# ayumiymk/DiG

Measured on AMD Instinct MI355X. Metric: pretrain images/sec (32x128, 2-view, mask 0.7) ViT-S/4, higher is better.
Workload: dtype bf16

## Files before the change

### cpu_abi/dig_cpu.cpp

```cpp
#include <algorithm>
#include <cmath>
#include <cstdint>
#include <cstring>
#include <vector>

#include "dig_cpu_common.h"

namespace {

inline float gelu_f(float x) { return 0.5f * x * (1.0f + std::erf(x * 0.70710678118654752f)); }
inline float dgelu_f(float x) {
  const float cdf = 0.5f * (1.0f + std::erf(x * 0.70710678118654752f));
  return cdf + x * 0.39894228040143268f * std::exp(-0.5f * x * x);
}
inline float drop_apply(float v, const dig_dropout_t& d, long long i, int j, int cols) {
  float s = 1.f;
  if (d.pthr) s = drop_keep(d.pk0, d.pk1, (unsigned)(i / d.rows_per_sample), 0u, d.pthr) ? d.pscale : 0.f;
  if (d.thr) {
    s *= d.scale;
    return drop_keep(d.k0, d.k1, (unsigned)i * (unsigned)cols + (unsigned)j, 0u, d.thr) ? v * s : 0.f;
  }
  return v * s;
}

// ... 39 lines not shown
#pragma omp parallel for collapse(2)
    for (int s = 0; s < splits; ++s)
      for (int i = 0; i < I; ++i) {
        const int r0 = s * per, r1 = std::min(R, r0 + per);
        for (int j = 0; j < J; ++j) {
          float acc = 0.f;
          for (int r = r0; r < r1; ++r) acc += a[(size_t)i * R + r] * b[(size_t)j * R + r];
          C[((size_t)s * I + i) * J + j] = acc;
        }
      }
    return DIG_OK;
  }
  const int groups = (I + 63) / 64;
  std::vector<float> csum(colsum_partials ? (size_t)groups * J : 0, 0.f);
#pragma omp parallel for
  for (int g = 0; g < groups; ++g)
    for (int i = g * 64; i < std::min(I, g * 64 + 64); ++i)
      for (int j = 0; j < J; ++j) {
        float acc = 0.f;
        for (int r = 0; r < R; ++r) acc += a[(size_t)i * R + r] * b[(size_t)j * R + r];
        float v = (acc + (bias ? bias[j] : 0.f)) * (j < alpha_cols ? alpha : 1.0f);
        if (act == 1) {
          if (pre) pre[(size_t)i * ldp + j] = f2bf(v);
          v = gelu_f(v);
          if (dropping) v = drop_apply(v, *drop, i, j, J);
        } else if (act == 2) {
          v *= dgelu_f(bf2f(resid[(size_t)i * ldr + j]));
          if (dropping) v = drop_apply(v, *drop, i, j, J);
          if (colsum_partials) csum[(size_t)g * J + j] += v;
        } else if (dropping) {
          v = drop_apply(v, *drop, i, j, J);
        }
        if (resid && act != 2) v += bf2f(resid[(size_t)i * ldr + j]);
        if (out_kind == 0) ((bf16_t*)C_)[(size_t)i * ldc + j] = f2bf(v);
        else ((float*)C_)[(size_t)i * ldc + j] = v;
      }
  if (colsum_partials) std::memcpy(colsum_partials, csum.data(), csum.size() * sizeof(float));
  return DIG_OK;
}

int dig_gemm_bf16(const void* A, const void* B, void* C, int I, int J, int R, int lda, int ldb, int ldc, int trans_a, int trans_b,
                  int out_kind, const float* bias, const void* resid, int ldr, void* pre_act, int ldp, float alpha, int alpha_cols,
                  int act, int splits, int a_rows, int b_rows, int bk, float* colsum_partials, hipStream_t stream) {
  return dig_gemm_bf16_dropout(A, B, C, I, J, R, lda, ldb, ldc, trans_a, trans_b, out_kind, bias, resid, ldr, pre_act, ldp, alpha, alpha_cols,
                               act, splits, a_rows, b_rows, bk, colsum_partials, nullptr, stream);
}

int dig_reduce_partials_bf16(const float* partials, int splits, long long n, void* out_, hipStream_t) {
  if (int rc = dig_rules::reduce_partials_bf16(partials, splits, n, out_)) return rc;
  bf16_t* out = (bf16_t*)out_;
  for (long long e = 0; e < n; ++e) {
    float a = 0.f;
    for (int s = 0; s < splits; ++s) a += partials[(long long)s * n + e];
    out[e] = f2bf(a);
  }
  return DIG_OK;
}
int dig_reduce_partials(const float* partials, int splits, long long n, float* out, int accumulate, hipStream_t) {
  if (int rc = dig_rules::reduce_partials(partials, splits, n, out, accumulate)) return rc;
#pragma omp parallel for
  for (long long e = 0; e < n; ++e) {
    float acc = accumulate ? out[e] : 0.f;
    for (int s = 0; s < splits; ++s) acc += partials[(long long)s * n + e];
    out[e] = acc;
  }
  return DIG_OK;
}

int dig_reduce_partials_multi(const dig_reduce_seg_t* segs, int n_segs, hipStream_t stream) {
  if (int rc = dig_rules::reduce_partials_multi(segs, n_segs)) return rc;
  for (int k = 0; k < n_segs; ++k) {
    const int rc = dig_reduce_partials(segs[k].partials, segs[k].splits, segs[k].n, segs[k].out, 1, stream);
    if (rc) return rc;
  }
  return DIG_OK;
}

int dig_colsum_partials_multi(const dig_colsum_seg_t* segs, int n_segs, hipStream_t) {
  if (int rc = dig_rules::colsum_partials_multi(segs, n_segs)) return rc;
  for (int k = 0; k < n_segs; ++k) {
    const dig_colsum_seg_t& g = segs[k];
    for (int c = 0; c < g.C; ++c) {
      float a = 0.f;
      for (int b = 0; b < g.n_parts; ++b) a += g.partials[(size_t)b * g.stride + c];
      g.out[c] += a;
    }
  }
  return DIG_OK;
}

int dig_attn_fwd_dropout(const void* qkv_, void* ctx_, float* lse, int n_img, int heads, int embed_dim, const dig_dropout_t* drop,
                         int q_rows, hipStream_t) {
  if (int rc = dig_rules::attn_fwd_dropout(qkv_, ctx_, lse, n_img, heads, embed_dim, drop, q_rows)) return rc;
  const bf16_t* qkv = (const bf16_t*)qkv_;
  bf16_t* ctx = (bf16_t*)ctx_;
  const int D = embed_dim, ld = 3 * D, nq = (q_rows + 31) / 32 * 32;
  const bool dropping = drop && drop->thr;
#pragma omp parallel for collapse(2)
  for (int b = 0; b < n_img; ++b)
    for (int h = 0; h < heads; ++h) {
      std::vector<float> s(N_TOK);
      for (int i = 0; i < nq; ++i) {
        const bf16_t* q = qkv + ((size_t)b * N_TOK + i) * ld + h * DH;
        float mx = -3.0e38f;
        for (int j = 0; j < N_TOK; ++j) {
          const bf16_t* k = qkv + ((size_t)b * N_TOK + j) * ld + D + h * DH;
          float acc = 0.f;
          for (int c = 0; c < DH; ++c) acc += bf2f(q[c]) * bf2f(k[c]);
          s[j] = acc;
          mx = std::max(mx, acc);
        }
        float sum = 0.f;
        for (int j = 0; j < N_TOK; ++j) { s[j] = std::exp(s[j] - mx); sum += s[j]; }
        lse[((size_t)b * heads + h) * N_TOK + i] = mx + std::log(sum);
        const float inv = 1.0f / sum;
        float o[DH];
        for (int c = 0; c < DH; ++c) o[c] = 0.f;
        for (int j = 0; j < N_TOK; ++j) {
          float p = s[j] * inv;
          if (dropping) p = drop_keep(drop->k0, drop->k1, ((unsigned)i << 16) | (unsigned)j, (unsigned)(b * heads + h), drop->thr) ? p * drop->scale : 0.f;
          const bf16_t* v = qkv + ((size_t)b * N_TOK + j) * ld + 2 * D + h * DH;
          for (int c = 0; c < DH; ++c) o[c] += p * bf2f(v[c]);
        }
        for (int c = 0; c < DH; ++c) ctx[((size_t)b * N_TOK + i) * D + h * DH + c] = f2bf(o[c]);
      }
    }
  return DIG_OK;
}

int dig_attn_fwd(const void* qkv, void* ctx, float* lse, int n_img, int heads, int embed_dim, hipStream_t stream) {
  return dig_attn_fwd_dropout(qkv, ctx, lse, n_img, heads, embed_dim, nullptr, N_TOK, stream);
}

int dig_attn_bwd_mode(int) { return 0; }
int dig_attn_bwd_store(int) { return 0; }

int dig_attn_block_fwd(const void* ln1, const void* x, const void* qkv_w, const float* qkv_b, const void* proj_w, const float* proj_b,
                       void* qkv, void* ctx, float* lse, void* x_mid, int n_img, int heads, int embed_dim, float scale, hipStream_t stream) {
  if (int rc = dig_rules::attn_block_fwd(ln1, x, qkv_w, qkv_b, proj_w, proj_b, qkv, ctx, lse, x_mid, n_img, heads, embed_dim, scale)) return rc;
  const int D = embed_dim, R = n_img * N_TOK;
  std::vector<bf16_t> tq;
  std::vector<float> tl;
  if (!qkv) {
    tq.resize((size_t)R * 3 * D + 8);
    tl.resize((size_t)n_img * heads * N_TOK);
    qkv = (void*)(((uintptr_t)tq.data() + 15) & ~(uintptr_t)15);
    lse = tl.data();
  }
  int rc = dig_gemm_bf16(ln1, qkv_w, qkv, R, 3 * D, D, D, D, 3 * D, 0, 0, 0, qkv_b, nullptr, 0, nullptr, 0, scale, D, 0, 1, 0, 0, 0, nullptr, stream);
  if (rc) return rc;
  rc = dig_attn_fwd(qkv, ctx, lse, n_img, heads, D, stream);
  if (rc) return rc;
  return dig_gemm_bf16(ctx, proj_w, x_mid, R, D, D, D, D, D, 0, 0, 0, proj_b, x, D, nullptr, 0, 1.0f, 0, 0, 1, 0, 0, 0, nullptr, stream);
}

int dig_attn_bwd_dropout(const void* qkv_, const void* ctx_, const void* dctx_, const float* lse, void* dqkv_, int n_img, int heads,
                         int embed_dim, float scale, float* q_colsum, float* v_colsum, const dig_dropout_t* drop, int q_rows, hipStream_t) {
  if (int rc = dig_rules::attn_bwd_dropout(qkv_, ctx_, dctx_, lse, dqkv_, n_img, heads, embed_dim, scale, q_colsum, v_colsum, drop, q_rows))
    return rc;
  const int nqb = (q_rows + 31) / 32;
  const bf16_t* qkv = (const bf16_t*)qkv_;
  const bf16_t* ctx = (const bf16_t*)ctx_;
  const bf16_t* dctx = (const bf16_t*)dctx_;
  bf16_t* dqkv = (bf16_t*)dqkv_;
  const int D = embed_dim, ld = 3 * D, nq = nqb * 32;
  const bool dropping = drop && drop->thr;
#pragma omp parallel for
  for (int b = 0; b < n_img; ++b) {
    std::vector<float> qs(q_colsum ? D : 0, 0.f), vs(q_colsum ? D : 0, 0.f);
    for (int h = 0; h < heads; ++h) {
      std::vector<float> dk((size_t)N_TOK * DH, 0.f), dv((size_t)N_TOK * DH, 0.f), p(N_TOK), dp(N_TOK);
      for (int i = 0; i < nq; ++i) {
        const size_t row = (size_t)b * N_TOK + i;
        const bf16_t* q = qkv + row * ld + h * DH;
        const bf16_t* o = ctx + row * D + h * DH;
        const bf16_t* go = dctx + row * D + h * DH;
        const float l = lse[((size_t)b * heads + h) * N_TOK + i];
        float delta = 0.f;
        for (int c = 0; c < DH; ++c) delta += bf2f(go[c]) * bf2f(o[c]);
        for (int j = 0; j < N_TOK; ++j) {
          const bf16_t* k = qkv + ((size_t)b * N_TOK + j) * ld + D + h * DH;
          const bf16_t* v = qkv + ((size_t)b * N_TOK + j) * ld + 2 * D + h * DH;
          float s = 0.f, d = 0.f;
          for (int c = 0; c < DH; ++c) { s += bf2f(q[c]) * bf2f(k[c]); d += bf2f(go[c]) * bf2f(v[c]); }
          p[j] = std::exp(s - l);
          dp[j] = d;
        }
        float dq[DH];
        for (int c = 0; c < DH; ++c) dq[c] = 0.f;
        for (int j = 0; j < N_TOK; ++j) {
          float keep = 1.f;
          if (dropping) keep = drop_keep(drop->k0, drop->k1, ((unsigned)i << 16) | (unsigned)j, (unsigned)(b * heads + h), drop->thr) ? drop->scale : 0.f;
          const float pd = bf2f(f2bf(p[j] * keep));
          const float ds = bf2f(f2bf(p[j] * (dp[j] * keep - delta)));
          const bf16_t* k = qkv + ((size_t)b * N_TOK + j) * ld + D + h * DH;
          for (int c = 0; c < DH; ++c) {
            dq[c] += ds * bf2f(k[c]);
            dk[(size_t)j * DH + c] += ds * bf2f(q[c]);
            dv[(size_t)j * DH + c] += pd * bf2f(go[c]);
          }
        }
        for (int c = 0; c < DH; ++c) {
          dqkv[row * ld + h * DH + c] = f2bf(dq[c] * scale);
          if (q_colsum) qs[h * DH + c] += dq[c] * scale;
        }
      }
      for (int j = 0; j < N_TOK; ++j)
        for (int c = 0; c < DH; ++c) {
          dqkv[((size_t)b * N_TOK + j) * ld + D + h * DH + c] = f2bf(dk[(size_t)j * DH + c]);
          dqkv[((size_t)b * N_TOK + j) * ld + 2 * D + h * DH + c] = f2bf(dv[(size_t)j * DH + c]);
          if (q_colsum) vs[h * DH + c] += dv[(size_t)j * DH + c];
        }
    }
    if (q_colsum) {
      std::memcpy(q_colsum + (size_t)b * D, qs.data(), D * sizeof(float));
      std::memcpy(v_colsum + (size_t)b * D, vs.data(), D * sizeof(float));
    }
  }
  return DIG_OK;
}

int dig_attn_bwd(const void* qkv, const void* ctx, const void* dctx, const float* lse, void* dqkv, int n_img, int heads, int embed_dim,
                 float scale, float* q_colsum, float* v_colsum, hipStream_t stream) {
  return dig_attn_bwd_dropout(qkv, ctx, dctx, lse, dqkv, n_img, heads, embed_dim, scale, q_colsum, v_colsum, nullptr, N_TOK, stream);
}

int dig_attn_bwd_proj(const void* qkv, const void* ctx, const void* dy_, const void* projt_, const float* lse, void* dqkv, int n_img, int heads,
                      int embed_dim, float scale, float* q_colsum, float* v_colsum, hipStream_t stream) {
  if (int rc = dig_rules::attn_bwd_proj(qkv, ctx, dy_, projt_, lse, dqkv, n_img, heads, embed_dim, scale, q_colsum, v_colsum)) return rc;
  const int D = embed_dim;
  const long R = (long)n_img * N_TOK;
  const uint16_t* dy = (const uint16_t*)dy_;
  const uint16_t* wt = (const uint16_t*)projt_;
  std::vector<float> w((size_t)D * D);
  for (size_t k = 0; k < w.size(); ++k) w[k] = bf2f(wt[k]);
  std::vector<uint16_t> dctx((size_t)R * D);
#pragma omp parallel for
  for (long r = 0; r < R; ++r) {
    std::vector<float> row(D);
    for (int o = 0; o < D; ++o) row[o] = bf2f(dy[r * D + o]);
    for (int i = 0; i < D; ++i) {
      float a = 0.f;
      for (int o = 0; o < D; ++o) a += row[o] * w[(size_t)i * D + o];
      dctx[r * D + i] = f2bf(a);
    }
  }
  return dig_attn_bwd(qkv, ctx, dctx.data(), lse, dqkv, n_img, heads, embed_dim, scale, q_colsum, v_colsum, stream);
}


int dig_layernorm_fwd(const void* x_, const float* gamma, const float* beta, void* y_, float* mean, float* rstd, int rows, int D, float eps,
                      int fuse_gelu, hipStream_t) {
  if (int rc = dig_rules::layernorm_fwd(x_, gamma, beta, y_, mean, rstd, rows, D, eps, fuse_gelu)) return rc;
  const bf16_t* x = (const bf16_t*)x_;
  bf16_t* y = (bf16_t*)y_;
#pragma omp parallel for
  for (int r = 0; r < rows; ++r) {
    float s = 0.f;
    for (int c = 0; c < D; ++c) s += bf2f(x[(size_t)r * D + c]);
    const float mu = s / D;
    float q = 0.f;
    for (int c = 0; c < D; ++c) { const float d = bf2f(x[(size_t)r * D + c]) - mu; q += d * d; }
    const float rs = 1.0f / std::sqrt(q / D + eps);
    for (int c = 0; c < D; ++c) {
      float v = (bf2f(x[(size_t)r * D + c]) - mu) * rs * gamma[c] + beta[c];
      if (fuse_gelu) v = gelu_f(v);
      y[(size_t)r * D + c] = f2bf(v);
    }
    mean[r] = mu;
    rstd[r] = rs;
  }
  return DIG_OK;
}


int dig_layernorm_bwd_partials(const void* dy_, const void* x_, const float* gamma, const float* beta, const float* mean, const float* rstd,
                               const void* dres_, void* dx_, float* workspace, int rows, int D, int fuse_gelu, hipStream_t) {
  if (int rc = dig_rules::layernorm_bwd_partials(dy_, x_, gamma, beta, mean, rstd, dres_, dx_, workspace, rows, D, fuse_gelu)) return rc;
  const bf16_t* dy = (const bf16_t*)dy_;
  const bf16_t* x = (const bf16_t*)x_;
  const bf16_t* dres = (const bf16_t*)dres_;
  bf16_t* dx = (bf16_t*)dx_;
  const int parts = dig_rules::layernorm_bwd_parts(rows);
  std::memset(workspace, 0, (size_t)parts * 3 * D * sizeof(float));
#pragma omp parallel for
  for (int p = 0; p < parts; ++p) {
    float* w = workspace + (size_t)p * 3 * D;
    std::vector<float> xh(D), d(D);
    for (int r = p; r < rows; r += parts) {
      float c1 = 0.f, c2 = 0.f;
      for (int c = 0; c < D; ++c) {
        xh[c] = (bf2f(x[(size_t)r * D + c]) - mean[r]) * rstd[r];
        float g = bf2f(dy[(size_t)r * D + c]);
        if (fuse_gelu) g *= dgelu_f(xh[c] * gamma[c] + beta[c]);
        w[c] += g * xh[c];
        w[D + c] += g;
        d[c] = g * gamma[c];
        c1 += d[c];
        c2 += d[c] * xh[c];
      }
      c1 /= D;
      c2 /= D;
      for (int c = 0; c < D; ++c) {
        float o = rstd[r] * (d[c] - c1 - xh[c] * c2);
        if (dres) { const float e = bf2f(dres[(size_t)r * D + c]); o += e; w[2 * D + c] += e; }
        dx[(size_t)r * D + c] = f2bf(o);
// ... 1101 lines not shown
```

### dig_amd/block_calls.py

```python
import ctypes
import math
from typing import NamedTuple

import torch

from . import ops

BF16, F32 = torch.bfloat16, torch.float32
_F32_PIECES = ("lse", "mu2", "rs2", "nmu", "nrs")


class Plan(NamedTuple):
    defer: bool
    red_defer: bool
    tile_direct: int
    attn_proj: bool
    fuse_ln2: bool
    chain_proj: bool


class _BlockSaved:
    __slots__ = ("b16", "b32", "off", "rows", "D", "F", "n_img", "heads", "inp", "inp_ptr")

    def __init__(self, b16, b32, off, rows, D, F, n_img, heads, inp, inp_ptr):
        self.b16, self.b32, self.off, self.rows, self.D, self.F, self.n_img, self.heads = b16, b32, off, rows, D, F, n_img, heads
        self.inp = inp
        self.inp_ptr = inp_ptr

    def ptr(self, name):
        return (self.b32 if name in _F32_PIECES else self.b16).data_ptr() + self.off[name]

    def view(self, name):
        R, D, F = self.rows, self.D, self.F
        if name == "lse":
            a = self.off["lse"] // 4
            return self.b32[a:a + self.n_img * self.heads * 256].view(self.n_img * self.heads, 256)
        if name in _F32_PIECES:
            a = self.off[name] // 4
            return self.b32[a:a + R]
        cols = {"qkv": 3 * D, "pre": F, "act": F}.get(name, D)
        a = self.off[name] // 2
        return self.b16[a:a + R * cols].view(R, cols)

    def tensors(self):
        if len(self.inp) == 4:
            x, ln1, mu1, rs1 = self.inp
        else:
            p = self.inp[2]
            x, ln1, mu1, rs1 = p.view("out"), p.view("nln"), p.view("nmu"), p.view("nrs")
        return (x, ln1, mu1, rs1) + tuple(self.view(k) for k in ("qkv", "ctx", "lse", "x_mid", "ln2", "mu2", "rs2", "pre", "act"))


def forward(blocks, x, n_img, heads, Fh, eps, save, fuse_attn):
    R, D = x.shape
    dev = x.device
    off, n16, n32 = ops.block_fwd_layout(R, D, Fh, n_img, heads, save)
    ln1, mu1, rs1 = ops.layernorm_fwd(x, blocks[0]["norm1.weight"], blocks[0]["norm1.bias"], eps)
    inp, inp_ptr = (x, ln1, mu1, rs1), (x.data_ptr(), ln1.data_ptr(), mu1.data_ptr(), rs1.data_ptr())
    stream, key, fuse_attn = ops.L.stream(), ("fwd_call", bool(save), R, n_img), int(fuse_attn)
    saved, prev = [], None
    for i, blk in enumerate(blocks):
        st = blk.get(key)
        if st is None:
            nb = blocks[i + 1] if i + 1 < len(blocks) else None
            st = blk[key] = ops.BlockFwd(
                n_img=n_img, heads=heads, D=D, F=Fh, rows=R, save=int(bool(save)),
                tile_qkv=ops.fwd_tile_code(R, 3 * D, D) or ops.GEMM_BK_FWD, tile_proj=ops.fwd_tile_code(R, D, D, has_resid=True) or ops.GEMM_BK_FWD,
                fuse_attn=fuse_attn, eps=eps, scale=(D // heads) ** -0.5,
                qkv_w=blk["attn.qkv.weight"].data_ptr(), qkv_b=blk["qkv_bias"].data_ptr(), proj_w=blk["attn.proj.weight"].data_ptr(),
                proj_b=blk["attn.proj.bias"].data_ptr(), n2_g=blk["norm2.weight"].data_ptr(), n2_b=blk["norm2.bias"].data_ptr(),
                fc1_w=blk["mlp.fc1.weight"].data_ptr(), fc1_b=blk["mlp.fc1.bias"].data_ptr(), fc2_w=blk["mlp.fc2.weight"].data_ptr(),
                fc2_b=blk["mlp.fc2.bias"].data_ptr(), next_n1_g=nb["norm1.weight"].data_ptr() if nb else None,
                next_n1_b=nb["norm1.bias"].data_ptr() if nb else None)
        b16 = torch.empty(n16 // 2, device=dev, dtype=BF16)
        b32 = torch.empty(n32 // 4, device=dev, dtype=F32)
        p16, p32 = b16.data_ptr(), b32.data_ptr()
        st.fuse_attn = fuse_attn
        st.x, st.ln1 = inp_ptr[0], inp_ptr[1]
        for k in off:
            setattr(st, k, (p32 if k in _F32_PIECES else p16) + off[k])
        ops.L.call("dig_encoder_block_fwd", ctypes.byref(st), stream)
        cur = _BlockSaved(b16, b32, off, R, D, Fh, n_img, heads, inp, inp_ptr)
        if save:
            saved.append(cur)
            inp, inp_ptr = (b16, b32, cur), (p16 + off["out"], p16 + off["nln"], p32 + off["nmu"], p32 + off["nrs"])
        else:
            inp, inp_ptr = (b16, b32), (p16 + off["out"], p16 + off["nln"], 0, 0)
        prev = cur
    return prev.view("out"), saved


def _bwd_struct(blk, wplan, n_img, heads, D, Fh, R):
    g, gb = blk["g"], blk["g"]["qkv_bias"]
    assert all(g[k].is_contiguous() for k in ("attn.qkv.weight", "attn.proj.weight", "mlp.fc1.weight", "mlp.fc2.weight"))
    return ops.BlockBwd(
        n_img=n_img, heads=heads, D=D, F=Fh, rows=R, tile_dgrad=ops.dgrad_tile_code(R, D) or ops.GEMM_BK_BWD, scale=(D // heads) ** -0.5,
        qkv_w=blk["attn.qkv.weight"].data_ptr(), proj_w=blk["attn.proj.weight"].data_ptr(),
        n1_g=blk["norm1.weight"].data_ptr(), n1_b=blk["norm1.bias"].data_ptr(), n2_g=blk["norm2.weight"].data_ptr(),
        n2_b=blk["norm2.bias"].data_ptr(),
        g_n1_g=g["norm1.weight"].data_ptr(), g_n1_b=g["norm1.bias"].data_ptr(), g_qkv_w=g["attn.qkv.weight"].data_ptr(),
        g_q_b=gb.data_ptr(), g_v_b=gb[2 * D:].data_ptr(), g_proj_w=g["attn.proj.weight"].data_ptr(),
        g_proj_b=g["attn.proj.bias"].data_ptr(), g_n2_g=g["norm2.weight"].data_ptr(), g_n2_b=g["norm2.bias"].data_ptr(),
        g_fc1_w=g["mlp.fc1.weight"].data_ptr(), g_fc1_b=g["mlp.fc1.bias"].data_ptr(), g_fc2_w=g["mlp.fc2.weight"].data_ptr(),
        g_fc2_b=g["mlp.fc2.bias"].data_ptr(),
        wg_fn=wplan.fn, wg_wa=wplan.wa, wg_splits=wplan.splits, wg_n_wg=wplan.n_wg, wg_fold_splits=wplan.splits,
        wg_trans=(ctypes.c_int * 4)(*wplan.trans))


def _hold_back(red, g, t32, off, R, n_img, D, Fh, n_b, n_l2):
    def piece(name, *shape):
        a = off[name] // 4
        return t32[a:a + math.prod(shape)].view(shape)
    gb = g["qkv_bias"]
    red.colsum_partials(piece("bparts", n_b, Fh), g["mlp.fc1.bias"])
    red.layernorm_finalize_parts(piece("ws2", n_l2, 3, D), g["norm2.weight"], g["norm2.bias"], g["mlp.fc2.bias"])
    red.colsum_partials(piece("qs", n_img, D), gb[:D])
    red.colsum_partials(piece("vs", n_img, D), gb[2 * D:])
    red.layernorm_finalize(t32[off["ws1"] // 4:], R, D, g["norm1.weight"], g["norm1.bias"], g["attn.proj.bias"])


def backward(plan, blocks, saved, dx, wT, wplan, n_img, heads, Fh, side, keep, block_done, grad_ready):
    R, D = dx.shape
    dev = dx.device
    off, n16, n32 = ops.block_bwd_layout(R, D, Fh, n_img)
    grp = wplan.group
    stream, key = ops.L.stream(), ("bwd_call", R, n_img)
    n_b, n_l2 = ops.L.query("dig_mlp_chain_colsum_rows", R), ops.L.query("dig_mlp_chain_ln_parts", R)
    red = ops.GradReduceBatch() if plan.red_defer else None

    def block(i, dy_ptr, probs, fold=None):
        blk, sv = blocks[i], saved[i]
        saved[i] = None
        st = blk.get(key)
        if st is None:
            st = blk[key] = _bwd_struct(blk, wplan, n_img, heads, D, Fh, R)
        w2t, w1t, projt, qkvt = wT[i]
        st.w2t, st.w1t = w2t.data_ptr(), w1t.data_ptr()
        st.projt = projt.data_ptr() if plan.chain_proj else None
        st.tile_direct, st.attn_proj = plan.tile_direct, int(plan.attn_proj)
        st.proj_wt = projt.data_ptr() if (plan.tile_direct or plan.attn_proj) else None
        st.qkv_wt = qkvt.data_ptr() if plan.tile_direct else None
        st.wg_defer, st.fuse_ln2, st.defer_red = int(plan.defer), int(plan.fuse_ln2), int(plan.red_defer)
        st.x, st.ln1, st.mu1, st.rs1 = sv.inp_ptr
        for k in ("qkv", "ctx", "lse", "x_mid", "ln2", "mu2", "rs2", "pre", "act"):
            setattr(st, k, sv.ptr(k))
        t16 = torch.empty(n16 // 2, device=dev, dtype=BF16)
        t32 = torch.empty(n32 // 4, device=dev, dtype=F32)
        p16, p32 = t16.data_ptr(), t32.data_ptr()
        st.dy = dy_ptr
        for k in off:
            setattr(st, k, (p16 if k in ("dln2", "dpre", "dctx", "dqkv") else p32) + off[k])
        slabs = grp.next_slabs(wplan.slab_bytes)
        st.wg_map, st.wg_slabs, st.wg_probs = wplan.wmap.data_ptr(), slabs.data_ptr(), ctypes.addressof(probs)
        st.wg_fold_n, st.wg_fold_probs, st.wg_fold_slabs = (4, ctypes.addressof(fold[0]), fold[1].data_ptr()) if fold else (0, None, None)
        st.side = side
        if red:
            _hold_back(red, blk["g"], t32, off, R, n_img, D, Fh, n_b, n_l2)
        ops.L.call("dig_encoder_block_bwd", ctypes.byref(st), stream)
        if keep is not None and not red:
            keep(t32)
        block_done()
        return t16, t32, slabs

    def ready(i):
        if i is not None:
            grad_ready(f"encoder.blocks.{i}")

    def inline():
        tables = ((ops._WgProb * 4)(), (ops._WgProb * 4)())
        t16, t32, last, dy_ptr = dx, None, None, dx.data_ptr()
        for n, i in enumerate(reversed(range(len(blocks)))):
            t16, t32, slabs = block(i, dy_ptr, tables[n & 1], last and (last[1], last[2]))
            dy_ptr = t16.data_ptr() + off["dctx"]
            ready(last and last[0])
            last = (i, tables[n & 1], slabs)
        return t16, last

    def deferred():
        t16, t32, held, dy_ptr = dx, None, [], dx.data_ptr()
        for i in reversed(range(len(blocks))):
            own, sv = (ops._WgProb * 4)(), saved[i]
            t16, t32, _ = block(i, dy_ptr, own)
            held.append((i, own, t16, sv))
            dy_ptr = t16.data_ptr() + off["dctx"]
        if red:
            red.flush()
        last = None
        for i, own, _, _ in held:
            slabs = grp.next_slabs(wplan.slab_bytes)
            grp.call(ctypes.addressof(own), 4, ctypes.addressof(last[1]) if last else None, 4 if last else 0, wplan.splits, wplan.wmap, wplan.n_wg,
                     slabs, last and last[2], wplan.splits)
            ready(last and last[0])
            last = (i, own, slabs)
        return t16, last

    t16, (i, table, slabs) = (deferred if plan.defer else inline)()
    grp.fold(ctypes.addressof(table), 4, slabs, wplan.splits)
    ready(i)
    a = off["dctx"] // 2
    return t16[a:a + R * D].view(R, D)


def defer_fits(cache, dev, extra_bytes):
    key = (dev.index, extra_bytes)
    if key not in cache:
        free, _ = torch.cuda.mem_get_info(dev)
        pooled = torch.cuda.memory_reserved(dev) - torch.cuda.memory_allocated(dev)
        cache[key] = extra_bytes <= (free + pooled) // 4
    return cache[key]
```

### dig_amd/build.py

```python
import os
import subprocess
import sys
from concurrent.futures import ThreadPoolExecutor

HERE = os.path.dirname(os.path.abspath(__file__))
CSRC = os.path.join(HERE, "csrc")
LIBDIR = os.path.join(HERE, "lib")
LIB = os.path.join(LIBDIR, "libdig_hip.so")
FLAGS = ["--offload-arch=gfx950", "-O3", "-std=c++17", "-fPIC", "-munsafe-fp-atomics", "-ffp-contract=fast",
         "-Wno-unused-result"]
FLAGS.append("-fno-slp-vectorize")
EXTRA_FLAGS = {"keyview.hip": ["-ffp-contract=off"], "abiaug.hip": ["-ffp-contract=off"]}


def sources():
    return sorted(f for f in os.listdir(CSRC) if f.endswith(".hip"))


def source_hash() -> str:
    import hashlib
    h = hashlib.sha256()
    files = sorted(os.path.join(CSRC, f) for f in os.listdir(CSRC) if f.endswith((".hip", ".h", ".inc")))
    inc = os.path.join(os.path.dirname(HERE), "include")
    files += sorted(os.path.join(inc, f) for f in os.listdir(inc) if f.endswith(".h"))
    for f in files:
        h.update(os.path.basename(f).encode())
        with open(f, "rb") as fh:
            h.update(fh.read())
    h.update(repr((FLAGS, sorted(EXTRA_FLAGS.items()))).encode())
    return h.hexdigest()[:16]


def _stale(out, deps):
    if not os.path.exists(out):
        return True
    t = os.path.getmtime(out)
    return any(os.path.getmtime(d) > t for d in deps)


def build(force: bool = False, verbose: bool = True) -> str:
    hipcc = os.environ.get("HIPCC", "/opt/rocm/bin/hipcc")
    os.makedirs(LIBDIR, exist_ok=True)
    objdir = os.path.join(LIBDIR, "obj")
    os.makedirs(objdir, exist_ok=True)
    headers = [os.path.join(CSRC, f) for f in os.listdir(CSRC) if f.endswith((".h", ".inc"))]
    inc = os.path.join(os.path.dirname(HERE), "include")
    headers += [os.path.join(inc, f) for f in os.listdir(inc) if f.endswith(".h")]
    headers = [h for h in headers if os.path.exists(h)]
    jobs = []
    for s in sources():
        src = os.path.join(CSRC, s)
        obj = os.path.join(objdir, s[:-4] + ".o")
        if force or _stale(obj, [src] + headers):
            jobs.append((src, obj))

    def cc(job):
        src, obj = job
        cmd = [hipcc] + FLAGS + EXTRA_FLAGS.get(os.path.basename(src), []) + ["-I", os.path.join(os.path.dirname(HERE), "include"), "-c", src, "-o", obj]
        r = subprocess.run(cmd, capture_output=True, text=True)
        if r.returncode != 0:
            raise RuntimeError(f"hipcc failed for {src}:\n{r.stderr}")
        if verbose:
            print("[dig_amd.build] compiled", os.path.basename(src), flush=True)

    with ThreadPoolExecutor(max_workers=min(8, max(1, len(jobs)))) as ex:
        list(ex.map(cc, jobs))
    objs = [os.path.join(objdir, s[:-4] + ".o") for s in sources()]
    if force or jobs or _stale(LIB, objs):
        r = subprocess.run([hipcc, "--offload-arch=gfx950", "-shared", "-fPIC", "-o", LIB] + objs,
                           capture_output=True, text=True)
        if r.returncode != 0:
            raise RuntimeError("link failed:\n" + r.stderr)
        if verbose:
            print("[dig_amd.build] linked", LIB, flush=True)
    return LIB


HOT_KERNELS = ("mlp_chain_kernel<1, true, false>", "mlp_chain_kernel<2, true, false>", "mlp_chain_kernel<0, true, false>",
               "wgrad_wide_kernel<3, 7>", "attn_block_kernel<true, 2>", "attn_block_kernel<false, 2>", "attn_bwd_kernel<false, 3, false>", "attn_bwd_kernel<false, 3, true>",
               "gemm_wide_kernel<false, true, 0, 4, 3, 2, 2, false, 64, 2, false>", "gemm_pwide_kernel<4, false, false>",
               "keyview_sample_kernel", "keyview_stage_a_kernel", "keyview_stage_b_kernel",
               "abiaug_sample_kernel", "abiaug_warp_kernel", "abiaug_det_kernel", "abiaug_tail_kernel",
               "lexicon_search_kernel",
               "tcv_fwd_kernel", "tcv_bwd_q_kernel", "tcv_bwd_k_kernel",
               "ctc_kernel<false>", "ctc_kernel<true>",
               "ctc_beam_kernel",
               "ctc_lex_score_kernel",
               "ctc_align_kernel",
               "addattn_fwd_slots_kernel", "attn_beam_advance_kernel")
LLVM_BIN = os.environ.get("DIG_LLVM_BIN", "/opt/rocm/lib/llvm/bin")


def kernel_resources():
    import re
    import tempfile
    rows = []
    objdir = os.path.join(LIBDIR, "obj")
    with tempfile.TemporaryDirectory() as tmp:
        for o in sorted(f for f in os.listdir(objdir) if f.endswith(".o")):
            fat, dev = os.path.join(tmp, o + ".fat"), os.path.join(tmp, o + ".co")
            r = subprocess.run([os.path.join(LLVM_BIN, "llvm-objcopy"), f"--dump-section=.hip_fatbin={fat}", os.path.join(objdir, o)], capture_output=True, text=True)
            if r.returncode != 0 or not os.path.exists(fat):
                continue
            subprocess.run([os.path.join(LLVM_BIN, "clang-offload-bundler"), "--unbundle", "--type=o", f"--input={fat}",
                            "--targets=hipv4-amdgcn-amd-amdhsa--gfx950", f"--output={dev}"], check=True, capture_output=True)
            notes = subprocess.run([os.path.join(LLVM_BIN, "llvm-readelf"), "--notes", dev], check=True, capture_output=True, text=True).stdout
            for blk in notes.split("- .agpr_count")[1:]:
                f = {k: re.search(rf"\.{k}:\s+(\S+)", blk) for k in ("name", "private_segment_fixed_size", "vgpr_count", "sgpr_count")}
                if not all(f.values()):
                    continue
                mangled = f["name"].group(1)
                try:
                    dm = subprocess.run(["c++filt", mangled], capture_output=True, text=True).stdout.strip() or mangled
                except OSError:
                    dm = mangled
                short = re.sub(r"^void ", "", dm).replace("(anonymous namespace)::", "")
                rows.append({"name": short, "object": o, "scratch": int(f["private_segment_fixed_size"].group(1)),
                             "vgpr": int(f["vgpr_count"].group(1)), "sgpr": int(f["sgpr_count"].group(1)),
                             "hot": any(short.startswith(h) for h in HOT_KERNELS)})
    return rows


def check_scratch(rows=None, raise_on_fail=True):
    rows = kernel_resources() if rows is None else rows
    missing = [h for h in HOT_KERNELS if not any(r["name"].startswith(h) for r in rows)]
    bad = [r for r in rows if r["hot"] and r["scratch"] > 0]
    if raise_on_fail and (bad or missing):
        raise RuntimeError(f"hot kernels with scratch memory: {[(b['name'][:60], b['scratch']) for b in bad]}; not found: {missing}")
    return bad + [{"name": m + " (not found)", "scratch": -1} for m in missing]


if __name__ == "__main__":
    build(force="--force" in sys.argv)
```

### dig_amd/csrc/abi_rules.h

```cpp
#pragma once
#include <cstddef>
#include <cstdint>

#include "../../include/dig_hip.h"

static inline bool aligned16(const void* p) { return (((uintptr_t)p) & 15u) == 0; }
static inline bool aligned8(const void* p) { return (((uintptr_t)p) & 7u) == 0; }
static inline bool ranges_overlap(const void* a, const void* b, size_t bytes) {
  const uintptr_t x = (uintptr_t)a, y = (uintptr_t)b;
  return x < y + bytes && y < x + bytes;
}

namespace dig_rules {

constexpr int LDS_LIMIT = 160 * 1024;
constexpr unsigned long long OFFSET_LIMIT = 1ull << 32;
constexpr int ATTN_TOKENS = 256, ATTN_HEAD_DIM = 64;
constexpr int ATTN_BWD_PROJ_MAX_DIM = 512;
constexpr int ATTN_BLOCK_DIM = 384, ATTN_BLOCK_HEADS = 6;
constexpr int GEMM_BR = 64;
constexpr int CHAIN_DIM = 384, CHAIN_FC = 64, CHAIN_ROWS = 128, CHAIN_SLOT = 16384;
constexpr int CHAIN_MAX_F = 6144, CHAIN_LN_MAX_F = 2048;
constexpr int BN_FUSED_COLS = 32, BN_FUSED_MAX_ROWS = 4096, BN_FUSED_MIN_C = 256;
constexpr int PATCH_EMBED_MAX_D = 1024;
// ... 274 lines not shown
}

static inline int layernorm_fwd(const void* x, const float* gamma, const float* beta, void* y, float* mean, float* rstd, int rows, int D, float eps,
                                int fuse_gelu) {
  if (!x || !gamma || !beta || !y || !mean || !rstd || rows <= 0) return DIG_ERR_ARG;
  if (!aligned16(x) || !aligned16(y)) return DIG_ERR_ALIGN;
  if (!layernorm_dim_ok(D)) return DIG_ERR_UNSUPPORTED;
  return DIG_OK;
}
static inline int layernorm_bwd_partials(const void* dy, const void* x, const float* gamma, const float* beta, const float* mean, const float* rstd,
                                         const void* dres, void* dx, float* workspace, int rows, int D, int fuse_gelu) {
  if (!dy || !x || !gamma || !mean || !rstd || !dx || !workspace || rows <= 0) return DIG_ERR_ARG;
  if (fuse_gelu && !beta) return DIG_ERR_ARG;
  if (!aligned16(x) || !aligned16(dy) || !aligned16(dx) || (dres && !aligned16(dres))) return DIG_ERR_ALIGN;
  if (!layernorm_dim_ok(D)) return DIG_ERR_UNSUPPORTED;
  return DIG_OK;
}

static inline int mask_views_u8(const void* mask, int elem_kind, int B, int V, int N, int keep_views, unsigned char* out) {
  if (!mask || !out || B <= 0 || V <= 0 || N <= 0 || keep_views < 0) return DIG_ERR_ARG;
  if (elem_kind < 0 || elem_kind > 4) return DIG_ERR_UNSUPPORTED;
  return DIG_OK;
}
static inline int colsum_partials_multi(const dig_colsum_seg_t* segs, int n_segs) {
  if (!segs || n_segs < 1 || n_segs > DIG_COLSUM_MAX_SEGS) return DIG_ERR_ARG;
  for (int k = 0; k < n_segs; ++k) {
    const dig_colsum_seg_t& g = segs[k];
    if (!g.partials || !g.out || g.n_parts <= 0 || g.C <= 0 || (g.C & 7) || g.stride < g.C || (g.stride & 3)) return DIG_ERR_ARG;
    if (!aligned16(g.partials)) return DIG_ERR_ALIGN;
  }
  return DIG_OK;
}

static inline int beam_step(const float* logits, int ld, float* seq_scores, int B, int beam_width, int C, int eos, long long* symbols,
                            long long* predecessors, float* stored_scores) {
  return beam_common(logits, ld, seq_scores, B, beam_width, BEAM_STEP_MAX_WIDTH, C, symbols, predecessors, stored_scores);
}
static inline int attn_beam_advance(const float* logits, int ld, float* seq_scores, int B, int beam_width, int C, int eos, long long* symbols,
                                    long long* predecessors, float* stored_scores, const long long* force_candidates, const float* s_in,
                                    const void* sbf_in, float* s_out, void* sbf_out, int S, const float* table, int E, void* inp, int ld_inp) {
  if (!s_in || !sbf_in || !s_out || !sbf_out || !table || !inp || S <= 0 || E <= 0 || ld_inp < E) return DIG_ERR_ARG;
  if (int rc = beam_common(logits, ld, seq_scores, B, beam_width, BEAM_ADVANCE_MAX_WIDTH, C, symbols, predecessors, stored_scores)) return rc;
  const size_t rows = (size_t)B * beam_width * S;
  if (ranges_overlap(s_in, s_out, rows * sizeof(float)) || ranges_overlap(sbf_in, sbf_out, rows * 2)) return DIG_ERR_ARG;
  return DIG_OK;
}

static inline int tcv_attn_fwd(const void* film, const void* u, const void* vk, const void* mem, const float* lnc_g, const float* lnc_b, float eps,
                               void* c, float* lse, float* wmean, int S, int Lq, int N, int heads, int d, int slots_per_mem,
                               const dig_dropout_t* drop) {
  if (!c || !lse) return DIG_ERR_ARG;
  if (int rc = tcv_common(film, u, vk, mem, lnc_g, lnc_b, S, Lq, N, heads, d, slots_per_mem)) return rc;
  if (!aligned16(c)) return DIG_ERR_ALIGN;
  return DIG_OK;
}
static inline int tcv_attn_bwd(const void* film, const void* u, const void* vk, const void* mem, const float* lnc_g, const float* lnc_b, float eps,
                               const void* c, const float* lse, const void* dc, void* du, void* dfilm, void* dvk, void* dmem, float* dlnc_g,
                               float* dlnc_b, float* workspace, int S, int Lq, int N, int heads, int d, int slots_per_mem,
                               const dig_dropout_t* drop) {
  if (!c || !lse || !dc || !du || !dfilm || !dvk || !dmem || !dlnc_g || !dlnc_b || !workspace) return DIG_ERR_ARG;
  if (int rc = tcv_common(film, u, vk, mem, lnc_g, lnc_b, S, Lq, N, heads, d, slots_per_mem)) return rc;
  if (slots_per_mem != 1) return DIG_ERR_UNSUPPORTED;
  if (!aligned16(c) || !aligned16(dc) || !aligned16(du) || !aligned16(dfilm) || !aligned16(dvk) || !aligned16(dmem)) return DIG_ERR_ALIGN;
  return DIG_OK;
}

static inline int ctc_loss(const float* logits, int ld, const long long* target, int ldt, const long long* target_len, int len_offset, int B, int T,
                           int C, int blank, float* nll, float* loss) {
  if (!nll || !loss) return DIG_ERR_ARG;
  return ctc_common(logits, ld, target, ldt, target_len, B, T, C, blank);
}
static inline int ctc_loss_bwd(const float* logits, int ld, const long long* target, int ldt, const long long* target_len, int len_offset,
                               const float* gscalar, int B, int T, int C, int blank, void* dlogits, int ldd, int dlogits_is_f32) {
  if (!dlogits || ldd < C) return DIG_ERR_ARG;
  return ctc_common(logits, ld, target, ldt, target_len, B, T, C, blank);
}
static inline int ctc_align(const float* logits, int ld, const long long* target, int ldt, const long long* target_len, int len_offset, int B, int T,
                            int C, int blank, int* start, int* end, float* char_logp, float* path_logp, int* frame_label) {
  if (!start || !end || !char_logp || !path_logp) return DIG_ERR_ARG;
  return ctc_common(logits, ld, target, ldt, target_len, B, T, C, blank);
}

static inline int abiaug_sample(dig_abi_params* params, long long* info, const int* heights, const int* widths, int n_img, const dig_abi_run* run,
                                unsigned long long seed, unsigned step) {
  if (!params || !info || !heights || !widths || n_img <= 0 || !abi_run_ok(run)) return DIG_ERR_ARG;
  return DIG_OK;
}
static inline int abiaug_workspace_bytes(int geom, int det, int wh, int ww, const dig_abi_run* run) {
  if (!abi_run_ok(run) || wh <= 0 || ww <= 0) return DIG_ERR_ARG;
  return DIG_OK;
}
static inline int abiaug_warp_u8(const unsigned char* packed, const long long* offsets, const int* heights, const int* widths, int n_img,
                                 const dig_abi_params* params, const dig_abi_run* run, unsigned char* work, long long work_bytes, int max_wh,
                                 int max_ww) {
  if (!packed || !offsets || !heights || !widths || !params || !abi_run_ok(run) || n_img <= 0 || max_wh <= 0 || max_ww <= 0 ||
      work_bytes < 0 || (work_bytes > 0 && !work))
    return DIG_ERR_ARG;
  return DIG_OK;
}
static inline int abiaug_deteriorate_u8(const unsigned char* packed, const long long* offsets, const int* heights, const int* widths, int n_img,
                                        const dig_abi_params* params, const dig_abi_run* run, unsigned char* work, long long work_bytes, int max_wh,
                                        int max_ww) {
  if (!packed || !offsets || !heights || !widths || !params || !abi_run_ok(run) || n_img <= 0 || max_wh <= 0 || max_ww <= 0 ||
      work_bytes < 0 || (work_bytes > 0 && !work))
    return DIG_ERR_ARG;
  return DIG_OK;
}
static inline int abiaug_tail(const unsigned char* packed, const long long* offsets, const int* heights, const int* widths, int n_img,
                              const dig_abi_params* params, const dig_abi_run* run, const unsigned char* work, long long work_bytes, float* out,
                              int out_h, int out_w, float mean, float std_, int max_wh, int max_ww) {
  if (!packed || !offsets || !heights || !widths || !params || !abi_run_ok(run) || !out || n_img <= 0 || out_h <= 0 || out_w <= 0 ||
      max_wh <= 0 || max_ww <= 0 || std_ == 0.f || work_bytes < 0 || (work_bytes > 0 && !work))
    return DIG_ERR_ARG;
  if (abiaug_tail_lds_bytes(out_h, out_w, resize_taps(max_ww, out_w), resize_taps(max_wh, out_h)) > LDS_LIMIT) return DIG_ERR_UNSUPPORTED;
  return DIG_OK;
}

static inline int attn_fwd_dropout(const void* qkv, void* ctx, float* lse, int n_img, int heads, int embed_dim, const dig_dropout_t* drop,
                                   int q_rows) {
  if (!qkv || !ctx || !lse || n_img <= 0 || heads <= 0 || embed_dim != (long long)heads * ATTN_HEAD_DIM || q_rows < 1 || q_rows > ATTN_TOKENS) return DIG_ERR_ARG;
  if (!aligned16(qkv) || !aligned16(ctx)) return DIG_ERR_ALIGN;
  if (attn_qkv_bytes_over(n_img, embed_dim)) return DIG_ERR_ARG;
  return DIG_OK;
}
static inline int attn_bwd_dropout(const void* qkv, const void* ctx, const void* dctx, const float* lse, void* dqkv, int n_img, int heads,
                                   int embed_dim, float scale, float* q_colsum, float* v_colsum, const dig_dropout_t* drop, int q_rows) {
  if (!qkv || !ctx || !dctx || !lse || !dqkv || n_img <= 0 || heads <= 0 || embed_dim != (long long)heads * ATTN_HEAD_DIM || q_rows < 1 || q_rows > ATTN_TOKENS) return DIG_ERR_ARG;
  if ((q_rows + 31) / 32 < 8 && q_colsum) return DIG_ERR_UNSUPPORTED;
  if ((q_colsum == nullptr) != (v_colsum == nullptr)) return DIG_ERR_ARG;
  if (!aligned16(qkv) || !aligned16(ctx) || !aligned16(dctx) || !aligned16(dqkv)) return DIG_ERR_ALIGN;
  if (attn_qkv_bytes_over(n_img, embed_dim)) return DIG_ERR_ARG;
  return DIG_OK;
}
static inline int attn_bwd_proj(const void* qkv, const void* ctx, const void* dy, const void* projt, const float* lse, void* dqkv, int n_img,
                                int heads, int embed_dim, float scale, float* q_colsum, float* v_colsum) {
  if (!qkv || !ctx || !dy || !projt || !lse || !dqkv || n_img <= 0 || heads <= 0) return DIG_ERR_ARG;
  if ((q_colsum == nullptr) != (v_colsum == nullptr)) return DIG_ERR_ARG;
  if (embed_dim != (long long)heads * ATTN_HEAD_DIM || (embed_dim & 127) || embed_dim > ATTN_BWD_PROJ_MAX_DIM) return DIG_ERR_UNSUPPORTED;
  if (!aligned16(qkv) || !aligned16(ctx) || !aligned16(dy) || !aligned16(projt) || !aligned16(dqkv)) return DIG_ERR_ALIGN;
  if (attn_qkv_bytes_over(n_img, embed_dim)) return DIG_ERR_ARG;
  return DIG_OK;
}

static inline int attn_block_fwd(const void* ln1, const void* x, const void* qkv_w, const float* qkv_b, const void* proj_w, const float* proj_b,
                                 void* qkv, void* ctx, float* lse, void* x_mid, int n_img, int heads, int embed_dim, float scale) {
  if (!ln1 || !x || !qkv_w || !proj_w || !ctx || !x_mid || n_img <= 0) return DIG_ERR_ARG;
  if ((qkv == nullptr) != (lse == nullptr)) return DIG_ERR_ARG;
  if (!attn_block_supported(heads, embed_dim)) return DIG_ERR_UNSUPPORTED;
  if (!aligned16(ln1) || !aligned16(x) || !aligned16(qkv_w) || !aligned16(proj_w) || !aligned16(ctx) || !aligned16(x_mid) || (qkv && !aligned16(qkv)))
    return DIG_ERR_ALIGN;
  if (attn_qkv_bytes_over(n_img, ATTN_BLOCK_DIM)) return DIG_ERR_ARG;
  return DIG_OK;
}

static inline int im2col3x3(const void* x, void* col, int n_img, int H, int W, int C, int ldc) {
  if (!x || !col || n_img <= 0 || H <= 0 || W <= 0 || C <= 0 || (C & 7) || ldc < 9LL * C || (ldc & 7)) return DIG_ERR_ARG;
  if (!aligned16(x) || !aligned16(col)) return DIG_ERR_ALIGN;
  return DIG_OK;
}
static inline int conv3x3_weight_flip(const void* w, void* wt, int c_out, int c_in) {
  if (!w || !wt || c_out <= 0 || c_in <= 0) return DIG_ERR_ARG;
  return DIG_OK;
}
static inline int maxpool2x2_fwd(const void* x, void* y, unsigned char* idx, int n_img, int H, int W, int C) {
  if (!x || !y || !idx || n_img <= 0 || H <= 0 || W <= 0 || (H & 1) || (W & 1) || C <= 0 || (C & 7)) return DIG_ERR_ARG;
  if (!aligned16(x) || !aligned16(y) || !aligned8(idx)) return DIG_ERR_ALIGN;
  return DIG_OK;
}
static inline int maxpool2x2_bwd(const void* dy, const unsigned char* idx, void* dx, int n_img, int H, int W, int C) {
  if (!dy || !dx || !idx || n_img <= 0 || H <= 0 || W <= 0 || (H & 1) || (W & 1) || C <= 0 || (C & 7)) return DIG_ERR_ARG;
  if (!aligned16(dy) || !aligned16(dx) || !aligned8(idx)) return DIG_ERR_ALIGN;
  return DIG_OK;
}

static inline int ctc_greedy_decode(const float* logits, int ld, int B, int T, int C, int blank, int eos, int padding, long long* ids, float* score,
                                    int* n) {
  if (!logits || !ids || !score || !n || B < 0 || T <= 0 || C <= 0 || ld < C) return DIG_ERR_ARG;
  if (T > CTC_MAX_T || C < 2 || C > CTC_MAX_C) return DIG_ERR_UNSUPPORTED;
  return DIG_OK;
}
static inline int ctc_beam_decode(const float* logits, int ld, int B, int T, int C, int blank, int eos, int padding, int beam_width, long long* ids,
                                  float* score, float* logp, int* n) {
  if (!logits || !ids || !score || !logp || !n || B < 0 || T <= 0 || C <= 0 || ld < C || blank < 0 || blank >= C || beam_width <= 0) return DIG_ERR_ARG;
  if (T > CTC_MAX_T || C < 2 || C > CTC_MAX_C || beam_width > CTC_MAX_W) return DIG_ERR_UNSUPPORTED;
  return DIG_OK;
}
static inline int ctc_lexicon_decode(const float* logits, int ld, int B, int T, int C, int blank, int eos, int padding, const int* words,
                                     const int* word_len, int ldw, int W, const int* lex_begin, const int* lex_count, int max_count, int* best_index,
                                     float* logp, long long* ids, float* score, int* n, float* scores, void* workspace, long long workspace_bytes) {
  if (!logits || !words || !word_len || !lex_begin || !lex_count || !best_index || !logp || !ids || !score || !n || !workspace) return DIG_ERR_ARG;
  if (B < 0 || T <= 0 || C <= 0 || ldw <= 0 || ld < C || blank < 0 || blank >= C || W < 0 || max_count < 0) return DIG_ERR_ARG;
  if (T > CTC_MAX_T || C < 2 || C > CTC_MAX_C || ldw > CTC_MAX_LDT || B > GRID_Y_MAX) return DIG_ERR_UNSUPPORTED;
  if (B == 0) return DIG_OK;
  if (!aligned8(workspace)) return DIG_ERR_ALIGN;
  if (workspace_bytes < ctc_lexicon_workspace_bytes(B, T, C, max_count)) return DIG_ERR_ARG;
  return DIG_OK;
}

static inline int decode_embed(const long long* tokens, const float* emb, const float* pe_row, void* x, int B, int d, int vocab) {
  if (!tokens || !emb || !pe_row || !x || B <= 0 || d <= 0 || vocab <= 0) return DIG_ERR_ARG;
  return DIG_OK;
}
static inline int decode_self_attn(const void* qkv_cache, void* out, int B, int T, int heads, int head_dim, int t, float scale) {
  if (!qkv_cache || !out || B <= 0 || heads <= 0 || t < 0 || t >= T) return DIG_ERR_ARG;
  if (!seq_head_dim_ok(head_dim)) return DIG_ERR_UNSUPPORTED;
  return DIG_OK;
}
static inline int decode_cross_attn(const void* q, const void* kv_mem, void* out, float* weights, int B, int n_mem, int heads, int head_dim,
                                    float scale, int slots_per_mem) {
  if (!q || !kv_mem || !out || B <= 0 || n_mem <= 0 || heads <= 0 || slots_per_mem < 1 || B % slots_per_mem) return DIG_ERR_ARG;
  if (!seq_head_dim_ok(head_dim) || n_mem > DECODE_MAX_MEM) return DIG_ERR_UNSUPPORTED;
  if (!aligned16(kv_mem) || !aligned16(q)) return DIG_ERR_ALIGN;
  return DIG_OK;
}
static inline int softmax_argmax(const float* logits, int ld, float* probs, long long* tokens, int B, int C) {
  if (!logits || !probs || !tokens || B <= 0 || C <= 0 || ld < C) return DIG_ERR_ARG;
  return DIG_OK;
}

static inline int patch_embed_fwd(const float* img, const float* W, const float* bias, const unsigned char* mask, const float* mask_token,
                                  const float* pos, void* out, int n_img, int gh, int gw, int D) {
  if (!img || !W || !bias || !mask_token || !pos || !out || n_img <= 0 || D <= 0 || D > PATCH_EMBED_MAX_D || (D & 63)) return DIG_ERR_ARG;
  return DIG_OK;
}
static inline int patch_embed_bwd(const void* dy, const float* img, const unsigned char* mask, float* dW, float* dbias, float* dmask_token,
                                  int n_img, int gh, int gw, int D) {
  if (!dy || !img || !dW || !dbias || !dmask_token || n_img <= 0 || D <= 0 || D > PATCH_EMBED_MAX_D || (D & 63)) return DIG_ERR_ARG;
  return DIG_OK;
}
static inline int window_pool_fwd(const void* x, void* out, int out_is_f32, int n_img, int gh, int gw, int nwin, int D) {
  if (!x || !out || n_img <= 0 || nwin <= 0 || gh <= 0 || gw <= 0 || (D & 1)) return DIG_ERR_ARG;
  return DIG_OK;
}
static inline int window_pool_bwd(const void* dpool, void* dx, int n_img, int gh, int gw, int nwin, int D, int accumulate) {
  if (!dpool || !dx || n_img <= 0 || nwin <= 0 || gh <= 0 || gw <= 0 || (D & 1)) return DIG_ERR_ARG;
  return DIG_OK;
}
static inline int mask_to_index(const unsigned char* mask, int* idx, int* count, int B, int N, int max_per_sample) {
  if (!mask || !idx || !count || B <= 0 || N <= 0 || max_per_sample <= 0) return DIG_ERR_ARG;
  return DIG_OK;
}
static inline int gather_rows(const void* src, const int* idx, void* dst, int M, int M_pad, int D) {
  if (!src || !idx || !dst || M <= 0 || M_pad < M || (D & 7)) return DIG_ERR_ARG;
  if (!aligned16(src) || !aligned16(dst)) return DIG_ERR_ALIGN;
  return DIG_OK;
}
static inline int scatter_rows_add(const void* src, const int* idx, void* dst, int M, int D) {
  if (!src || !idx || !dst || M <= 0 || (D & 7)) return DIG_ERR_ARG;
  if (!aligned16(src) || !aligned16(dst)) return DIG_ERR_ALIGN;
  return DIG_OK;
}
static inline int mim_target(const float* img, const int* idx, float* target, int M, int gh, int gw, int normalize) {
  if (!img || !idx || !target || M <= 0) return DIG_ERR_ARG;
  return DIG_OK;
}
static inline int mse_fwd_bwd_ws(const float* pred, int ld_pred, const float* target, int M, int C, float gscale, float* loss, void* dpred,
                                 int ld_dpred, float* workspace) {
  if (!pred || !target || M <= 0 || C <= 0 || ld_pred < C || (dpred && ld_dpred < C)) return DIG_ERR_ARG;
  return DIG_OK;
}
static inline int add_bf16(const void* a, const void* b, void* out, long long n) {
  if (!a || !b || !out || n <= 0 || (n & 7)) return DIG_ERR_ARG;
  if (!aligned16(a) || !aligned16(b) || !aligned16(out)) return DIG_ERR_ALIGN;
  return DIG_OK;
}
static inline int gelu_bwd(const void* dact, const void* pre, void* dpre, long long n) {
  if (!dact || !pre || !dpre || n <= 0 || (n & 7)) return DIG_ERR_ARG;
  if (!aligned16(dact) || !aligned16(pre) || !aligned16(dpre)) return DIG_ERR_ALIGN;
  return DIG_OK;
}
static inline int colsum(const void* x, float* out, float* workspace, int rows, int C, int ld) {
  if (!x || !out || !workspace || rows <= 0 || C <= 0 || (C & 7) || (ld & 7)) return DIG_ERR_ARG;
  if (!aligned16(x)) return DIG_ERR_ALIGN;
  return DIG_OK;
}
static inline int colsum_partials(const float* partials, int n_parts, int C, float* out) {
  if (!partials || !out || n_parts <= 0 || C <= 0 || (C & 7)) return DIG_ERR_ARG;
  if (!aligned16(partials)) return DIG_ERR_ALIGN;
  return DIG_OK;
}
static inline int patchify_bf16(const float* img, const unsigned char* mask, void* out, int n_img, int gh, int gw) {
  if (!img || !out || n_img <= 0) return DIG_ERR_ARG;
  if (!aligned16(img) || !aligned16(out)) return DIG_ERR_ALIGN;
  return DIG_OK;
}
static inline int colsum_masked(const void* x, const unsigned char* mask, float* out_unmasked, float* out_masked, float* workspace, int rows, int C) {
  if (!x || !mask || !out_unmasked || !out_masked || !workspace || rows <= 0 || C <= 0 || (C & 7)) return DIG_ERR_ARG;
  if (!aligned16(x)) return DIG_ERR_ALIGN;
  return DIG_OK;
}
static inline int dropout_apply(const void* in, void* out, long long rows, int cols, const dig_dropout_t* drop) {
  if (!in || !out || !drop || rows <= 0 || cols <= 0 || (cols & 7) || rows >= (1ll << 32) || rows * cols >= (1ll << 32)) return DIG_ERR_ARG;
  if (drop->pthr && drop->rows_per_sample <= 0) return DIG_ERR_ARG;
  if (!aligned16(in) || !aligned16(out)) return DIG_ERR_ALIGN;
  return DIG_OK;
}

static inline int reduce_partials_bf16(const float* partials, int splits, long long n, void* out) {
  if (!partials || !out || splits < 1 || n <= 0 || (n & 3)) return DIG_ERR_ARG;
  if (!aligned16(partials) || !aligned8(out)) return DIG_ERR_ALIGN;
  return DIG_OK;
}
static inline int reduce_partials(const float* partials, int splits, long long n, float* out, int accumulate) {
  if (!partials || !out || splits < 1 || n <= 0 || (n & 3)) return DIG_ERR_ARG;
  if (!aligned16(partials) || !aligned16(out)) return DIG_ERR_ALIGN;
  return DIG_OK;
// ... 357 lines not shown
```

### dig_amd/csrc/attn_block.hip

```cpp
#include "common.h"
#include "lds_dma.h"
#include "attn_tiles.h"
#include <type_traits>

#ifndef DIG_AB_SAFE_WAITS
#define DIG_AB_SAFE_WAITS 0
#endif
#ifndef DIG_AB_NSPLIT
#define DIG_AB_NSPLIT 2
#endif
#ifndef DIG_AB_P0
#define DIG_AB_P0 2
#define DIG_AB_P1 5
#define DIG_AB_P2 8
#endif
#ifndef DIG_AB_PRIO
#define DIG_AB_PRIO 0
#endif
#ifndef DIG_AB_NT
#define DIG_AB_NT 1
#endif
#ifndef DIG_AB_SKEW
#define DIG_AB_SKEW 0
#endif
#ifndef DIG_AB_ABL
#define DIG_AB_ABL 0
#endif
#ifndef DIG_AB_TS
#define DIG_AB_TS(k)
#define DIG_AB_TS_BEGIN()
#define DIG_AB_TS_END()
#endif

namespace {

constexpr int KD = dig_rules::ATTN_BLOCK_DIM;
constexpr int NH = dig_rules::ATTN_BLOCK_HEADS;
constexpr int SLOTB = 24576;
constexpr int RING_OFF = 0;
constexpr int K_OFF = 3 * SLOTB;
constexpr int V_OFF = K_OFF + 32768;
constexpr int VEC_OFF = V_OFF + 32768;
constexpr int STG_OFF = VEC_OFF + (3 * KD + KD) * 4;
constexpr int LDS_BYTES = STG_OFF + 8 * 2048;
constexpr int NTICK = 48;

struct AbParams {
  const bf16_t* X;
  const bf16_t* resid;
  const bf16_t* Wqkv;
  const float* bqkv;
  const bf16_t* Wp;
  const float* bp;
  bf16_t* qkv;
  bf16_t* ctx;
  float* lse;
  bf16_t* out;
  float scale;
  unsigned x_bytes;
};

template <int N>
__device__ __forceinline__ void ab_wait_vm() {
  if (DIG_AB_SAFE_WAITS) asm volatile("s_waitcnt vmcnt(0)" ::: "memory");
  else asm volatile("s_waitcnt vmcnt(%0)" ::"n"(N) : "memory");
}
__device__ __forceinline__ void ab_wait_lgkm0() { asm volatile("s_waitcnt lgkmcnt(0)" ::: "memory"); }

template <bool NT = false>
__device__ __forceinline__ void store_block_lines(bf16_t* blk , int ld, unsigned (&P)[2][4][2],
                                                  unsigned char* stg, int lane) {
  const int rr = lane & 31, hi = lane >> 5;
  const int wr = (rr & 15) * 128 + hi * 8, ws = rr & 7;
  const int r8 = lane >> 3, c = lane & 7;
#pragma unroll
  for (int pass = 0; pass < 2; ++pass) {
    if ((rr >> 4) == pass) {
#pragma unroll
      for (int b = 0; b < 2; ++b)
#pragma unroll
        for (int g = 0; g < 4; ++g) *reinterpret_cast<uint2*>(stg + wr + (((4 * b + g) ^ ws) << 4)) = make_uint2(P[b][g][0], P[b][g][1]);
    }
    asm volatile("s_waitcnt lgkmcnt(0)" ::: "memory");
    __builtin_amdgcn_wave_barrier();
    const dig_u32x4 v0 = *reinterpret_cast<const dig_u32x4*>(stg + r8 * 128 + ((c ^ (r8 & 7)) << 4));
    const dig_u32x4 v1 = *reinterpret_cast<const dig_u32x4*>(stg + (8 + r8) * 128 + ((c ^ (r8 & 7)) << 4));
    asm volatile("s_waitcnt lgkmcnt(0)" ::: "memory");
    __builtin_amdgcn_wave_barrier();
    if (!(DIG_AB_ABL & 4)) {
      dig_u32x4* d0 = reinterpret_cast<dig_u32x4*>(blk + (size_t)(16 * pass + r8) * ld + c * 8);
      dig_u32x4* d1 = reinterpret_cast<dig_u32x4*>(blk + (size_t)(16 * pass + 8 + r8) * ld + c * 8);
      if (NT) { __builtin_nontemporal_store(v0, d0); __builtin_nontemporal_store(v1, d1); }
      else { *d0 = v0; *d1 = v1; }
    }
  }
}

template <bool SAVE> struct AbCounts {
  static constexpr int E_BLK = (DIG_AB_ABL & 4) ? 0 : (SAVE ? 4 : 0);
  static constexpr int E_ATT = (DIG_AB_ABL & 4) ? 0 : 4 + (SAVE ? 1 : 0);
  static constexpr int E_OUT = (DIG_AB_ABL & 4) ? 0 : 4;
  static constexpr int E_RES = 4;
};

__device__ __forceinline__ int ab_opaque(int v) {
  asm volatile("" : "+v"(v));
  return v;
}

template <bool SAVE, int NSPLIT>
__global__ __launch_bounds__(512) void attn_block_kernel(AbParams p) {
  using C = AbCounts<SAVE>;
  extern __shared__ __attribute__((aligned(16))) unsigned char smem[];
  const int tid0 = threadIdx.x;
  const int wave = __builtin_amdgcn_readfirstlane(tid0 >> 6);
  const int img = blockIdx.x;
  DIG_AB_TS_BEGIN()
#if DIG_AB_PRIO
  if (wave >= 4) __builtin_amdgcn_s_setprio(1);
#endif
#if DIG_AB_SKEW
  for (int i = 0; i < (int)((blockIdx.x >> 3) & 15); ++i) __builtin_amdgcn_s_sleep(DIG_AB_SKEW);
#endif

  const dig_u32x4 rWq = make_rsrc(p.Wqkv, 3u * KD * KD * 2u);
  const dig_u32x4 rWp = make_rsrc(p.Wp, (unsigned)(KD * KD * 2));
  const dig_u32x4 rRes = make_rsrc(p.resid, p.x_bytes);
  const unsigned lds0 = (unsigned)(uintptr_t)LDS_PTR(smem);

  auto piece_voff = [&](int tid, int k) -> unsigned {
    if (k < 2) {
      const int r0 = tid >> 4, c0 = (tid & 15) ^ (r0 & 15);
      return (unsigned)(((r0 + 32 * k) * KD + 8 * c0) * 2);
    }
    const int r2 = tid >> 3, c2 = (tid & 7) ^ ((r2 >> 1) & 7);
    return (unsigned)((r2 * KD + 128 + 8 * c2) * 2);
  };
  dig_u32x4 src_rs = rWq;
  unsigned src_off = 0;
  auto select_source = [&](bool proj, int row0) {
#pragma unroll
    for (int e = 0; e < 4; ++e) src_rs[e] = proj ? rWp[e] : rWq[e];
    src_off = (unsigned)(row0 * KD * 2);
  };
  auto issue_piece = [&](int slot, int tau, int k, unsigned voff) {
    if (DIG_AB_ABL & 16) voff = 0x7fffff00u;
    dma16(lds0 + (unsigned)(RING_OFF + slot * SLOTB + k * 8192 + wave * 1024), voff, src_rs, src_off + (unsigned)(tau * 192 * 2));
  };
#pragma unroll
  for (int tau = 0; tau < 2; ++tau)
#pragma unroll
    for (int k = 0; k < 3; ++k) issue_piece(tau, tau, k, piece_voff(tid0, k));

  dig_u32x4 xf[KD / 16];
  auto load_rows = [&](const bf16_t* base) {
    const int tid = ab_opaque(tid0);
    const auto rX = __builtin_amdgcn_make_buffer_rsrc((void*)base, 0, p.x_bytes, 0x00020000);
    const unsigned xo = (unsigned)((((unsigned)img * 256u + (unsigned)(wave * 32 + (tid & 31))) * KD + ((tid >> 5) & 1) * 8) * 2);
#pragma unroll
    for (int s = 0; s < KD / 16; ++s) xf[s] = __builtin_amdgcn_raw_buffer_load_b128(rX, xo, s * 32, 0);
  };
  load_rows(p.X);
  {
    float* vec = reinterpret_cast<float*>(smem + VEC_OFF);
#pragma unroll
    for (int u = 0; u < 3; ++u) {
      const int i = u * 512 + tid0;
      float v;
      if (i < 3 * KD) v = p.bqkv ? p.bqkv[i] : 0.f;
      else v = p.bp ? p.bp[i - 3 * KD] : 0.f;
      vec[i] = v;
    }
  }

  auto tick = [&](auto slot_tag, auto tau_tag, auto nw_tag, auto pre_tag, f32x16 (&acc)[2], auto&& pre_fn) {
    constexpr int SLOT = decltype(slot_tag)::value, TAU = decltype(tau_tag)::value, NW = decltype(nw_tag)::value;
    constexpr int FREE = (SLOT + 2) % 3;
    DIG_AB_TS(0)
    ab_wait_vm<NW>();
    ab_wait_lgkm0();
    __builtin_amdgcn_s_barrier();
    asm volatile("" ::: "memory");
    DIG_AB_TS(1)
    if (decltype(pre_tag)::value) pre_fn();
    const int tid = ab_opaque(tid0);
    const int rr = tid & 31, hi = (tid >> 5) & 1;
    const int bA = rr * 256 + ((hi ^ (rr & 15)) << 4) + RING_OFF + SLOT * SLOTB;
    const int bB = 16384 + rr * 128 + ((hi ^ ((rr >> 1) & 7)) << 4) + RING_OFF + SLOT * SLOTB;
    auto frag = [&](int s, int half) {
      const int a = s < 8 ? (bA ^ (s << 5)) + half * 8192 : (bB ^ ((s - 8) << 5)) + half * 4096;
      return *reinterpret_cast<const bf16x8*>(smem + a);
    };
    bf16x8 fa[2], fb[2];
    fa[0] = frag(0, 0);
    fa[1] = frag(0, 1);
    __builtin_amdgcn_sched_barrier(0);
    auto kstep = [&](auto s_tag, bf16x8 (&cur)[2], bf16x8 (&nxt)[2]) {
      constexpr int S = decltype(s_tag)::value;
      if constexpr (S < 11) {
        nxt[0] = frag(S + 1, 0);
        nxt[1] = frag(S + 1, 1);
      }
      if (!(DIG_AB_ABL & 2)) {
        acc[0] = __builtin_amdgcn_mfma_f32_32x32x16_bf16(cur[0], __builtin_bit_cast(bf16x8, xf[TAU * 12 + S]), acc[0], 0, 0, 0);
        acc[1] = __builtin_amdgcn_mfma_f32_32x32x16_bf16(cur[1], __builtin_bit_cast(bf16x8, xf[TAU * 12 + S]), acc[1], 0, 0, 0);
      } else {
        asm volatile("" ::"v"(cur[0]), "v"(cur[1]));
      }
      if (S == DIG_AB_P0) issue_piece(FREE, TAU, 0, piece_voff(tid, 0));
      if (S == DIG_AB_P1) issue_piece(FREE, TAU, 1, piece_voff(tid, 1));
      if (S == DIG_AB_P2) issue_piece(FREE, TAU, 2, piece_voff(tid, 2));
      __builtin_amdgcn_sched_barrier(0);
    };
    kstep(std::integral_constant<int, 0>{}, fa, fb); kstep(std::integral_constant<int, 1>{}, fb, fa);
    kstep(std::integral_constant<int, 2>{}, fa, fb); kstep(std::integral_constant<int, 3>{}, fb, fa);
    kstep(std::integral_constant<int, 4>{}, fa, fb); kstep(std::integral_constant<int, 5>{}, fb, fa);
    kstep(std::integral_constant<int, 6>{}, fa, fb); kstep(std::integral_constant<int, 7>{}, fb, fa);
    kstep(std::integral_constant<int, 8>{}, fa, fb); kstep(std::integral_constant<int, 9>{}, fb, fa);
    kstep(std::integral_constant<int, 10>{}, fa, fb); kstep(std::integral_constant<int, 11>{}, fb, fa);
    DIG_AB_TS(2)
  };
  auto no_pre = []() {};
  using FALSE_ = std::false_type;
  using TRUE_ = std::true_type;

  auto finish_block = [&](const f32x16 (&acc)[2], int vec_col0, float al, unsigned (&P)[2][4][2], int hi) {
    const float* bv = reinterpret_cast<const float*>(smem + VEC_OFF + (vec_col0 + 4 * hi) * 4);
#pragma unroll
    for (int b = 0; b < 2; ++b)
#pragma unroll
      for (int g = 0; g < 4; ++g) {
        const f32x4 b4 = *reinterpret_cast<const f32x4*>(bv + 32 * b + 8 * g);
        P[b][g][0] = pack_bf2((acc[b][4 * g] + b4[0]) * al, (acc[b][4 * g + 1] + b4[1]) * al);
        P[b][g][1] = pack_bf2((acc[b][4 * g + 2] + b4[2]) * al, (acc[b][4 * g + 3] + b4[3]) * al);
      }
  };
  const size_t wave_row0 = (DIG_AB_ABL & 32) ? (size_t)wave * 32 : (size_t)img * 256 + wave * 32;

  bf16x8 Qp[4];

  auto head = [&](auto first_tag, int h) {
    constexpr bool FIRST = decltype(first_tag)::value;
    constexpr int EPREV = FIRST ? 0 : C::E_BLK + C::E_ATT;
    using I0 = std::integral_constant<int, 0>;
    using I1 = std::integral_constant<int, 1>;
    using I2 = std::integral_constant<int, 2>;
    f32x16 acc[2];
    unsigned P[2][4][2];
    auto zero = [&]() {
#pragma unroll
      for (int b = 0; b < 2; ++b)
#pragma unroll
        for (int e = 0; e < 16; ++e) acc[b][e] = 0.f;
    };
    select_source(false, KD + h * 64);
    zero();
    tick(I0{}, I0{}, std::integral_constant<int, 3 + EPREV>{}, FALSE_{}, acc, no_pre);
    tick(I1{}, I1{}, std::integral_constant<int, 3 + EPREV>{}, FALSE_{}, acc, no_pre);
    {
      const int tid = ab_opaque(tid0), hi = (tid >> 5) & 1;
      finish_block(acc, h * 64, p.scale, P, hi);
#pragma unroll
      for (int b = 0; b < 2; ++b)
#pragma unroll
        for (int u = 0; u < 2; ++u)
          Qp[2 * b + u] = __builtin_bit_cast(bf16x8, make_uint4(P[b][2 * u][0], P[b][2 * u][1], P[b][2 * u + 1][0], P[b][2 * u + 1][1]));
      if (SAVE) store_block_lines<(DIG_AB_NT & 1) != 0>(p.qkv + wave_row0 * (3 * KD) + h * 64, 3 * KD, P, smem + STG_OFF + wave * 2048, tid & 63);
    }
    __builtin_amdgcn_sched_barrier(0);
    select_source(false, 2 * KD + h * 64);
    zero();
    tick(I2{}, I0{}, std::integral_constant<int, 3 + C::E_BLK>{}, FALSE_{}, acc, no_pre);
    tick(I0{}, I1{}, std::integral_constant<int, 3 + C::E_BLK>{}, FALSE_{}, acc, no_pre);
    {
      const int tid = ab_opaque(tid0), hi = (tid >> 5) & 1;
      finish_block(acc, KD + h * 64, 1.0f, P, hi);
      unsigned char* kw = smem + K_OFF + wave * 4096 + (tid & 63) * 16;
#pragma unroll
      for (int b = 0; b < 2; ++b)
#pragma unroll
        for (int u = 0; u < 2; ++u)
          *reinterpret_cast<uint4*>(kw + (2 * b + u) * 1024) = make_uint4(P[b][2 * u][0], P[b][2 * u][1], P[b][2 * u + 1][0], P[b][2 * u + 1][1]);
      if (SAVE) store_block_lines<(DIG_AB_NT & 1) != 0>(p.qkv + wave_row0 * (3 * KD) + KD + h * 64, 3 * KD, P, smem + STG_OFF + wave * 2048, tid & 63);
    }
    __builtin_amdgcn_sched_barrier(0);
    select_source(h + 1 == NH, h + 1 == NH ? 0 : (h + 1) * 64);
    zero();
    tick(I1{}, I0{}, std::integral_constant<int, 3 + C::E_BLK>{}, FALSE_{}, acc, no_pre);
    tick(I2{}, I1{}, std::integral_constant<int, 3 + C::E_BLK>{}, FALSE_{}, acc, no_pre);
    {
      const int tid = ab_opaque(tid0), hi = (tid >> 5) & 1;
      finish_block(acc, 2 * KD + h * 64, 1.0f, P, hi);
      const int key = wave * 32 + (tid & 31);
      const int vw = V_OFF + key * 128 + 8 * hi + (swz(key) << 4);
#pragma unroll
      for (int b = 0; b < 2; ++b)
#pragma unroll
        for (int g = 0; g < 4; ++g) *reinterpret_cast<uint2*>(smem + (vw ^ ((4 * b + g) << 4))) = make_uint2(P[b][g][0], P[b][g][1]);
      if (SAVE) store_block_lines<(DIG_AB_NT & 1) != 0>(p.qkv + wave_row0 * (3 * KD) + 2 * KD + h * 64, 3 * KD, P, smem + STG_OFF + wave * 2048, tid & 63);
    }
    ab_wait_lgkm0();
    __builtin_amdgcn_s_barrier();
    asm volatile("" ::: "memory");
    __builtin_amdgcn_sched_barrier(0);

    DIG_AB_TS(3)
    const int tid = ab_opaque(tid0);
    const int lane = tid & 63, hi = lane >> 5;
    f32x16 O[2];
#pragma unroll
    for (int dt = 0; dt < 2; ++dt)
#pragma unroll
      for (int e = 0; e < 16; ++e) O[dt][e] = 0.f;
    float m = 0.f, l = 0.f;
    const unsigned char* Kl = smem + K_OFF + lane * 16;
    const int i16 = lane & 15;
    const int vt0 = V_OFF + u_addr(4 * hi + (i16 >> 2), ((lane >> 4) & 1) * 16 + (i16 & 3) * 4);
    auto vfrag = [&](int blk16, int dt) {
      typedef __attribute__((address_space(3))) bf16x4* lp;
      const int a = vt0 ^ (dt * 64);
      const bf16x4 lo = __builtin_amdgcn_ds_read_tr16_b64_v4i16((lp)(smem + a + blk16 * 2048));
      const bf16x4 h4 = __builtin_amdgcn_ds_read_tr16_b64_v4i16((lp)(smem + (a ^ 32) + 1024 + blk16 * 2048));
      return __builtin_shufflevector(lo, h4, 0, 1, 2, 3, 4, 5, 6, 7);
    };
    auto xhalf = [&](float v, float& lo, float& up) {
      const unsigned a = __float_as_uint(v);
      const auto r = __builtin_amdgcn_permlane32_swap(a, a, false, false);
      const unsigned r0 = r[0], r1 = r[1];
      lo = __uint_as_float(r0);
      up = __uint_as_float(r1);
    };
    auto xhalf_max = [&](float v) {
      float lo, up;
      xhalf(v, lo, up);
      return fmaxf(lo, up);
    };
    constexpr int TPP = 8 / NSPLIT;
#pragma unroll
    for (int part = 0; part < NSPLIT; ++part) {
      f32x16 S[TPP];
#pragma unroll
      for (int kt = 0; kt < TPP; ++kt)
#pragma unroll
        for (int e = 0; e < 16; ++e) S[kt][e] = 0.f;
      __builtin_amdgcn_sched_barrier(0);
      if (!(DIG_AB_ABL & 1)) {
#pragma unroll
        for (int bu = 0; bu < 4; ++bu)
#pragma unroll
          for (int kt = 0; kt < TPP; ++kt)
            S[kt] = __builtin_amdgcn_mfma_f32_32x32x16_bf16(*reinterpret_cast<const bf16x8*>(Kl + ((TPP * part + kt) * 4 + bu) * 1024), Qp[bu],
                                                            S[kt], 0, 0, 0);
      }
      __builtin_amdgcn_sched_barrier(0);
      float mx = S[0][0];
#pragma unroll
      for (int kt = 0; kt < TPP; ++kt)
#pragma unroll
        for (int e = 0; e < 16; ++e) mx = fmaxf(mx, S[kt][e]);
      mx = xhalf_max(mx);
      if (part == 0) {
        m = mx;
      } else {
        const float mn = fmaxf(m, mx);
        const float alpha = __expf(m - mn);
        m = mn;
        l *= alpha;
#pragma unroll
        for (int dt = 0; dt < 2; ++dt)
#pragma unroll
          for (int e = 0; e < 16; ++e) O[dt][e] *= alpha;
      }
      __builtin_amdgcn_sched_barrier(0);
#pragma unroll
      for (int kt = 0; kt < TPP; ++kt) {
        float la = 0.f, lb = 0.f;
#pragma unroll
        for (int e = 0; e < 16; e += 2) {
          const float pa = (DIG_AB_ABL & 8) ? S[kt][e] : __expf(S[kt][e] - m), pb = (DIG_AB_ABL & 8) ? S[kt][e + 1] : __expf(S[kt][e + 1] - m);
          S[kt][e] = pa; S[kt][e + 1] = pb;
          la += pa; lb += pb;
        }
        l += la + lb;
        asm volatile("" : "+v"(l));
        if (!(DIG_AB_ABL & 1)) {
#pragma unroll
          for (int u = 0; u < 2; ++u) {
            const bf16x8 v0 = vfrag((TPP * part + kt) * 2 + u, 0), v1 = vfrag((TPP * part + kt) * 2 + u, 1);
            const bf16x8 pf = pack8(S[kt], u);
            O[0] = __builtin_amdgcn_mfma_f32_32x32x16_bf16(v0, pf, O[0], 0, 0, 0);
            O[1] = __builtin_amdgcn_mfma_f32_32x32x16_bf16(v1, pf, O[1], 0, 0, 0);
          }
        } else {
#pragma unroll
          for (int e = 0; e < 16; ++e) asm volatile("" ::"v"(S[kt][e]));
        }
        __builtin_amdgcn_sched_barrier(0);
      }
    }
    {
      float lo, up;
      xhalf(l, lo, up);
      l = lo + up;
    }
    const float inv = 1.0f / l;
    {
      unsigned Pc[2][4][2];
#pragma unroll
      for (int dt = 0; dt < 2; ++dt)
#pragma unroll
        for (int g = 0; g < 4; ++g) {
          Pc[dt][g][0] = pack_bf2(O[dt][4 * g] * inv, O[dt][4 * g + 1] * inv);
          Pc[dt][g][1] = pack_bf2(O[dt][4 * g + 2] * inv, O[dt][4 * g + 3] * inv);
        }
      store_block_lines<(DIG_AB_NT & 4) != 0>(p.ctx + wave_row0 * KD + h * 64, KD, Pc, smem + STG_OFF + wave * 2048, lane);
    }
    if (SAVE && hi == 0 && !(DIG_AB_ABL & 4)) p.lse[((size_t)img * NH + h) * 256 + wave * 32 + (lane & 31)] = m + __logf(l);
    __builtin_amdgcn_sched_barrier(0);
  };

  head(TRUE_{}, 0);
  for (int h = 1; h < NH; ++h) head(FALSE_{}, h);

  DIG_AB_TS(4)
  asm volatile("s_waitcnt vmcnt(0)" ::: "memory");
  load_rows(p.ctx);
  asm volatile("s_waitcnt vmcnt(0)" ::: "memory");
  auto triple = [&](auto first_tag, int jb0) {
    constexpr bool FIRST = decltype(first_tag)::value;
    using I0 = std::integral_constant<int, 0>;
    using I1 = std::integral_constant<int, 1>;
    using I2 = std::integral_constant<int, 2>;
    auto block = [&](auto s0_tag, auto s1_tag, auto eprev_tag, int jb) {
      constexpr int EPREV = decltype(eprev_tag)::value;
      select_source(true, jb < 5 ? (jb + 1) * 64 : 0);
      f32x16 acc[2];
#pragma unroll
      for (int b = 0; b < 2; ++b)
#pragma unroll
        for (int e = 0; e < 16; ++e) acc[b][e] = 0.f;
      auto res_pre = [&]() {
        const int tid = ab_opaque(tid0), lane = tid & 63;
        const unsigned rbase = ((unsigned)img * 256u + (unsigned)(wave * 32 + (lane >> 3))) * KD;
#pragma unroll
        for (int k = 0; k < 4; ++k)
          dma16(lds0 + (unsigned)(K_OFF + wave * 4096 + k * 1024),
                (unsigned)((rbase + 8 * ((lane & 7) ^ (4 * (k & 1) + (lane >> 4)))) * 2) + (unsigned)(k * 8 * KD * 2), rRes, (unsigned)(jb * 64 * 2));
      };
      tick(s0_tag, I0{}, std::integral_constant<int, 3 + EPREV>{}, TRUE_{}, acc, res_pre);
      tick(s1_tag, I1{}, std::integral_constant<int, 3 + EPREV + C::E_RES>{}, FALSE_{}, acc, no_pre);
      ab_wait_vm<6>();
      const int tid = ab_opaque(tid0), rr = tid & 31, hi = (tid >> 5) & 1;
      unsigned P[2][4][2];
      const float* bv = reinterpret_cast<const float*>(smem + VEC_OFF + (3 * KD + jb * 64 + 4 * hi) * 4);
      const int ro = K_OFF + wave * 4096 + rr * 128 + hi * 8 + (((rr >> 1) & 7) << 4);
#pragma unroll
      for (int b = 0; b < 2; ++b)
#pragma unroll
        for (int g = 0; g < 4; ++g) {
          const f32x4 b4 = *reinterpret_cast<const f32x4*>(bv + 32 * b + 8 * g);
          const uint2 rw = *reinterpret_cast<const uint2*>(smem + (ro ^ ((4 * b + g) << 4)));
          const float v0 = (acc[b][4 * g] + b4[0]) + bf2f((bf16_t)(rw.x & 0xffff));
          const float v1 = (acc[b][4 * g + 1] + b4[1]) + bf2f((bf16_t)(rw.x >> 16));
          const float v2 = (acc[b][4 * g + 2] + b4[2]) + bf2f((bf16_t)(rw.y & 0xffff));
          const float v3 = (acc[b][4 * g + 3] + b4[3]) + bf2f((bf16_t)(rw.y >> 16));
          P[b][g][0] = pack_bf2(v0, v1);
          P[b][g][1] = pack_bf2(v2, v3);
        }
      store_block_lines<(DIG_AB_NT & 2) != 0>(p.out + wave_row0 * KD + jb * 64, KD, P, smem + STG_OFF + wave * 2048, tid & 63);
      __builtin_amdgcn_sched_barrier(0);
    };
    block(I0{}, I1{}, std::integral_constant<int, FIRST ? 0 : C::E_OUT>{}, jb0);
    block(I2{}, I0{}, std::integral_constant<int, C::E_OUT>{}, jb0 + 1);
    block(I1{}, I2{}, std::integral_constant<int, C::E_OUT>{}, jb0 + 2);
  };
  triple(TRUE_{}, 0);
  triple(FALSE_{}, 3);
  asm volatile("s_waitcnt vmcnt(0)" ::: "memory");
  DIG_AB_TS_END()
}

}


extern "C" int dig_attn_block_fwd(const void* ln1, const void* x, const void* qkv_w, const float* qkv_b, const void* proj_w, const float* proj_b,
                                  void* qkv, void* ctx, float* lse, void* x_mid, int n_img, int heads, int embed_dim, float scale,
                                  hipStream_t stream) {
  if (int rc = dig_rules::attn_block_fwd(ln1, x, qkv_w, qkv_b, proj_w, proj_b, qkv, ctx, lse, x_mid, n_img, heads, embed_dim, scale)) return rc;
  const size_t qb = (size_t)n_img * 256 * 3 * KD * 2;
  AbParams p;
  p.X = (const bf16_t*)ln1; p.resid = (const bf16_t*)x; p.Wqkv = (const bf16_t*)qkv_w; p.bqkv = qkv_b; p.Wp = (const bf16_t*)proj_w; p.bp = proj_b;
  p.qkv = (bf16_t*)qkv; p.ctx = (bf16_t*)ctx; p.lse = lse; p.out = (bf16_t*)x_mid; p.scale = scale;
  p.x_bytes = (unsigned)((size_t)n_img * 256 * KD * 2);
  static bool attr[DIG_MAX_DEVICES] = {};
  const int dev = dig_device();
  if (!attr[dev]) {
    if (hipFuncSetAttribute(reinterpret_cast<const void*>(&attn_block_kernel<false, DIG_AB_NSPLIT>), hipFuncAttributeMaxDynamicSharedMemorySize, LDS_BYTES) != hipSuccess ||
        hipFuncSetAttribute(reinterpret_cast<const void*>(&attn_block_kernel<true, DIG_AB_NSPLIT>), hipFuncAttributeMaxDynamicSharedMemorySize, LDS_BYTES) != hipSuccess)
      return DIG_ERR_LAUNCH;
    attr[dev] = true;
  }
  if (qkv) dig_launch(attn_block_kernel<true, DIG_AB_NSPLIT>, dim3(n_img), dim3(512), LDS_BYTES, stream, p);
  else dig_launch(attn_block_kernel<false, DIG_AB_NSPLIT>, dim3(n_img), dim3(512), LDS_BYTES, stream, p);
  return dig_check_launch();
}
```

### dig_amd/csrc/encoder_block.inc

```

#define DIG_BLOCK_TRY(call) do { const int rc_ = (call); if (rc_) return rc_; } while (0)

extern "C" int dig_encoder_block_fwd(const dig_block_fwd_t* b, hipStream_t stream) {
  if (!b || b->rows <= 0 || b->D <= 0 || b->F <= 0 || b->n_img <= 0 || b->heads <= 0 || b->rows != b->n_img * 256) return -1;
  if (!b->x || !b->ln1 || !b->qkv || !b->ctx || !b->lse || !b->x_mid || !b->out) return -1;
  if (b->save && (!b->ln2 || !b->mu2 || !b->rs2 || !b->pre || !b->act)) return -1;
  if (b->next_n1_g && (!b->nln || (b->save && (!b->nmu || !b->nrs)))) return -1;
  const int D = b->D, R = b->rows;
  if (b->fuse_attn && dig_attn_block_supported(b->heads, D)) {
    DIG_BLOCK_TRY(dig_attn_block_fwd(b->ln1, b->x, b->qkv_w, b->qkv_b, b->proj_w, b->proj_b, b->save ? b->qkv : nullptr, b->ctx,
                                     b->save ? b->lse : nullptr, b->x_mid, b->n_img, b->heads, D, b->scale, stream));
  } else {
    DIG_BLOCK_TRY(dig_gemm_bf16(b->ln1, b->qkv_w, b->qkv, R, 3 * D, D, D, D, 3 * D, 0, 0, 0, b->qkv_b, nullptr, 0, nullptr, 0, b->scale, D, 0, 1, 0, 0,
                                b->tile_qkv, nullptr, stream));
    DIG_BLOCK_TRY(dig_attn_fwd(b->qkv, b->ctx, b->lse, b->n_img, b->heads, D, stream));
    DIG_BLOCK_TRY(dig_gemm_bf16(b->ctx, b->proj_w, b->x_mid, R, D, D, D, D, D, 0, 0, 0, b->proj_b, b->x, D, nullptr, 0, 1.0f, 0, 0, 1, 0, 0,
                                b->tile_proj, nullptr, stream));
  }
  return dig_mlp_chain_fwd_ln(b->x_mid, b->x_mid, b->n2_g, b->n2_b, b->eps, b->save ? b->ln2 : nullptr, b->save ? b->mu2 : nullptr,
                              b->save ? b->rs2 : nullptr, b->fc1_w, b->fc1_b, b->fc2_w, b->fc2_b, b->out, b->save ? b->pre : nullptr,
                              b->save ? b->act : nullptr, b->next_n1_g, b->next_n1_b, b->next_n1_g ? b->nln : nullptr,
                              (b->next_n1_g && b->save) ? b->nmu : nullptr, (b->next_n1_g && b->save) ? b->nrs : nullptr, R, D, b->F, stream);
}

extern "C" int dig_encoder_block_bwd(const dig_block_bwd_t* b, hipStream_t stream) {
  if (!b || b->rows <= 0 || b->D <= 0 || b->F <= 0 || b->n_img <= 0 || b->rows != b->n_img * 256) return -1;
  if (!b->dy || !b->dln2 || !b->dpre || !b->dctx || !b->dqkv || !b->bparts || !b->ws1 || !b->ws2 || !b->qs || !b->vs) return -1;
  if (!b->wg_probs || (!b->wg_defer && (!b->wg_map || !b->wg_slabs || (b->wg_fold_n > 0 && (!b->wg_fold_probs || !b->wg_fold_slabs))))) return -1;
  const int D = b->D, F = b->F, R = b->rows;
  dig_wgrad_prob_t* q = b->wg_probs;
  auto prob = [&](int k, const void* dy, int out_dim, const void* x, int in_dim, float* dw) {
    if (b->wg_trans[k]) q[k] = dig_wgrad_prob_t{x, dy, dw, in_dim, out_dim, in_dim, in_dim, out_dim, 1};
    else                q[k] = dig_wgrad_prob_t{dy, x, dw, out_dim, in_dim, in_dim, out_dim, in_dim, 0};
  };
  prob(0, b->dy, D, b->act, F, b->g_fc2_w);
  const bool proj_in = b->fuse_ln2 && b->projt;
  if (b->fuse_ln2) {
    DIG_BLOCK_TRY(dig_mlp_chain_bwd_ln_proj(b->dy, b->w2t, b->pre, b->w1t, b->dpre, b->x_mid, b->n2_g, b->mu2, b->rs2, b->dln2, b->bparts, b->ws2,
                                            proj_in ? b->projt : nullptr, proj_in ? b->dctx : nullptr, R, D, F, stream));
    prob(1, b->dpre, F, b->ln2, D, b->g_fc1_w);
  } else {
    DIG_BLOCK_TRY(dig_mlp_chain_bwd(b->dy, b->w2t, b->pre, b->w1t, b->dpre, b->dln2, b->bparts, R, D, F, stream));
    prob(1, b->dpre, F, b->ln2, D, b->g_fc1_w);
    DIG_BLOCK_TRY(dig_layernorm_bwd_partials(b->dln2, b->x_mid, b->n2_g, b->n2_b, b->mu2, b->rs2, b->dy, b->dln2, b->ws2, R, D, 0, stream));
  }
  prob(2, b->dln2, D, b->ctx, D, b->g_proj_w);
  const bool proj_attn = !proj_in && b->attn_proj && b->proj_wt && (D & 127) == 0 && D <= 512 && D == b->heads * 64;
  if (!proj_in && !proj_attn) {
    if (b->tile_direct && b->proj_wt)
      DIG_BLOCK_TRY(dig_gemm_bf16(b->dln2, b->proj_wt, b->dctx, R, D, D, D, D, D, 0, 0, 0, nullptr, nullptr, 0, nullptr, 0, 1.0f, 0, 0, 1, 0, 0,
                                  b->tile_direct, nullptr, stream));
    else
      DIG_BLOCK_TRY(dig_gemm_bf16(b->dln2, b->proj_w, b->dctx, R, D, D, D, D, D, 0, 1, 0, nullptr, nullptr, 0, nullptr, 0, 1.0f, 0, 0, 1, 0, 0,
                                  b->tile_dgrad, nullptr, stream));
  }
  if (proj_attn)
    DIG_BLOCK_TRY(dig_attn_bwd_proj(b->qkv, b->ctx, b->dln2, b->proj_wt, b->lse, b->dqkv, b->n_img, b->heads, D, b->scale, b->qs, b->vs, stream));
  else
    DIG_BLOCK_TRY(dig_attn_bwd(b->qkv, b->ctx, b->dctx, b->lse, b->dqkv, b->n_img, b->heads, D, b->scale, b->qs, b->vs, stream));
  prob(3, b->dqkv, 3 * D, b->ln1, D, b->g_qkv_w);
  if (!b->wg_defer)
    DIG_BLOCK_TRY(dig_wgrad_group(q, 4, b->wg_fold_probs, b->wg_fold_n, R, b->wg_splits, b->wg_map, b->wg_n_wg, b->wg_slabs, b->wg_fold_slabs,
                                  b->wg_fold_n > 0 ? b->wg_fold_splits : 1, b->wg_fn, b->wg_wa, stream));
  if (b->tile_direct && b->qkv_wt)
    DIG_BLOCK_TRY(dig_gemm_bf16(b->dqkv, b->qkv_wt, b->dctx, R, D, 3 * D, 3 * D, 3 * D, D, 0, 0, 0, nullptr, nullptr, 0, nullptr, 0, 1.0f, 0, 0, 1, 0, 0,
                                b->tile_direct, nullptr, stream));
  else
    DIG_BLOCK_TRY(dig_gemm_bf16(b->dqkv, b->qkv_w, b->dctx, R, D, 3 * D, 3 * D, D, D, 0, 1, 0, nullptr, nullptr, 0, nullptr, 0, 1.0f, 0, 0, 1, 0, 0,
                                b->tile_dgrad, nullptr, stream));
  DIG_BLOCK_TRY(dig_layernorm_bwd_partials(b->dctx, b->x, b->n1_g, b->n1_b, b->mu1, b->rs1, b->dln2, b->dctx, b->ws1, R, D, 0, stream));
  if (b->defer_red) return 0;
  DIG_BLOCK_TRY(DIG_BLOCK_HANDOVER(stream, b->side));
  hipStream_t sd = b->side;
  DIG_BLOCK_TRY(dig_colsum_partials(b->bparts, dig_mlp_chain_colsum_rows(R), F, b->g_fc1_b, sd));
  if (b->fuse_ln2) DIG_BLOCK_TRY(dig_layernorm_bwd_finalize_parts(b->ws2, dig_mlp_chain_ln_parts(R), D, b->g_n2_g, b->g_n2_b, b->g_fc2_b, sd));
  else DIG_BLOCK_TRY(dig_layernorm_bwd_finalize(b->ws2, R, D, b->g_n2_g, b->g_n2_b, b->g_fc2_b, sd));
  DIG_BLOCK_TRY(dig_colsum_partials(b->qs, b->n_img, D, b->g_q_b, sd));
  DIG_BLOCK_TRY(dig_colsum_partials(b->vs, b->n_img, D, b->g_v_b, sd));
  return dig_layernorm_bwd_finalize(b->ws1, R, D, b->g_n1_g, b->g_n1_b, b->g_proj_b, sd);
}
```

### dig_amd/encoder_blocks.py

```python
from typing import NamedTuple

import torch

from . import ops

BF16 = torch.bfloat16
_NO_DROP = (None, None, None)


class Plan(NamedTuple):
    chain: bool = False
    chain_ln: bool = False
    attn_block: bool = False
    chain_bwd: bool = False
    chain_every: int = 1
    chain_phase: int = 0
    chain_lnb: bool = False
    chain_proj: bool = False
    attn_proj: bool = False
    direct: bool = False
    fused_qv: bool = False
    grouping: str = "off"
    inline: bool = False
    side_each: bool = False
    batch_reduce: bool = False
    red_defer: bool = False


def _tensors(s):
    return s if isinstance(s, tuple) else s.tensors()


def _no_mark(name, dev):
    pass


def forward(plan, blocks, x, n_img, heads, eps, save, drops=None, tail=(None, None), frozen=0):
    R, D = x.shape
    scale = (D // heads) ** -0.5
    saved, nxt, last = [], None, len(blocks) - 1
    for i, blk in enumerate(blocks):
        keep = save and i >= frozen
        ln1, mu1, rs1 = nxt if nxt is not None else ops.layernorm_fwd(x, blk["norm1.weight"], blk["norm1.bias"], eps)
        nxt = None
        da, dp, dm = (drops[i] or _NO_DROP) if drops is not None else _NO_DROP
        if plan.attn_block and da is None and dp is None:
            x_mid, ctx, qkv, lse = ops.attn_block_fwd(ln1, x, blk["attn.qkv.weight"], blk["qkv_bias"], blk["attn.proj.weight"],
                                                      blk["attn.proj.bias"], n_img, heads, D, scale, save=keep)
        else:
            qkv = ops.linear_fwd(ln1, blk["attn.qkv.weight"], bias=blk["qkv_bias"], alpha=scale, alpha_cols=D)
            ctx, lse = ops.attn_fwd(qkv, n_img, heads, D, drop=da)
            x_mid = ops.linear_fwd(ctx, blk["attn.proj.weight"], bias=blk["attn.proj.bias"], resid=x, drop=dp)
        if plan.chain_ln:
            ng, nb = (blocks[i + 1]["norm1.weight"], blocks[i + 1]["norm1.bias"]) if i < last else tail
            if i < frozen:
                ng = nb = None
            r = ops.mlp_chain_fwd_ln(x_mid, blk["norm2.weight"], blk["norm2.bias"], eps, blk["mlp.fc1.weight"], blk["mlp.fc1.bias"],
                                     blk["mlp.fc2.weight"], blk["mlp.fc2.bias"], ng, nb, save=keep, drop=dm)
            x_out, ln2, mu2, rs2, pre, act = r["out"], r["ln"], r["ln_mean"], r["ln_rstd"], r["pre"], r["act"]
            if ng is not None:
                nxt = (r["nln"], r["nln_mean"], r["nln_rstd"])
        else:
            ln2, mu2, rs2 = ops.layernorm_fwd(x_mid, blk["norm2.weight"], blk["norm2.bias"], eps)
            if plan.chain and dm is None:
                r = ops.mlp_chain_fwd(ln2, blk["mlp.fc1.weight"], blk["mlp.fc1.bias"], blk["mlp.fc2.weight"], blk["mlp.fc2.bias"], x_mid, save=keep)
                x_out, pre, act = r if keep else (r, None, None)
            else:
                pre = torch.empty((R, blk["mlp.fc1.weight"].shape[0]), device=x.device, dtype=BF16) if keep else None
                act = ops.linear_fwd(ln2, blk["mlp.fc1.weight"], bias=blk["mlp.fc1.bias"], act=1, pre=pre)
                x_out = ops.linear_fwd(act, blk["mlp.fc2.weight"], bias=blk["mlp.fc2.bias"], resid=x_mid, drop=dm)
        if save:
            saved.append((x, ln1, mu1, rs1, qkv, ctx, lse, x_mid, ln2, mu2, rs2, pre, act) if keep else None)
        x = x_out
    return x, saved, nxt


def backward(plan, blocks, saved, dx, wT, n_img, heads, on_side, first=0, drops=None, rows=None, block_done=None, grad_ready=None,
             mark=_no_mark):
    D = dx.shape[1]
    scale = (D // heads) ** -0.5
    dev = dx.device
    grp = ops.WgradGroup(dev) if plan.grouping != "off" else None
    batch_side = grp is not None and not plan.side_each
    vred = ops.GradReduceBatch() if (plan.red_defer and grp) else None
    prev_block = None

    def launch_group(*tensors):
        if plan.inline:
            grp.launch()
        else:
            on_side(grp.launch, *tensors)

    for i in reversed(range(first, len(blocks))):
        blk, g = blocks[i], blocks[i]["g"]
        x, ln1, mu1, rs1, qkv, ctx, lse, x_mid, ln2, mu2, rs2, pre, act = _tensors(saved[i])
        saved[i] = None
        chain = plan.chain_bwd and (i % plan.chain_every == plan.chain_phase % plan.chain_every)
        if rows is not None:
            x, ln1, mu1, rs1, qkv, ctx, x_mid, ln2, mu2, rs2, pre, act = (t[:rows] for t in (x, ln1, mu1, rs1, qkv, ctx, x_mid, ln2, mu2, rs2, pre, act))
            lse = lse[:n_img * heads]
        red = ops.GradReduceBatch() if plan.batch_reduce else None
        wg = red.wgrad if red else ops.linear_wgrad
        csum = red.colsum_partials if red else ops.colsum_partials
        held = []
        late, late_t = [], []

        def side_later(fn, *tensors):
            if batch_side:
                late.append(fn)
                late_t.extend(tensors)
            else:
                on_side(fn, *tensors)
        if grp:
            def wg(dy_, x_, dw_):
                if not grp.add(dy_, x_, dw_):
                    raise RuntimeError("grouped weight gradient: a problem of this block does not fit the group's plan")
                held.extend((dy_, x_))
        da, dp, dm = (drops[i] or _NO_DROP) if drops is not None else _NO_DROP
        dz = ops.dropout_apply(dx, dm)
        if dm is not None:
            on_side(lambda dz=dz: ops.colsum(dz, g["mlp.fc2.bias"]), dz)
        if grp:
            wg(dz, act, g["mlp.fc2.weight"])
        else:
            on_side(lambda dz=dz: wg(dz, act, g["mlp.fc2.weight"]), dz, act)
        dctx = lnp = None
        if chain:
            w2t, w1t = wT[i][0], wT[i][1]
            if dm is not None or red is not None or not plan.chain_lnb:
                dln2, dact, bparts = ops.mlp_chain_bwd(dz, w2t, pre, w1t)
            elif plan.chain_proj:
                dx_mid, dact, bparts, lnp, dctx = ops.mlp_chain_bwd_ln(dx, w2t, pre, w1t, x_mid, blk["norm2.weight"], mu2, rs2, projt=wT[i][2])
                dln2 = dx_mid
            else:
                dx_mid, dact, bparts, lnp = ops.mlp_chain_bwd_ln(dx, w2t, pre, w1t, x_mid, blk["norm2.weight"], mu2, rs2)
                dln2 = dx_mid
            mark("blk: fused MLP backward", dev)
        else:
            dact, bparts = ops.linear_dgrad(dz, blk["mlp.fc2.weight"], gelu_pre=pre, colsum=True)
            dln2 = None
        if grp:
            wg(dact, ln2, g["mlp.fc1.weight"])
            if vred:
                vred.colsum_partials(bparts, g["mlp.fc1.bias"])
            else:
                side_later(lambda: csum(bparts, g["mlp.fc1.bias"]), bparts)
            if plan.grouping == "pair":
                launch_group(*held)
        elif plan.side_each:
            on_side(lambda: csum(bparts, g["mlp.fc1.bias"]), bparts)
            on_side(lambda: wg(dact, ln2, g["mlp.fc1.weight"]), dact, ln2)
        else:
            on_side(lambda: (wg(dact, ln2, g["mlp.fc1.weight"]), csum(bparts, g["mlp.fc1.bias"])), dact, ln2, bparts)
        if dln2 is None:
            dln2 = ops.dgrad_direct(dact, wT[i][1]) if plan.direct else None
            if dln2 is None:
                dln2 = ops.linear_dgrad(dact, blk["mlp.fc1.weight"])
        if lnp is not None and vred:
            vred.layernorm_finalize_parts(lnp, g["norm2.weight"], g["norm2.bias"], g["mlp.fc2.bias"])
        elif lnp is not None:
            side_later(lambda lnp=lnp, g=g: ops.layernorm_finalize_parts(lnp, g["norm2.weight"], g["norm2.bias"], g["mlp.fc2.bias"]), lnp)
        else:
            fc2_b = g["mlp.fc2.bias"] if dm is None else None
            dx_mid, fin2, ws2 = ops.layernorm_bwd(dln2, x_mid, blk["norm2.weight"], blk["norm2.bias"], mu2, rs2, dx, g["norm2.weight"],
                                                  g["norm2.bias"], out=dln2, dres_colsum=fc2_b, defer=True)
            if red or vred:
                (red or vred).layernorm_finalize(ws2, x_mid.shape[0], D, g["norm2.weight"], g["norm2.bias"], fc2_b)
            else:
                side_later(fin2, ws2)
        dzp = ops.dropout_apply(dx_mid, dp)
        if dp is not None:
            on_side(lambda dzp=dzp: ops.colsum(dzp, g["attn.proj.bias"]), dzp)
        if grp:
            wg(dzp, ctx, g["attn.proj.weight"])
        else:
            on_side(lambda dzp=dzp: wg(dzp, ctx, g["attn.proj.weight"]), dzp, ctx)
        mark("blk: LayerNorm backward (norm2)", dev)
        proj_attn = dctx is None and plan.attn_proj and plan.fused_qv and dp is None and da is None
        if dctx is None and not proj_attn:
            dctx = ops.dgrad_direct(dzp, wT[i][2]) if plan.direct else None
            if dctx is None:
                dctx = ops.linear_dgrad(dzp, blk["attn.proj.weight"])
        mark("blk: proj data gradient", dev)
        gb = g["qkv_bias"]
        if plan.fused_qv:
            if proj_attn:
                dqkv, qs, vs = ops.attn_bwd_proj(qkv, ctx, dzp, wT[i][2], lse, n_img, heads, D, scale, bias_sums=True)
                dctx = None
            else:
                dqkv, qs, vs = ops.attn_bwd(qkv, ctx, dctx, lse, n_img, heads, D, scale, bias_sums=True, drop=da)
            mark("blk: attention backward", dev)
            if grp:
                wg(dqkv, ln1, g["attn.qkv.weight"])
                launch_group(*held)
                mark("blk: grouped weight gradients", dev)
                if vred:
                    vred.colsum_partials(qs, gb[:D]); vred.colsum_partials(vs, gb[2 * D:])
                else:
                    side_later(lambda: (csum(qs, gb[:D]), csum(vs, gb[2 * D:])), qs, vs)
            else:
                on_side(lambda: (wg(dqkv, ln1, g["attn.qkv.weight"]), csum(qs, gb[:D]), csum(vs, gb[2 * D:])), dqkv, ln1, qs, vs)
        else:
            dqkv = ops.attn_bwd(qkv, ctx, dctx, lse, n_img, heads, D, scale, drop=da)
            if grp:
                wg(dqkv, ln1, g["attn.qkv.weight"])
                launch_group(*held)
                side_later(lambda: (ops.colsum(dqkv, gb[:D], cols=D), ops.colsum(dqkv[:, 2 * D:], gb[2 * D:], cols=D)), dqkv)
            else:
# ... 56 lines not shown
```

### dig_amd/engine_core.py

```python
import ctypes
import functools
import itertools
import os
import weakref
from typing import Optional, Tuple

import torch

from . import block_calls as BC
from . import encoder_blocks as EB
from . import ops
from .arena import enc_block_views
from .parallel import LOCAL, LocalComm, bn_backward, bn_forward

BF16, F32 = torch.bfloat16, torch.float32
FWD_MODE = os.environ.get("DIG_FWD_MODE", "flip")
CHAIN_BWD_EVERY = max(1, int(os.environ.get("DIG_CHAIN_BWD_EVERY", "1")))
CHAIN_BWD_PHASE = int(os.environ.get("DIG_CHAIN_BWD_PHASE", "0"))
BATCH_REDUCE = os.environ.get("DIG_BATCH_REDUCE", "0") == "1"
FUSED_QV_BIAS_SUMS = os.environ.get("DIG_FUSED_QV_BIAS", "1") != "0"
WGRAD_GROUPING = os.environ.get("DIG_WGRAD_GROUPING", "block")
WGRAD_INLINE = os.environ.get("DIG_WGRAD_INLINE", "1") == "1"
WGRAD_DEFER = os.environ.get("DIG_WGRAD_DEFER", "auto").strip().lower()
if WGRAD_DEFER not in ("auto", "0", "1"):
    raise ValueError(f"DIG_WGRAD_DEFER={WGRAD_DEFER!r}: one of auto, 0, 1")
RED_DEFER = os.environ.get("DIG_RED_DEFER", "1") != "0"
BWD_SINGLE_STREAM = os.environ.get("DIG_BWD_SINGLE", "0") == "1"


PHASE_MARKS = None


def _mark(name, dev):
    if PHASE_MARKS is not None:
        ev = torch.cuda.Event(enable_timing=True)
        ev.record(torch.cuda.current_stream(dev))
        PHASE_MARKS.append((name, ev))


ONLINE_HEADS = ("online", "pix_projector", "patch_extractor", "encoder_projection_layer", "predictor")
MOMENTUM_HEADS = ("momentum", "pix_projector_m", "momentum_patch_extractor", "momentum_projection_layer", None)


class _EncWeights:

    def __init__(self, model, prefix, arena):
        f32, g32 = model._f32, model._g32 if arena == "online" else {}
        self.blocks = enc_block_views(model.specs, prefix, model.depth, model.D, model._flat[arena], model.shadow(arena),
                                      model._flat["grad"] if g32 else None)
        self.pe_w = f32[prefix + "patch_embed.proj.weight"].view(model.D, 48)
        self.pe_b = f32[prefix + "patch_embed.proj.bias"]
        self.mask_token = f32[prefix + "mask_token"].view(model.D)
        if g32:
            self.g_pe_w = g32[prefix + "patch_embed.proj.weight"].view(model.D, 48)
            self.g_pe_b = g32[prefix + "patch_embed.proj.bias"]
            self.g_mask_token = g32[prefix + "mask_token"].view(model.D)


def _weights(model):
    cache = getattr(model, "_wcache", None)
    mom = getattr(model, "use_moco_target", True)
    if cache is None or cache[0] != model._views_version or model._shadow.get("online") is None or (mom and model._shadow.get("momentum") is None):
        model.shadow("online")
        if mom:
            model.shadow("momentum")
        model._w16 = None
        cache = (model._views_version, _EncWeights(model, "encoder.", "online"),
                 _EncWeights(model, "momentum_encoder.", "momentum") if mom else None)
        model._wcache = cache
    return cache[1], cache[2]


class _Step:
    def __init__(self, model):
        self._keep = []
        self._keep_marks = []
        self.m = model
        self.comm = model.comm or LOCAL

    def _path_specs(self, plan, site_off):
        from . import dropout as DR
        M = self.m
        out = []
        for i, p in enumerate(M.dpr):
            if not p:
                out.append(None)
                continue
            out.append((plan.spec(0, 0.0, path_site=DR.enc_site(i + site_off, 2), path_p=p, rows_per_sample=M.N),
                        plan.spec(0, 0.0, path_site=DR.enc_site(i + site_off, 4), path_p=p, rows_per_sample=M.N)))
        return out

    def encoder_forward(self, ew, images, aug, mask_u8, save, views=2, path=None):
        M = self.m
        B, D, H, N = images.shape[0], M.D, M.H, M.N
        R = views * B * N
        x = torch.empty((R, D), device=images.device, dtype=BF16)
        for half, im in enumerate((images, aug)[:views]):
            ops.L.call("dig_patch_embed_fwd", ops.L.ptr(im), ops.L.ptr(ew.pe_w), ops.L.ptr(ew.pe_b),
                       ops.L.ptr(mask_u8[half * B:(half + 1) * B]), ops.L.ptr(ew.mask_token), ops.L.ptr(M._pos),
                       ops.L.ptr(x[half * B * N:(half + 1) * B * N]), B, M.gh, M.gw, D, ops.L.stream())
        chain = ops.mlp_chain_supported(D, M.F, R) and bool(ops.MLP_CHAIN_MASK & (2 if save else 1))
        plan = EB.Plan(chain=chain, chain_ln=chain and ops.MLP_CHAIN_LN and M.F <= 2048,
                       attn_block=ops.attn_block_supported(H, D, B if views == 1 else None))
        if plan.chain_ln and ops.BLOCK_CALLS and D == H * 64 and path is None:
            return BC.forward(ew.blocks, x, views * B, H, M.F, M.ln_eps, save, fuse_attn=plan.attn_block)
        drops = [ds and (None, ds[0], ds[1]) for ds in path] if path is not None else None
        x, saved, _ = EB.forward(plan, ew.blocks, x, views * B, H, M.ln_eps, save, drops=drops)
        return x, saved

    def mlp_weight_transposes(self, ew, fresh=False):
        tr = self.m.transposed_weight_table() if hasattr(self.m, "transposed_weight_table") else None
        self.head_wT = {}
        if tr is not None and fresh:
            self.head_wT = tr[6]
            return tr[4]
        outs = tr[4] if tr is not None else None
        w2t = ops.transpose_bf16_multi([b["mlp.fc2.weight"] for b in ew.blocks], [o[0] for o in outs] if outs else None)
        w1t = ops.transpose_bf16_multi([b["mlp.fc1.weight"] for b in ew.blocks], [o[1] for o in outs] if outs else None)
        projt = ops.transpose_bf16_multi([b["attn.proj.weight"] for b in ew.blocks], [o[2] for o in outs] if outs else None)
        qkvt = ops.transpose_bf16_multi([b["attn.qkv.weight"] for b in ew.blocks], [o[3] for o in outs] if outs else None)
        if tr is not None:
            w16 = self.m._w("online")
            for name, dst in tr[6].items():
                ops.transpose_bf16(w16[name], dst)
            self.head_wT = tr[6]
        return list(zip(w2t, w1t, projt, qkvt))

    def _backward_transposes(self, ew, training, rows, fresh):
        M = self.m
        if training and ((ops.mlp_chain_supported(M.D, M.F, rows) and (ops.MLP_CHAIN_MASK & 4)) or (ops.DGRAD_DIRECT and rows >= 8192)):
            return self.mlp_weight_transposes(ew, fresh)
        return None

    def _streams(self, dev):
        M = self.m
        main = torch.cuda.current_stream(dev)
        side = M._bwd_side_stream(dev) if (getattr(M, "overlap_streams", True) and not BWD_SINGLE_STREAM) else main
        return main, side

    def _on_side(self, dev, fn, *tensors):
        main, side = self._streams(dev)
        if side is main:
            fn()
            return
        side.wait_stream(main)
        with torch.cuda.stream(side):
            fn()
        self._keep.extend(tensors)

    def _mark_kept(self, dev):
        main, side = self._streams(dev)
        if side is main or not self._keep:
            return
        ev = torch.cuda.Event()
        ev.record(side)
        self._keep_marks.append((ev, len(self._keep)))

    def _release_kept(self, dev, lag=2):
        main, side = self._streams(dev)
        while len(self._keep_marks) > lag:
            ev, n = self._keep_marks.pop(0)
            main.wait_event(ev)
            del self._keep[:n]
            self._keep_marks = [(e, m - n) for e, m in self._keep_marks]

    def _grad_ready(self, dev, key):
        main, side = self._streams(dev)
        if side is not main and (self.comm.world > 1 or getattr(self.comm, "world_override", False)):
            side.wait_stream(main)
            with torch.cuda.stream(side):
                self.comm.grad_ready(self.m, key)
        else:
            self.comm.grad_ready(self.m, key)

    def _backward_plan(self, chain, have_wT, rows, path):
        D, Fh = self.m.D, self.m.F
        grouped = (ops.WGRAD_GROUP and WGRAD_GROUPING != "off" and
                   all(ops.wgrad_group_route(o, i_, rows) is not None for o, i_ in ((Fh, D), (D, Fh), (3 * D, D), (D, D))))
        return EB.Plan(chain_bwd=chain, chain_every=CHAIN_BWD_EVERY, chain_phase=CHAIN_BWD_PHASE, chain_lnb=ops.MLP_CHAIN_LNB,
                       chain_proj=ops.MLP_CHAIN_PROJ, direct=have_wT, fused_qv=FUSED_QV_BIAS_SUMS,
                       attn_proj=bool(ops.ATTN_BWD_PROJ and FUSED_QV_BIAS_SUMS and have_wT and ops.attn_bwd_proj_supported(D)
                                      and not ops.attn_bwd_mode()),
                       grouping=WGRAD_GROUPING if grouped else "off", inline=WGRAD_INLINE, batch_reduce=BATCH_REDUCE,
                       red_defer=bool(RED_DEFER and self.comm is LOCAL and path is None and not BATCH_REDUCE and PHASE_MARKS is None))

    def _block_call_plan(self, dev, n_img, R):
        M, local = self.m, self.comm is LOCAL
        kept = M.depth * ops.block_bwd_layout(R, M.D, M.F, n_img)[1]
        defer = WGRAD_DEFER == "1" or (WGRAD_DEFER == "auto" and local and BC.defer_fits(M.__dict__.setdefault("_defer_fits_cache", {}), dev, kept))
        return BC.Plan(defer=defer, red_defer=bool(RED_DEFER and defer and local and ops.MLP_CHAIN_LNB and M.depth * 9 <= ops.COLSUM_MAX_SEGS),
                       tile_direct=ops.dgrad_direct_tile_code(R, M.D),
                       attn_proj=bool(ops.ATTN_BWD_PROJ and ops.attn_bwd_proj_supported(M.D) and not ops.attn_bwd_mode()),
                       fuse_ln2=bool(ops.MLP_CHAIN_LNB), chain_proj=bool(ops.MLP_CHAIN_LNB and ops.MLP_CHAIN_PROJ))

    @staticmethod
    def _takes_block_calls(plan, path, saved, dx):
        return (ops.BLOCK_CALLS and plan.grouping == "block" and plan.inline and plan.chain_bwd and plan.chain_every == 1 and plan.fused_qv
                and path is None and not plan.batch_reduce and PHASE_MARKS is None and all(isinstance(s_, BC._BlockSaved) for s_ in saved)
                and dx.is_contiguous())

    def encoder_backward(self, ew, saved, dx, images, aug, mask_u8, views=2):
        M = self.m
        B, D, H, N = images.shape[0], M.D, M.H, M.N
        dev = dx.device
        main, side = self._streams(dev)
        n_img, R = views * B, views * B * N
        chain = ops.mlp_chain_supported(D, M.F, R) and bool(ops.MLP_CHAIN_MASK & 4)
        wT = getattr(self, "wT", None)
        if chain and wT is None:
            wT = self.mlp_weight_transposes(ew)
        elif wT is not None:
            for pair_ in wT:
                for t in pair_:
                    t.record_stream(main)
        path = getattr(self, "path_on", None)
        plan = self._backward_plan(chain, wT is not None, R, path)
        grad_ready = functools.partial(self._grad_ready, dev)

        def block_done():
            self._mark_kept(dev)
            self._release_kept(dev)
        wplan = ops.wgrad_block_plan(dev, R, D, M.F) if self._takes_block_calls(plan, path, saved, dx) else None
        if wplan is not None:
            dx = BC.backward(self._block_call_plan(dev, n_img, R), ew.blocks, saved, dx, wT, wplan, n_img, H, M.F,
                             ctypes.c_void_p(side.cuda_stream), keep=self._keep.append if side is not main else None,
                             block_done=block_done, grad_ready=grad_ready)
        else:
            drops = [ds and (None, ds[0], ds[1]) for ds in path] if path is not None else None
            dx = EB.backward(plan, ew.blocks, saved, dx, wT, n_img, H, functools.partial(self._on_side, dev), drops=drops, rows=R if views == 1 else None,
                             block_done=block_done, grad_ready=grad_ready, mark=_mark)
        for half, im in enumerate((images, aug)[:views]):
            ops.patch_embed_bwd_mfma(dx[half * B * N:(half + 1) * B * N], im, mask_u8[half * B:(half + 1) * B], ew.g_pe_w, ew.g_pe_b,
                                     ew.g_mask_token, D, M.gh, M.gw)
        main.wait_stream(side)
        self.comm.grad_ready(M, "encoder.embed")

    def mlp_forward(self, stacks):
        M = self.m
        dims = M.mlps[stacks[0][1]]
        assert all(M.mlps[pre] == dims for _, pre, _, _ in stacks)
        xs = [x for x, _, _, _ in stacks]
        saved = [[] for _ in stacks]
        for l in range(len(dims)):
            last = l == len(dims) - 1
            hs = [ops.linear_fwd(x, M._w(arena)[f"{pre}.{3 * l}.weight"]) for x, (_, pre, arena, _) in zip(xs, stacks)]
            outs = bn_forward(self, hs, [f"{pre}.{3 * l + 1}" for _, pre, _, _ in stacks], relu=not last, affine=not last)
            for k, (y, mean, rstd) in enumerate(outs):
                if stacks[k][3]:
                    saved[k].append((xs[k], hs[k], mean, rstd))
                xs[k] = y
        self.saved_heads.update({pre: kept for (_, pre, _, save), kept in zip(stacks, saved) if save})
        return xs

    def mlp_backward(self, dy, pre, need_dx=True, dx_out=None):
        M = self.m
        dims, saved = M.mlps[pre], self.saved_heads[pre]
        w16, g32 = M._w("online"), M._g32
        for l in reversed(range(len(dims))):
# ... 372 lines not shown
```

### dig_amd/ops.py

```python
import ctypes
import os
from collections import namedtuple

import torch

from . import _lib as L
from . import scratch

cf = ctypes.c_float
cll = ctypes.c_longlong
BF16 = torch.bfloat16
F32 = torch.float32

OUT_BF16, OUT_F32, OUT_F32_PARTIAL = 0, 1, 2
GEMM_BK_FWD, GEMM_BK_BWD = 64, 32
SLAB_FLOOR, PARTIAL_FLOOR, LOSS_FLOOR, GROUP_FLOOR = 1 << 22, 1 << 20, 4096, 1 << 24
_workspace = _workspace2 = None


def gemm(A, B, I, J, R, *, ta=False, tb=False, out=None, out_kind=OUT_BF16, bias=None, resid=None, pre=None, alpha=1.0,
         alpha_cols=0, act=0, splits=1, ldc=None, a_rows=0, b_rows=0, bk=0, colsum_partials=None, drop=None):
    if out is None:
        out = torch.empty((I, J), device=A.device, dtype=BF16 if out_kind == OUT_BF16 else F32)
    if not bk:
# ... 292 lines not shown
        n = L.query("dig_layernorm_bwd_parts", rows)
        for k, out in enumerate((dgamma, dbeta, dcolsum)):
            if out is not None:
                self._vec(ws[k * D:], out, 3 * D, n, D)

    def layernorm_finalize_parts(self, ln_parts, dgamma, dbeta, dcolsum):
        n, _, D = ln_parts.shape
        flat = ln_parts.view(-1)
        for k, out in enumerate((dgamma, dbeta, dcolsum)):
            if out is not None:
                self._vec(flat[k * D:], out, 3 * D, n, D)

    def _vec(self, parts, out, stride, n_parts, C):
        if len(self.vecs) == COLSUM_MAX_SEGS:
            self._flush_vecs()
        self.vecs.append((parts, out, stride, n_parts, C))

    def tensors(self):
        return [v[0] for v in self.vecs]

    def _flush_vecs(self):
        if self.vecs:
            segs = (_ColsumSeg * len(self.vecs))(*[_ColsumSeg(p.data_ptr(), o.data_ptr(), st, n, C) for p, o, st, n, C in self.vecs])
            L.call("dig_colsum_partials_multi", segs, len(self.vecs), L.stream())
            self.vecs = []

    def flush(self):
        if self.slabs:
            segs = (_ReduceSeg * len(self.slabs))(*[_ReduceSeg(w.data_ptr(), d.data_ptr(), n, sp, 0) for w, d, n, sp in self.slabs])
            L.call("dig_reduce_partials_multi", segs, len(self.slabs), L.stream())
            self.slabs, self.off = [], 0
        self._flush_vecs()


WGRAD_ASSIGN = os.environ.get("DIG_WGRAD_ASSIGN", "1") != "0"


def linear_wgrad(dy, x, dw, rows=None, assign=False):
    rows = dy.shape[0] if rows is None else rows
    I, J = dw.shape
    if assign and WGRAD_ASSIGN and rows <= 2048 and dw.is_contiguous() and ((I + 127) // 128) * ((J + 127) // 128) >= 64:
        gemm(dy, x, I, J, rows, ta=True, tb=True, out=dw, out_kind=OUT_F32_PARTIAL, splits=1, ldc=J, bk=32)
        return
    wgrad(dy, x, dw, I, J, rows)


WGRAD_GROUP = os.environ.get("DIG_WGRAD_GROUP", "1") != "0"
WGRAD_GROUP_WA = int(os.environ.get("DIG_WGRAD_WA", "2"))
WGRAD_GROUP_SLOTS = int(os.environ.get("DIG_WGRAD_SLOTS", "0")) or 512 // WGRAD_GROUP_WA
_wg_plans = {}


class _WgProb(ctypes.Structure):
    _fields_ = [("A", ctypes.c_void_p), ("B", ctypes.c_void_p), ("out", ctypes.c_void_p), ("lda", ctypes.c_int), ("ldb", ctypes.c_int),
                ("ldo", ctypes.c_int), ("I", ctypes.c_int), ("J", ctypes.c_int), ("trans_out", ctypes.c_int)]


def wgrad_group_route(out_dim, in_dim, rows, fn=None):
    cands = ((0, out_dim, in_dim), (1, in_dim, out_dim))
    if out_dim < in_dim:
        cands = cands[::-1]
    for trans, wide, narrow in cands:
        if narrow <= 512 and L.query("dig_wgrad_group_supported", int(wide), int(narrow), int(rows)):
            f = L.query("dig_wgrad_group_fn", int(narrow))
            if fn is None or f == fn:
                return trans, f
    return None


class WgradGroup:

    def __init__(self, dev):
        self.dev, self.cur, self.pending, self.set, self.fn, self.rows = dev, [], None, 0, None, None

    def add(self, dy, x, dw, rows=None):
        rows = dy.shape[0] if rows is None else rows
        r = wgrad_group_route(dw.shape[0], dw.shape[1], rows, self.fn) if WGRAD_GROUP else None
        if r is None or len(self.cur) == 6 or (self.rows not in (None, rows)) or dw.stride(1) != 1:
            return False
        if rows * max(dy.stride(0), x.stride(0)) * 2 >= 1 << 32:
            return False
        trans, self.fn = r
        self.rows = rows
        A, B = (x, dy) if trans else (dy, x)
        self.cur.append((A, B, dw, trans))
        return True

    def _plan(self, tiles):
        key = (tuple(tiles), self.rows, WGRAD_GROUP_SLOTS, WGRAD_GROUP_WA, str(self.dev))
        pl = _wg_plans.get(key)
        if pl is None:
            tp = (ctypes.c_int * len(tiles))(*tiles)
            cap = 8 * max(WGRAD_GROUP_SLOTS, sum(tiles))
            buf = (ctypes.c_uint * cap)()
            sp = ctypes.c_int(0)
            n = L.query("dig_wgrad_group_plan", tp, len(tiles), int(self.rows), WGRAD_GROUP_SLOTS, ctypes.byref(sp), buf, cap)
            if n <= 0:
                L.check(n or -1, "dig_wgrad_group_plan")
            import numpy as np
            m = torch.from_numpy(np.frombuffer(buf, dtype=np.uint32, count=n).view(np.int32).copy())
            pl = _wg_plans[key] = (sp.value, n, m.to(self.dev))
        return pl

    def _structs(self, items):
        arr = (_WgProb * max(len(items), 1))()
        for k, (A, B, dw, trans) in enumerate(items):
            J = dw.shape[0] if trans else dw.shape[1]
            I = dw.shape[1] if trans else dw.shape[0]
            arr[k] = _WgProb(A.data_ptr() if A is not None else None, B.data_ptr() if B is not None else None, dw.data_ptr(),
                             A.stride(0) if A is not None else 0, B.stride(0) if B is not None else 0, dw.stride(0), I, J, trans)
        return arr

    def next_slabs(self, nbytes):
        slabs = scratch.get(f"wgrad_group{self.set}", self.dev, (nbytes + 3) // 4, floor=GROUP_FLOOR)
        self.set ^= 1
        return slabs

    def call(self, probs, n, fold_probs, fold_n, splits, wmap, n_wg, slabs, fold_slabs, fold_splits):
        L.call("dig_wgrad_group", probs, n, fold_probs, fold_n, int(self.rows), splits, L.ptr(wmap), n_wg, L.ptr(slabs), L.ptr(fold_slabs), fold_splits,
               self.fn, WGRAD_GROUP_WA, L.stream())

    def fold(self, probs, n, slabs, splits):
        self.call(None, 0, probs, n, 1, None, WGRAD_GROUP_SLOTS, None, slabs, splits)

    def launch(self):
        if not self.cur and self.pending is None:
            return
        fn, wa = self.fn, WGRAD_GROUP_WA
        tiles = [L.query("dig_wgrad_group_tiles", int(dw.shape[1] if t else dw.shape[0]), int(dw.shape[0] if t else dw.shape[1]), fn, wa)
                 for _, _, dw, t in self.cur]
        if self.cur:
            splits, n_wg, wmap = self._plan(tiles)
            slabs = self.next_slabs(sum(tiles) * splits * 128 * wa * 128 * fn * 4)
        else:
            splits, n_wg, wmap, slabs = 1, WGRAD_GROUP_SLOTS, None, None
        items, fold_slabs, fold_splits = self.pending or ([], None, 1)
        self.call(self._structs(self.cur), len(self.cur), self._structs(items) if items else None, len(items), splits, wmap, n_wg, slabs,
                  fold_slabs, fold_splits)
        self.pending = ([(None, None, dw, t) for _, _, dw, t in self.cur], slabs, splits) if self.cur else None
        self.cur = []

    def flush(self):
        assert not self.cur, "launch() the queued problems first"
        self.launch()


BLOCK_CALLS = os.environ.get("DIG_BLOCK_CALLS", "1") != "0"
_VP, _FP, _I, _F = ctypes.c_void_p, ctypes.c_void_p, ctypes.c_int, ctypes.c_float


class BlockFwd(ctypes.Structure):
    _fields_ = ([(k, _I) for k in ("n_img", "heads", "D", "F", "rows", "save", "tile_qkv", "tile_proj", "fuse_attn", "reserved0")] + [("eps", _F), ("scale", _F)] +
                [(k, _VP) for k in ("qkv_w", "qkv_b", "proj_w", "proj_b", "n2_g", "n2_b", "fc1_w", "fc1_b", "fc2_w", "fc2_b", "next_n1_g", "next_n1_b",
                                    "x", "ln1", "qkv", "ctx", "lse", "x_mid", "ln2", "mu2", "rs2", "pre", "act", "out", "nln", "nmu", "nrs")])


class BlockBwd(ctypes.Structure):
    _fields_ = ([(k, _I) for k in ("n_img", "heads", "D", "F", "rows", "tile_dgrad", "tile_direct")] + [("scale", _F)] +
                [(k, _VP) for k in ("qkv_w", "proj_w", "w2t", "w1t", "projt", "proj_wt", "qkv_wt", "n1_g", "n1_b", "n2_g", "n2_b",
                                    "g_n1_g", "g_n1_b", "g_qkv_w", "g_q_b", "g_v_b", "g_proj_w", "g_proj_b", "g_n2_g", "g_n2_b", "g_fc1_w", "g_fc1_b",
                                    "g_fc2_w", "g_fc2_b",
                                    "x", "ln1", "mu1", "rs1", "qkv", "ctx", "lse", "x_mid", "ln2", "mu2", "rs2", "pre", "act", "dy",
                                    "dln2", "dpre", "dctx", "dqkv", "bparts", "ws1", "ws2", "qs", "vs")] +
                [(k, _I) for k in ("wg_fn", "wg_wa", "wg_splits", "wg_n_wg", "wg_fold_n", "wg_fold_splits")] + [("wg_trans", _I * 4)] +
                [("wg_defer", _I), ("fuse_ln2", _I), ("attn_proj", _I), ("defer_red", _I)] +
                [(k, _VP) for k in ("wg_map", "wg_slabs", "wg_fold_slabs", "wg_probs", "wg_fold_probs", "side")])


def _round_up(n, m):
    return (n + m - 1) // m * m


_block_layouts = {}


def block_fwd_layout(rows, D, Fh, n_img, heads, save):
    key = ("f", rows, D, Fh, n_img, heads, bool(save))
    lay = _block_layouts.get(key)
    if lay is None:
        off, n16, n32 = {}, 0, 0
        for name, cols in (("qkv", 3 * D), ("ctx", D), ("x_mid", D), ("out", D), ("nln", D)) + ((("ln2", D), ("pre", Fh), ("act", Fh)) if save else ()):
            off[name] = n16
            n16 += _round_up(rows * cols * 2, 256)
        for name, n in (("lse", n_img * heads * 256),) + ((("mu2", rows), ("rs2", rows), ("nmu", rows), ("nrs", rows)) if save else ()):
            off[name] = n32
            n32 += _round_up(n * 4, 256)
        lay = _block_layouts[key] = (off, n16, n32)
    return lay


def block_bwd_layout(rows, D, Fh, n_img):
    key = ("b", rows, D, Fh, n_img)
    lay = _block_layouts.get(key)
    if lay is None:
        off, n16, n32 = {}, 0, 0
        for name, cols in (("dln2", D), ("dpre", Fh), ("dctx", D), ("dqkv", 3 * D)):
            off[name] = n16
            n16 += _round_up(rows * cols * 2, 256)
        parts = L.query("dig_layernorm_bwd_parts", rows) * 3 * D
        parts2 = max(parts, L.query("dig_mlp_chain_ln_parts", rows) * 3 * D)
        for name, n in (("bparts", L.query("dig_mlp_chain_colsum_rows", rows) * Fh), ("ws1", parts), ("ws2", parts2), ("qs", n_img * D), ("vs", n_img * D)):
            off[name] = n32
            n32 += _round_up(n * 4, 256)
        lay = _block_layouts[key] = (off, n16, n32)
    return lay


WgradBlockPlan = namedtuple("WgradBlockPlan", "fn wa splits n_wg wmap trans group slab_bytes")


def wgrad_block_plan(dev, rows, D, Fh):
    grp = WgradGroup(dev)
    grp.rows = rows
    trans, tiles = [], []
    for out_dim, in_dim in ((D, Fh), (Fh, D), (D, D), (3 * D, D)):
        r = wgrad_group_route(out_dim, in_dim, rows, grp.fn) if WGRAD_GROUP else None
        if r is None:
            return None
        t, grp.fn = r
        trans.append(t)
        tiles.append(L.query("dig_wgrad_group_tiles", int(in_dim if t else out_dim), int(out_dim if t else in_dim), grp.fn, WGRAD_GROUP_WA))
    splits, n_wg, wmap = grp._plan(tiles)
    return WgradBlockPlan(grp.fn, WGRAD_GROUP_WA, splits, n_wg, wmap, trans, grp, sum(tiles) * splits * 128 * WGRAD_GROUP_WA * 128 * grp.fn * 4)


def colsum(x, out, rows=None, cols=None):
    rows = x.shape[0] if rows is None else rows
    cols = x.shape[1] if cols is None else cols
    ws = scratch.get("partials", x.device, scratch.floats("dig_colsum_workspace_bytes", rows, cols), floor=PARTIAL_FLOOR)
    L.call("dig_colsum", L.ptr(x), L.ptr(out), L.ptr(ws), rows, cols, x.stride(0), L.stream())


def layernorm_fwd(x, gamma, beta, eps, gelu=False):
    rows, D = x.shape
    y = torch.empty_like(x)
    mean = torch.empty(rows, device=x.device, dtype=F32)
    rstd = torch.empty(rows, device=x.device, dtype=F32)
    L.call("dig_layernorm_fwd", L.ptr(x), L.ptr(gamma), L.ptr(beta), L.ptr(y), L.ptr(mean), L.ptr(rstd), rows, D, cf(eps),
           int(gelu), L.stream())
    return y, mean, rstd


def layernorm_bwd(dy, x, gamma, beta, mean, rstd, dres, dgamma, dbeta, gelu=False, out=None, dres_colsum=None, defer=False):
    rows, D = x.shape
    dx = torch.empty_like(x) if out is None else out
    if not defer:
        ws = scratch.get("partials", x.device, scratch.floats("dig_layernorm_bwd_workspace_bytes", rows, D), floor=PARTIAL_FLOOR)
        L.call("dig_layernorm_bwd", L.ptr(dy), L.ptr(x), L.ptr(gamma), L.ptr(beta), L.ptr(mean), L.ptr(rstd), L.ptr(dres), L.ptr(dx),
               L.ptr(dgamma), L.ptr(dbeta), L.ptr(dres_colsum), L.ptr(ws), rows, D, int(gelu), L.stream())
        return dx
    ws = torch.empty(L.query("dig_layernorm_bwd_parts", rows) * 3 * D, device=x.device, dtype=F32)
    L.call("dig_layernorm_bwd_partials", L.ptr(dy), L.ptr(x), L.ptr(gamma), L.ptr(beta), L.ptr(mean), L.ptr(rstd), L.ptr(dres),
           L.ptr(dx), L.ptr(ws), rows, D, int(gelu), L.stream())

    def finish():
        L.call("dig_layernorm_bwd_finalize", L.ptr(ws), rows, D, L.ptr(dgamma), L.ptr(dbeta), L.ptr(dres_colsum), L.stream())
    return dx, finish, ws


def attn_fwd(qkv, n_img, heads, D, drop=None, q_rows=256):
    ctx = torch.empty((qkv.shape[0], D), device=qkv.device, dtype=BF16)
    lse = torch.empty((n_img * heads, 256), device=qkv.device, dtype=F32)
    L.call("dig_attn_fwd_dropout", L.ptr(qkv), L.ptr(ctx), L.ptr(lse), n_img, heads, D, ctypes.byref(drop) if drop is not None else None,
           q_rows, L.stream())
    return ctx, lse


def seq_attn_fwd(q, k, v, B, heads, Lq, Lk, dk, scale, causal=False, lens=None, drop=None):
    out = torch.empty((B * Lq, heads * dk), device=q.device, dtype=BF16)
    lse = torch.empty((B, heads, Lq), device=q.device, dtype=F32)
    L.call("dig_seq_attn_fwd_hd", L.ptr(q), q.stride(0), L.ptr(k), k.stride(0), L.ptr(v), v.stride(0), L.ptr(out), heads * dk, L.ptr(lse), B, heads,
           Lq, Lk, cf(scale), int(causal), L.ptr(lens), ctypes.byref(drop) if drop is not None else None, dk, L.stream())
    return out, lse


def seq_attn_bwd(q, k, v, dout, lse, dq, dk_, dv, B, heads, Lq, Lk, dk, scale, causal=False, lens=None, drop=None):
    L.call("dig_seq_attn_bwd_hd", L.ptr(q), q.stride(0), L.ptr(k), k.stride(0), L.ptr(v), v.stride(0), L.ptr(dout), dout.stride(0), L.ptr(lse),
           L.ptr(dq), dq.stride(0), L.ptr(dk_), dk_.stride(0), L.ptr(dv), dv.stride(0), B, heads, Lq, Lk, cf(scale), int(causal), L.ptr(lens),
           ctypes.byref(drop) if drop is not None else None, dk, L.stream())


def tcv_attn_fwd(film, u, vk, mem, lnc_g, lnc_b, S, Lq, N, heads, slots_per_mem=1, drop=None, wmean=None, eps=1e-5):
    d = vk.shape[1]
    c = torch.empty((S * Lq, heads * d), device=u.device, dtype=BF16)
    lse = torch.empty((S * Lq, heads), device=u.device, dtype=F32)
    L.call("dig_tcv_attn_fwd", L.ptr(film), L.ptr(u), L.ptr(vk), L.ptr(mem), L.ptr(lnc_g), L.ptr(lnc_b), cf(eps), L.ptr(c), L.ptr(lse), L.ptr(wmean),
           S, Lq, N, heads, d, slots_per_mem, ctypes.byref(drop) if drop is not None else None, L.stream())
    return c, lse


def tcv_attn_bwd(film, u, vk, mem, lnc_g, lnc_b, c, lse, dc, dlnc_g, dlnc_b, S, Lq, N, heads, drop=None, eps=1e-5):
    d = vk.shape[1]
    du, dfilm, dvk, dmem = torch.empty_like(u), torch.empty_like(film), torch.empty_like(vk), torch.empty_like(mem)
    ws = scratch.get("slabs", u.device, scratch.floats("dig_tcv_attn_bwd_workspace_bytes", S, Lq, heads, d), floor=SLAB_FLOOR)
    L.call("dig_tcv_attn_bwd", L.ptr(film), L.ptr(u), L.ptr(vk), L.ptr(mem), L.ptr(lnc_g), L.ptr(lnc_b), cf(eps), L.ptr(c), L.ptr(lse), L.ptr(dc),
           L.ptr(du), L.ptr(dfilm), L.ptr(dvk), L.ptr(dmem), L.ptr(dlnc_g), L.ptr(dlnc_b), L.ptr(ws), S, Lq, N, heads, d, 1,
           ctypes.byref(drop) if drop is not None else None, L.stream())
    return du, dfilm, dvk, dmem


ATTN_BLOCK = os.environ.get("DIG_ATTN_BLOCK", "1") != "0"


ATTN_BLOCK_MIN_IMG = int(os.environ.get("DIG_ATTN_BLOCK_MIN_IMG", "160"))


def attn_block_supported(heads, D, n_img=None):
    return (ATTN_BLOCK and (n_img is None or n_img >= ATTN_BLOCK_MIN_IMG or n_img < 32)
            and bool(L.query("dig_attn_block_supported", int(heads), int(D))))


def attn_block_fwd(ln1, x, qkv_w, qkv_b, proj_w, proj_b, n_img, heads, D, scale, save=False):
    rows = ln1.shape[0]
    x_mid = torch.empty((rows, D), device=ln1.device, dtype=BF16)
    ctx = torch.empty((rows, D), device=ln1.device, dtype=BF16)
    qkv = torch.empty((rows, 3 * D), device=ln1.device, dtype=BF16) if save else None
    lse = torch.empty((n_img * heads, 256), device=ln1.device, dtype=F32) if save else None
    L.call("dig_attn_block_fwd", L.ptr(ln1), L.ptr(x), L.ptr(qkv_w), L.ptr(qkv_b), L.ptr(proj_w), L.ptr(proj_b), L.ptr(qkv), L.ptr(ctx),
           L.ptr(lse), L.ptr(x_mid), n_img, heads, D, cf(scale), L.stream())
    return x_mid, ctx, qkv, lse


def attn_bwd_mode(single_pass=None):
    return bool(L.query("dig_attn_bwd_mode", -1 if single_pass is None else int(bool(single_pass))))


if os.environ.get("DIG_ATTN_BWD_SP") in ("0", "1"):
    attn_bwd_mode(os.environ["DIG_ATTN_BWD_SP"] == "1")


def attn_bwd_store(mode=None):
    if mode is not None and mode not in (0, 1, 3):
        raise ValueError(f"attn_bwd_store: mode {mode!r} (one of 0, 1, 3)")
    return int(L.query("dig_attn_bwd_store", -1 if mode is None else int(mode)))


if os.environ.get("DIG_ATTN_BWD_STORE") is not None:
    attn_bwd_store(int(os.environ["DIG_ATTN_BWD_STORE"]))


def attn_bwd(qkv, ctx, dctx, lse, n_img, heads, D, scale, bias_sums=False, drop=None, q_rows=256):
    dqkv = torch.empty_like(qkv)
    qs = torch.empty((n_img, D), device=qkv.device, dtype=F32) if bias_sums else None
    vs = torch.empty((n_img, D), device=qkv.device, dtype=F32) if bias_sums else None
    L.call("dig_attn_bwd_dropout", L.ptr(qkv), L.ptr(ctx), L.ptr(dctx), L.ptr(lse), L.ptr(dqkv), n_img, heads, D, cf(scale), L.ptr(qs), L.ptr(vs),
           ctypes.byref(drop) if drop is not None else None, q_rows, L.stream())
    return (dqkv, qs, vs) if bias_sums else dqkv


def attn_bwd_proj(qkv, ctx, dy, projt, lse, n_img, heads, D, scale, bias_sums=False):
    dqkv = torch.empty_like(qkv)
    qs = torch.empty((n_img, D), device=qkv.device, dtype=F32) if bias_sums else None
    vs = torch.empty((n_img, D), device=qkv.device, dtype=F32) if bias_sums else None
    L.call("dig_attn_bwd_proj", L.ptr(qkv), L.ptr(ctx), L.ptr(dy), L.ptr(projt), L.ptr(lse), L.ptr(dqkv), n_img, heads, D, cf(scale), L.ptr(qs), L.ptr(vs),
           L.stream())
    return (dqkv, qs, vs) if bias_sums else dqkv


def attn_bwd_proj_supported(D):
    return D % 128 == 0 and D <= 512


def patch_embed_fwd(img, W, bias, mask_u8, mask_token, pos, D, gh, gw):
    n_img = img.shape[0]
    out = torch.empty((n_img * gh * gw, D), device=img.device, dtype=BF16)
    L.call("dig_patch_embed_fwd", L.ptr(img), L.ptr(W), L.ptr(bias), L.ptr(mask_u8), L.ptr(mask_token), L.ptr(pos), L.ptr(out),
           n_img, gh, gw, D, L.stream())
    return out


def patch_embed_bwd(dy, img, mask_u8, dW, dbias, dmask_token, D, gh, gw):
    L.call("dig_patch_embed_bwd", L.ptr(dy), L.ptr(img), L.ptr(mask_u8), L.ptr(dW), L.ptr(dbias), L.ptr(dmask_token),
           img.shape[0], gh, gw, D, L.stream())


def patch_embed_bwd_mfma(dy, img, mask_u8, dW, dbias, dmask_token, D, gh, gw):
    n_tok = img.shape[0] * gh * gw
    P = torch.empty((n_tok, 64), device=img.device, dtype=BF16)
    L.call("dig_patchify_bf16", L.ptr(img), L.ptr(mask_u8), L.ptr(P), img.shape[0], gh, gw, L.stream())
    wgrad(dy, P, dW, D, 48, n_tok)
    ws = scratch.get("partials", dy.device, 2 * scratch.floats("dig_colsum_workspace_bytes", n_tok, D), floor=PARTIAL_FLOOR)
    L.call("dig_colsum_masked", L.ptr(dy), L.ptr(mask_u8), L.ptr(dbias), L.ptr(dmask_token), L.ptr(ws), n_tok, D, L.stream())


def window_pool_fwd(x, out, n_img, gh, gw, nwin, D):
    L.call("dig_window_pool_fwd", L.ptr(x), L.ptr(out), int(out.dtype == F32), n_img, gh, gw, nwin, D, L.stream())


def window_pool_bwd(dpool, dx, n_img, gh, gw, nwin, D, accumulate):
    L.call("dig_window_pool_bwd", L.ptr(dpool), L.ptr(dx), n_img, gh, gw, nwin, D, int(accumulate), L.stream())


def im2col3x3(x, n_img, H, W, C):
    ldc = _round_up(9 * C, 64)
    col = torch.empty((n_img * H * W, ldc), device=x.device, dtype=BF16)
    L.call("dig_im2col3x3", L.ptr(x), L.ptr(col), n_img, H, W, C, ldc, L.stream())
    return col


def conv3x3_weight_flip(w, c_out, c_in):
    wt = torch.empty((c_in, c_out * 9), device=w.device, dtype=BF16)
    L.call("dig_conv3x3_weight_flip", L.ptr(w), L.ptr(wt), c_out, c_in, L.stream())
    return wt


def maxpool2x2_fwd(x, n_img, H, W, C):
    y = torch.empty((n_img * (H // 2) * (W // 2), C), device=x.device, dtype=BF16)
    idx = torch.empty((n_img * (H // 2) * (W // 2), C), device=x.device, dtype=torch.uint8)
    L.call("dig_maxpool2x2_fwd", L.ptr(x), L.ptr(y), L.ptr(idx), n_img, H, W, C, L.stream())
    return y, idx


def maxpool2x2_bwd(dy, idx, n_img, H, W, C):
    dx = torch.empty((n_img * H * W, C), device=dy.device, dtype=BF16)
    L.call("dig_maxpool2x2_bwd", L.ptr(dy), L.ptr(idx), L.ptr(dx), n_img, H, W, C, L.stream())
    return dx


_MASK_KINDS = {torch.bool: 0, torch.uint8: 0, torch.float32: 1, torch.float64: 2, torch.int32: 3, torch.int64: 4}


def mask_views_u8(mask_bvn, keep_views):
    kind = _MASK_KINDS.get(mask_bvn.dtype)
    if kind is None or mask_bvn.dim() != 3 or not mask_bvn.is_contiguous():
        return None
    B, V, N = mask_bvn.shape
    out = torch.empty((V * B, N), device=mask_bvn.device, dtype=torch.uint8)
    L.call("dig_mask_views_u8", L.ptr(mask_bvn), kind, B, V, N, int(keep_views), L.ptr(out), L.stream())
    return out


def mask_to_index(mask_u8, max_per_sample):
    B, N = mask_u8.shape
    idx = torch.zeros((B, max_per_sample), device=mask_u8.device, dtype=torch.int32)
    cnt = torch.empty((B,), device=mask_u8.device, dtype=torch.int32)
    L.call("dig_mask_to_index", L.ptr(mask_u8), L.ptr(idx), L.ptr(cnt), B, N, max_per_sample, L.stream())
    return idx, cnt


def gather_rows(src, idx, M, M_pad):
    D = src.shape[1]
    dst = torch.empty((M_pad, D), device=src.device, dtype=BF16)
    L.call("dig_gather_rows", L.ptr(src), L.ptr(idx), L.ptr(dst), M, M_pad, D, L.stream())
    return dst


def scatter_rows_add(src, idx, dst, M):
    L.call("dig_scatter_rows_add", L.ptr(src), L.ptr(idx), L.ptr(dst), M, src.shape[1], L.stream())


def mim_target(img, idx, M, gh, gw, normalize=False):
    tgt = torch.empty((M, 48), device=img.device, dtype=F32)
    L.call("dig_mim_target", L.ptr(img), L.ptr(idx), L.ptr(tgt), M, gh, gw, int(normalize), L.stream())
    return tgt


def mse_fwd_bwd(pred, ld_pred, target, M, C, gscale, loss, dpred, ld_dpred):
    ws = scratch.get("mse", pred.device, scratch.floats("dig_mse_workspace_bytes"), zero=True, floor=LOSS_FLOOR)
    L.call("dig_mse_fwd_bwd_ws", L.ptr(pred), ld_pred, L.ptr(target), M, C, cf(gscale), L.ptr(loss), L.ptr(dpred), ld_dpred, L.ptr(ws), L.stream())


def add_bf16(a, b, out):
    L.call("dig_add_bf16", L.ptr(a), L.ptr(b), L.ptr(out), cll(a.numel()), L.stream())


def gelu_bwd(dact, pre, out):
    L.call("dig_gelu_bwd", L.ptr(dact), L.ptr(pre), L.ptr(out), cll(dact.numel()), L.stream())


def bn_stats(x, sums):
# ... 172 lines not shown
```

### include/dig_block_types.h

```cpp
#ifndef DIG_BLOCK_TYPES_H
#define DIG_BLOCK_TYPES_H

typedef struct dig_wgrad_prob {
  const void* A; const void* B; float* out;
  int lda, ldb, ldo, I, J, trans_out;
} dig_wgrad_prob_t;

typedef struct dig_block_fwd {
  int n_img, heads, D, F, rows;
  int save;
  int tile_qkv, tile_proj;
  int fuse_attn;
  int reserved0;
  float eps, scale;
  const void* qkv_w; const float* qkv_b; const void* proj_w; const float* proj_b;
  const float* n2_g; const float* n2_b; const void* fc1_w; const float* fc1_b; const void* fc2_w; const float* fc2_b;
  const float* next_n1_g; const float* next_n1_b;
  const void* x; const void* ln1;
  void* qkv; void* ctx; float* lse; void* x_mid; void* ln2; float* mu2; float* rs2; void* pre; void* act;
  void* out; void* nln; float* nmu; float* nrs;
} dig_block_fwd_t;

typedef struct dig_block_bwd {
  int n_img, heads, D, F, rows;
  int tile_dgrad;
  int tile_direct;
  float scale;
  const void* qkv_w; const void* proj_w; const void* w2t; const void* w1t;
  const void* projt;
  const void* proj_wt; const void* qkv_wt;
  const float* n1_g; const float* n1_b; const float* n2_g; const float* n2_b;
  float* g_n1_g; float* g_n1_b; float* g_qkv_w; float* g_q_b; float* g_v_b; float* g_proj_w; float* g_proj_b;
  float* g_n2_g; float* g_n2_b; float* g_fc1_w; float* g_fc1_b; float* g_fc2_w; float* g_fc2_b;
  const void* x; const void* ln1; const float* mu1; const float* rs1; const void* qkv; const void* ctx; const float* lse;
  const void* x_mid; const void* ln2; const float* mu2; const float* rs2; const void* pre; const void* act;
  const void* dy;
  void* dln2; void* dpre; void* dctx; void* dqkv;
  float* bparts; float* ws1; float* ws2; float* qs; float* vs;
  int wg_fn, wg_wa, wg_splits, wg_n_wg, wg_fold_n, wg_fold_splits;
  int wg_trans[4];
  int wg_defer;
  int fuse_ln2;
  int attn_proj;
  int defer_red;
  const unsigned* wg_map; float* wg_slabs; const float* wg_fold_slabs;
  dig_wgrad_prob_t* wg_probs; const dig_wgrad_prob_t* wg_fold_probs;
  hipStream_t side;
} dig_block_bwd_t;

#endif
```

### include/dig_hip.h

```cpp
#ifndef DIG_HIP_H
#define DIG_HIP_H

#ifdef __cplusplus
extern "C" {
#endif

#ifndef __HIP_PLATFORM_AMD__
typedef struct ihipStream_t* hipStream_t;
#endif

#include "dig_aug_types.h"

#define DIG_OK 0
#define DIG_ERR_ARG (-1)
#define DIG_ERR_ALIGN (-2)
#define DIG_ERR_LAUNCH (-3)
#define DIG_ERR_UNSUPPORTED (-4)

#define DIG_GEMM_TILE_DEFAULT 0
#define DIG_GEMM_TILE_128x128_K32 32
#define DIG_GEMM_TILE_128x128_K64 64
#define DIG_GEMM_TILE_256x256 244
#define DIG_GEMM_TILE_256x192 264
#define DIG_GEMM_TILE_64x128 212
#define DIG_GEMM_TILE_128x64 221
#define DIG_GEMM_TILE_256x256_PERSISTENT 544
#define DIG_GEMM_TILE_256x192_PERSISTENT 564
int dig_gemm_bf16(const void* A, const void* B, void* C, int I, int J, int R, int lda, int ldb, int ldc, int trans_a,
                  int trans_b, int out_kind, const float* bias, const void* resid, int ldr, void* pre_act, int ldp, float alpha,
                  int alpha_cols, int act, int splits, int a_rows, int b_rows, int bk, float* colsum_partials,
                  hipStream_t stream);
int dig_gemm_effective_splits(int R, int splits);
int dig_reduce_partials(const float* partials, int splits, long long n, float* out, int accumulate, hipStream_t stream);
int dig_reduce_partials_bf16(const float* partials, int splits, long long n, void* out, hipStream_t stream);
#define DIG_REDUCE_MAX_SEGS 8
typedef struct dig_reduce_seg { const float* partials; float* out; long long n; int splits; int reserved; } dig_reduce_seg_t;
int dig_reduce_partials_multi(const dig_reduce_seg_t* segs, int n_segs, hipStream_t stream);

#define DIG_WGRAD_MAX_PROBS 6
#include "dig_block_types.h"
int dig_wgrad_group_supported(int I, int J, int R);
int dig_wgrad_group_fn(int J);
int dig_wgrad_group_rows_per_split(int R, int splits);
int dig_wgrad_group_effective_splits(int R, int splits);
long long dig_wgrad_group_slab_bytes(int total_tiles, int splits, int fn, int wa);
int dig_wgrad_group_tiles(int I, int J, int fn, int wa);
int dig_wgrad_group_plan(const int* tiles_per_prob, int n_probs, int R, int max_wg, int* splits_out, unsigned* map_out, int max_out);
int dig_wgrad_group(const dig_wgrad_prob_t* probs, int n_probs, const dig_wgrad_prob_t* fold_probs, int n_fold, int R, int splits,
                    const unsigned* wg_map, int n_wg, float* slabs, const float* fold_slabs, int fold_splits, int fn, int wa,
                    hipStream_t stream);

int dig_mlp_chain_supported(int D, int F);
int dig_mlp_chain_fwd(const void* x, const void* w1, const float* b1, const void* w2, const float* b2, const void* resid, void* out,
                      void* pre_out, void* act_out, int R, int D, int F, hipStream_t stream);
int dig_mlp_chain_fwd_ln(const void* x, const void* resid, const float* ln_g, const float* ln_b, float eps, void* ln_out, float* ln_mean,
                         float* ln_rstd, const void* w1, const float* b1, const void* w2, const float* b2, void* out, void* pre_out, void* act_out,
                         const float* nln_g, const float* nln_b, void* nln_out, float* nln_mean, float* nln_rstd, int R, int D, int F,
                         hipStream_t stream);
int dig_mlp_chain_bwd(const void* dy, const void* w2t, const void* pre, const void* w1t, void* dpre_out, void* dx_out,
                      float* colsum_partials, int R, int D, int F, hipStream_t stream);
int dig_mlp_chain_bwd_ln(const void* dy, const void* w2t, const void* pre, const void* w1t, void* dpre_out, const void* x_mid,
                         const float* ln_g, const float* ln_mean, const float* ln_rstd, void* dx_mid_out, float* colsum_partials,
                         float* ln_partials, int R, int D, int F, hipStream_t stream);
int dig_mlp_chain_bwd_ln_proj(const void* dy, const void* w2t, const void* pre, const void* w1t, void* dpre_out, const void* x_mid,
                              const float* ln_g, const float* ln_mean, const float* ln_rstd, void* dx_mid_out, float* colsum_partials,
                              float* ln_partials, const void* projt, void* dctx_out, int R, int D, int F, hipStream_t stream);
int dig_mlp_chain_colsum_rows(int R);
int dig_mlp_chain_ln_parts(int R);
int dig_transpose_bf16(const void* src, void* dst, int rows, int cols, hipStream_t stream);
int dig_transpose_bf16_multi(const void* const* srcs, void* const* dsts, int count, int rows, int cols, hipStream_t stream);

int dig_attn_fwd(const void* qkv, void* ctx, float* lse, int n_img, int heads, int embed_dim, hipStream_t stream);
int dig_attn_bwd(const void* qkv, const void* ctx, const void* dctx, const float* lse, void* dqkv, int n_img, int heads,
                 int embed_dim, float scale, float* q_colsum, float* v_colsum, hipStream_t stream);
int dig_attn_bwd_proj(const void* qkv, const void* ctx, const void* dy, const void* projt, const float* lse, void* dqkv, int n_img, int heads,
                      int embed_dim, float scale, float* q_colsum, float* v_colsum, hipStream_t stream);
int dig_attn_bwd_mode(int single_pass);
int dig_attn_bwd_store(int mode);

int dig_attn_block_supported(int heads, int embed_dim);
int dig_attn_block_fwd(const void* ln1, const void* x, const void* qkv_w, const float* qkv_b, const void* proj_w, const float* proj_b,
                       void* qkv, void* ctx, float* lse, void* x_mid, int n_img, int heads, int embed_dim, float scale,
                       hipStream_t stream);

int dig_layernorm_fwd(const void* x, const float* gamma, const float* beta, void* y, float* mean, float* rstd, int rows, int D,
                      float eps, int fuse_gelu, hipStream_t stream);
long long dig_layernorm_bwd_workspace_bytes(int rows, int D);
int dig_layernorm_bwd(const void* dy, const void* x, const float* gamma, const float* beta, const float* mean, const float* rstd,
                      const void* dres, void* dx, float* dgamma, float* dbeta, float* dcolsum, float* workspace, int rows, int D,
                      int fuse_gelu, hipStream_t stream);
int dig_layernorm_bwd_parts(int rows);
int dig_layernorm_bwd_partials(const void* dy, const void* x, const float* gamma, const float* beta, const float* mean,
                               const float* rstd, const void* dres, void* dx, float* workspace, int rows, int D, int fuse_gelu,
                               hipStream_t stream);
int dig_layernorm_bwd_finalize(const float* workspace, int rows, int D, float* dgamma, float* dbeta, float* dcolsum,
                               hipStream_t stream);
int dig_layernorm_bwd_finalize_parts(const float* workspace, int parts, int D, float* dgamma, float* dbeta, float* dcolsum,
                                     hipStream_t stream);

long long dig_bn_stats_workspace_bytes(int rows, int C);
int dig_bn_stats(const void* x, float* sums, float* workspace, int rows, int C, hipStream_t stream);
int dig_bn_fwd_apply(const void* x, const float* sums, float n_total, float eps, const float* gamma, const float* beta, int relu,
                     void* y, float* mean_out, float* rstd_out, int rows, int C, hipStream_t stream);
int dig_bn_update_running(const float* sums, float n_total, float momentum, float* running_mean, float* running_var, int C,
                          hipStream_t stream);
int dig_bn_fwd_apply_running(const void* x, const float* sums, float n_total, float eps, const float* gamma, const float* beta, int relu,
                             void* y, float* mean_out, float* rstd_out, float momentum, float* running_mean, float* running_var, int rows,
                             int C, hipStream_t stream);
int dig_bn_bwd_stats(const void* dy, const void* x, const float* mean, const float* rstd, const float* gamma, const float* beta,
                     int relu, float* sums, float* workspace, int rows, int C, hipStream_t stream);
int dig_bn_bwd_stats_acc(const void* dy, const void* x, const float* mean, const float* rstd, const float* gamma, const float* beta,
                         int relu, float* sums, float* dbeta_acc, float* dgamma_acc, float* workspace, int rows, int C, hipStream_t stream);
int dig_bn_fused_supported(int rows, int C);
int dig_bn_fwd_fused(const void* x, float eps, const float* gamma, const float* beta, int relu, void* y, float* mean_out, float* rstd_out,
                     float momentum, float* running_mean, float* running_var, int rows, int C, hipStream_t stream);
int dig_bn_bwd_fused(const void* dy, const void* x, const float* mean, const float* rstd, const float* gamma, const float* beta, int relu,
                     float* dbeta_acc, float* dgamma_acc, void* dx, int rows, int C, hipStream_t stream);
int dig_bn_bwd_apply(const void* dy, const void* x, const float* mean, const float* rstd, const float* gamma, const float* beta,
                     int relu, const float* sums, float n_total, void* dx, int rows, int C, hipStream_t stream);

int dig_patch_embed_fwd(const float* img, const float* W, const float* bias, const unsigned char* mask, const float* mask_token,
                        const float* pos, void* out, int n_img, int gh, int gw, int D, hipStream_t stream);
int dig_patch_embed_bwd(const void* dy, const float* img, const unsigned char* mask, float* dW, float* dbias, float* dmask_token,
                        int n_img, int gh, int gw, int D, hipStream_t stream);
int dig_patchify_bf16(const float* img, const unsigned char* mask, void* out, int n_img, int gh, int gw, hipStream_t stream);
int dig_colsum_masked(const void* x, const unsigned char* mask, float* out_unmasked, float* out_masked, float* workspace,
                      int rows, int C, hipStream_t stream);

int dig_window_pool_fwd(const void* x, void* out, int out_is_f32, int n_img, int gh, int gw, int nwin, int D, hipStream_t stream);
int dig_window_pool_bwd(const void* dpool, void* dx, int n_img, int gh, int gw, int nwin, int D, int accumulate, hipStream_t stream);

int dig_im2col3x3(const void* x, void* col, int n_img, int H, int W, int C, int ldc, hipStream_t stream);
int dig_conv3x3_weight_flip(const void* w, void* wt, int c_out, int c_in, hipStream_t stream);
int dig_maxpool2x2_fwd(const void* x, void* y, unsigned char* idx, int n_img, int H, int W, int C, hipStream_t stream);
int dig_maxpool2x2_bwd(const void* dy, const unsigned char* idx, void* dx, int n_img, int H, int W, int C, hipStream_t stream);

int dig_mask_views_u8(const void* mask, int elem_kind, int B, int V, int N, int keep_views, unsigned char* out, hipStream_t stream);
int dig_mask_to_index(const unsigned char* mask, int* idx, int* count, int B, int N, int max_per_sample, hipStream_t stream);
int dig_gather_rows(const void* src, const int* idx, void* dst, int M, int M_pad, int D, hipStream_t stream);
int dig_scatter_rows_add(const void* src, const int* idx, void* dst, int M, int D, hipStream_t stream);
int dig_mim_target(const float* img, const int* idx, float* target, int M, int gh, int gw, int normalize , hipStream_t stream);
int dig_mse_fwd_bwd(const float* pred, int ld_pred, const float* target, int M, int C, float gscale, float* loss, void* dpred,
                    int ld_dpred, hipStream_t stream);

int dig_l2norm_fwd(const float* x, float* y, float* inv_norm, int n, int C, float eps, hipStream_t stream);
int dig_l2norm_bwd(const float* dy, const float* y, const float* inv_norm, float* dx, int n, int C, hipStream_t stream);
int dig_sgemm(const float* A, const float* B, float* C, int I, int J, int R, int lda, int ldb, int ldc, int trans_b, float alpha,
              int r_splits , hipStream_t stream);
int dig_ce_rows(float* logits, int n, int m, int label_offset, float gscale, float* out3, hipStream_t stream);
long long dig_mse_workspace_bytes(void);
long long dig_ce_rows_workspace_bytes(int n);
int dig_mse_fwd_bwd_ws(const float* pred, int ld_pred, const float* target, int M, int C, float gscale, float* loss, void* dpred,
                       int ld_dpred, float* workspace, hipStream_t stream);
int dig_ce_rows_ws(float* logits, int n, int m, int label_offset, float gscale, float* out3, float* workspace, hipStream_t stream);
int dig_infonce_finish(const float* stats6, float loss_scale, float acc_scale, float* contra, float* accs4, hipStream_t stream);
int dig_step_meters(const float* loss, const float* contra, const float* pixel, const float* accs4, const int* counts, int n_counts,
                    const float* grad_norm, float* out10, hipStream_t stream);

int dig_adamw_step(float* p, const float* g, float* m, float* v, void* bf16_shadow, long long n, const unsigned char* group_flags,
                   float lr0, float wd0, float lr1, float wd1, float beta1, float beta2, float eps, int step, float grad_scale,
                   const float* finite_gate, hipStream_t stream);
int dig_adamw_step_tr(float* p, const float* g, float* m, float* v, void* bf16_shadow, long long n, const unsigned char* group_flags,
                      float lr0, float wd0, float lr1, float wd1, float beta1, float beta2, float eps, int step, float grad_scale,
                      const float* finite_gate, const void* mats, int n_mats, int n_tiles, void* tr_out, hipStream_t stream);
int dig_adamw_step_groups(float* p, const float* g, float* m, float* v, void* bf16_shadow, long long n, const unsigned char* group_idx,
                          const float* lr_tab, const float* wd_tab, float beta1, float beta2, float eps, int step, float grad_scale,
                          const float* finite_gate, hipStream_t stream);
int dig_ema_update(float* pm, const float* p, void* bf16_shadow, long long n, float m, hipStream_t stream);
int dig_adamw_bias_corrections(float beta1, float beta2, int step, float* out2_host);
int dig_adamw_step_dev(float* p, const float* g, float* m, float* v, void* bf16_shadow, long long n, const unsigned char* group_flags,
                       const float* scalars6, float beta1, float beta2, float eps, float grad_scale, const float* finite_gate,
                       hipStream_t stream);
int dig_ema_update_dev(float* pm, const float* p, void* bf16_shadow, long long n, const float* m_and_one_minus_m, hipStream_t stream);
long long dig_sumsq_workspace_bytes(long long n);
int dig_sumsq(const float* x, long long n, float* workspace, float* out, hipStream_t stream);

long long dig_colsum_workspace_bytes(int rows, int C);
int dig_colsum(const void* x, float* out, float* workspace, int rows, int C, int ld, hipStream_t stream);
int dig_colsum_partials(const float* partials, int n_parts, int C, float* out, hipStream_t stream);
#define DIG_COLSUM_MAX_SEGS 112
typedef struct dig_colsum_seg { const float* partials; float* out; long long stride; int n_parts; int C; } dig_colsum_seg_t;
int dig_colsum_partials_multi(const dig_colsum_seg_t* segs, int n_segs, hipStream_t stream);
int dig_gelu_bwd(const void* dact, const void* pre, void* dpre, long long n, hipStream_t stream);
int dig_add_bf16(const void* a, const void* b, void* out, long long n, hipStream_t stream);
int dig_cast_f32_to_bf16(const float* x, void* y, long long n, hipStream_t stream);
int dig_cast_bf16_to_f32(const void* x, float* y, long long n, hipStream_t stream);
int dig_pad_cast_rows(const float* src, void* dst, int M, int C, int M_pad, int ld, hipStream_t stream);
int dig_fill_f32(float* x, long long n, float value, hipStream_t stream);
int dig_scale_f32(float* x, long long n, float s, hipStream_t stream);
int dig_scale_by_device_scalar(float* x, long long n, const float* scalar, float extra, hipStream_t stream);
int dig_axpy_f32(float* y, const float* x, long long n, float a, hipStream_t stream);

int dig_resize_bicubic_normalize_u8(const unsigned char* packed, const long long* offsets, const int* heights, const int* widths,
                                    int n_img, float* out, int out_h, int out_w, float mean, float std_, int max_h, int max_w,
                                    hipStream_t stream);
int dig_random_masks(unsigned char* mask, int n_rows, int n_patches, int num_mask, unsigned long long seed, unsigned step,
                     hipStream_t stream);

int dig_keyview_sample(struct dig_kv_params* params, const int* heights, const int* widths, int n_img, unsigned long long seed, unsigned step,
                       hipStream_t stream);
long long dig_keyview_workspace_bytes(long long packed_bytes, int n_img);
int dig_keyview_stage_a_u8(const unsigned char* packed, const long long* offsets, const int* heights, const int* widths, int n_img,
                           const struct dig_kv_params* params, unsigned char* work, long long work_bytes, int max_h, int max_w,
                           hipStream_t stream);
int dig_keyview_stage_b(const unsigned char* stage_a, const long long* offsets, const int* heights, const int* widths, int n_img,
                        const struct dig_kv_params* params, float* out, int out_h, int out_w, float mean, float std_, int max_h, int max_w,
                        hipStream_t stream);

int dig_abiaug_sample(struct dig_abi_params* params, long long* info, const int* heights, const int* widths, int n_img,
                      const struct dig_abi_run* run, unsigned long long seed, unsigned step, hipStream_t stream);
long long dig_abiaug_workspace_bytes(int geom, int det, int wh, int ww, const struct dig_abi_run* run);
int dig_abiaug_warp_u8(const unsigned char* packed, const long long* offsets, const int* heights, const int* widths, int n_img,
                       const struct dig_abi_params* params, const struct dig_abi_run* run, unsigned char* work, long long work_bytes,
                       int max_wh, int max_ww, hipStream_t stream);
int dig_abiaug_deteriorate_u8(const unsigned char* packed, const long long* offsets, const int* heights, const int* widths, int n_img,
                              const struct dig_abi_params* params, const struct dig_abi_run* run, unsigned char* work, long long work_bytes,
                              int max_wh, int max_ww, hipStream_t stream);
int dig_abiaug_tail(const unsigned char* packed, const long long* offsets, const int* heights, const int* widths, int n_img,
                    const struct dig_abi_params* params, const struct dig_abi_run* run, const unsigned char* work, long long work_bytes,
                    float* out, int out_h, int out_w, float mean, float std_, int max_wh, int max_ww, hipStream_t stream);
int dig_encode_labels(const int* chars, const int* offsets, const int* class_of, int eos, int padding, int unknown, int max_len, int B,
                      long long* labels, long long* lens, hipStream_t stream);

int dig_decode_embed(const long long* tokens, const float* emb, const float* pe_row, void* x, int B, int d, int vocab,
                     hipStream_t stream);
int dig_decode_self_attn(const void* qkv_cache, void* out, int B, int T, int heads, int head_dim, int t, float scale,
                         hipStream_t stream);
int dig_decode_cross_attn(const void* q, const void* kv_mem, void* out, float* weights, int B, int n_mem, int heads, int head_dim,
                          float scale, int slots_per_mem , hipStream_t stream);
int dig_beam_step(const float* logits, int ld, float* seq_scores, int B, int beam_width, int C, int eos, long long* symbols,
                  long long* predecessors, float* stored_scores, hipStream_t stream);
int dig_softmax_argmax(const float* logits, int ld, float* probs, long long* tokens, int B, int C, hipStream_t stream);
int dig_string_match(const long long* pred, const long long* target, const unsigned char* canon, int n_classes, int eos, int B, int T,
                     unsigned char* match, hipStream_t stream);
int dig_seq_cross_entropy(const float* input, const long long* target, const long long* length, int B, int T, int C,
                          float* row_workspace, float* loss, hipStream_t stream);
// ... 125 lines not shown
```

Before: 6750.

## Fuse norm1 LayerNorm into the fused attention block kernel

Adds an LN-enabled variant of attn_block_kernel that normalises the residual rows in registers before the QKV GEMM. When saving for backward it writes ln1, mean and rstd itself. The previous block's MLP chain then stops producing the next block's norm1, and the separate first layernorm launch is skipped. This removes the nln/nmu/nrs round trip through global memory and one kernel launch per block. In exchange the attention kernel gets longer prologue work and more register pressure, and the buffer layout and ABI structs grow.

```diff
diff --git a/cpu_abi/dig_cpu.cpp b/cpu_abi/dig_cpu.cpp
--- a/cpu_abi/dig_cpu.cpp
+++ b/cpu_abi/dig_cpu.cpp
@@ -215,6 +215,26 @@
   rc = dig_attn_fwd(qkv, ctx, lse, n_img, heads, D, stream);
   if (rc) return rc;
   return dig_gemm_bf16(ctx, proj_w, x_mid, R, D, D, D, D, D, 0, 0, 0, proj_b, x, D, nullptr, 0, 1.0f, 0, 0, 1, 0, 0, 0, nullptr, stream);
+}
+
+int dig_attn_block_fwd_ln(const void* x, const void* qkv_w, const float* qkv_b, const void* proj_w, const float* proj_b, const float* n1_g,
+                          const float* n1_b, float eps, void* ln1_out, float* mean, float* rstd, void* qkv, void* ctx, float* lse, void* x_mid,
+                          int n_img, int heads, int embed_dim, float scale, hipStream_t stream) {
+  if (int rc = dig_rules::attn_block_fwd_ln(x, qkv_w, qkv_b, proj_w, proj_b, n1_g, n1_b, eps, ln1_out, mean, rstd, qkv, ctx, lse, x_mid, n_img, heads,
+                                            embed_dim, scale))
+    return rc;
+  const int R = n_img * N_TOK;
+  std::vector<bf16_t> tn;
+  std::vector<float> ts;
+  if (!ln1_out) {
+    tn.resize((size_t)R * embed_dim + 8);
+    ts.resize((size_t)2 * R);
+    ln1_out = (void*)(((uintptr_t)tn.data() + 15) & ~(uintptr_t)15);
+    mean = ts.data();
+    rstd = ts.data() + R;
+  }
+  if (int rc = dig_layernorm_fwd(x, n1_g, n1_b, ln1_out, mean, rstd, R, embed_dim, eps, 0, stream)) return rc;
+  return dig_attn_block_fwd(ln1_out, x, qkv_w, qkv_b, proj_w, proj_b, qkv, ctx, lse, x_mid, n_img, heads, embed_dim, scale, stream);
 }
 
 int dig_attn_bwd_dropout(const void* qkv_, const void* ctx_, const void* dctx_, const float* lse, void* dqkv_, int n_img, int heads,
diff --git a/dig_amd/block_calls.py b/dig_amd/block_calls.py
--- a/dig_amd/block_calls.py
+++ b/dig_amd/block_calls.py
@@ -7,7 +7,7 @@
 from . import ops
 
 BF16, F32 = torch.bfloat16, torch.float32
-_F32_PIECES = ("lse", "mu2", "rs2", "nmu", "nrs")
+_F32_PIECES = ("lse", "mu2", "rs2", "nmu", "nrs", "mu1", "rs1")
 
 
 class Plan(NamedTuple):
@@ -20,12 +20,13 @@
 
 
 class _BlockSaved:
-    __slots__ = ("b16", "b32", "off", "rows", "D", "F", "n_img", "heads", "inp", "inp_ptr")
-
-    def __init__(self, b16, b32, off, rows, D, F, n_img, heads, inp, inp_ptr):
+    __slots__ = ("b16", "b32", "off", "rows", "D", "F", "n_img", "heads", "inp", "inp_ptr", "own_n1")
+
+    def __init__(self, b16, b32, off, rows, D, F, n_img, heads, inp, inp_ptr, own_n1=False):
         self.b16, self.b32, self.off, self.rows, self.D, self.F, self.n_img, self.heads = b16, b32, off, rows, D, F, n_img, heads
         self.inp = inp
         self.inp_ptr = inp_ptr
+        self.own_n1 = own_n1
 
     def ptr(self, name):
         return (self.b32 if name in _F32_PIECES else self.b16).data_ptr() + self.off[name]
@@ -43,7 +44,10 @@
         return self.b16[a:a + R * cols].view(R, cols)
 
     def tensors(self):
-        if len(self.inp) == 4:
+        if self.own_n1:
+            x = self.inp[0] if len(self.inp) == 1 else self.inp[2].view("out")
+            ln1, mu1, rs1 = self.view("ln1"), self.view("mu1"), self.view("rs1")
+        elif len(self.inp) == 4:
             x, ln1, mu1, rs1 = self.inp
         else:
             p = self.inp[2]
@@ -51,18 +55,22 @@
         return (x, ln1, mu1, rs1) + tuple(self.view(k) for k in ("qkv", "ctx", "lse", "x_mid", "ln2", "mu2", "rs2", "pre", "act"))
 
 
-def forward(blocks, x, n_img, heads, Fh, eps, save, fuse_attn):
+def forward(blocks, x, n_img, heads, Fh, eps, save, fuse_attn, norm1_in_attn=False):
     R, D = x.shape
     dev = x.device
-    off, n16, n32 = ops.block_fwd_layout(R, D, Fh, n_img, heads, save)
-    ln1, mu1, rs1 = ops.layernorm_fwd(x, blocks[0]["norm1.weight"], blocks[0]["norm1.bias"], eps)
-    inp, inp_ptr = (x, ln1, mu1, rs1), (x.data_ptr(), ln1.data_ptr(), mu1.data_ptr(), rs1.data_ptr())
-    stream, key, fuse_attn = ops.L.stream(), ("fwd_call", bool(save), R, n_img), int(fuse_attn)
+    n1 = bool(norm1_in_attn and fuse_attn and ops.L.query("dig_attn_block_supported", int(heads), int(D)))
+    off, n16, n32 = ops.block_fwd_layout(R, D, Fh, n_img, heads, save, norm1=n1)
+    if n1:
+        inp, inp_ptr = (x,), (x.data_ptr(), 0, 0, 0)
+    else:
+        ln1, mu1, rs1 = ops.layernorm_fwd(x, blocks[0]["norm1.weight"], blocks[0]["norm1.bias"], eps)
+        inp, inp_ptr = (x, ln1, mu1, rs1), (x.data_ptr(), ln1.data_ptr(), mu1.data_ptr(), rs1.data_ptr())
+    stream, key, fuse_attn = ops.L.stream(), ("fwd_call", bool(save), R, n_img, n1), int(fuse_attn)
     saved, prev = [], None
     for i, blk in enumerate(blocks):
         st = blk.get(key)
         if st is None:
-            nb = blocks[i + 1] if i + 1 < len(blocks) else None
+            nb = blocks[i + 1] if i + 1 < len(blocks) and not n1 else None
             st = blk[key] = ops.BlockFwd(
                 n_img=n_img, heads=heads, D=D, F=Fh, rows=R, save=int(bool(save)),
                 tile_qkv=ops.fwd_tile_code(R, 3 * D, D) or ops.GEMM_BK_FWD, tile_proj=ops.fwd_tile_code(R, D, D, has_resid=True) or ops.GEMM_BK_FWD,
@@ -71,18 +79,24 @@
                 proj_b=blk["attn.proj.bias"].data_ptr(), n2_g=blk["norm2.weight"].data_ptr(), n2_b=blk["norm2.bias"].data_ptr(),
                 fc1_w=blk["mlp.fc1.weight"].data_ptr(), fc1_b=blk["mlp.fc1.bias"].data_ptr(), fc2_w=blk["mlp.fc2.weight"].data_ptr(),
                 fc2_b=blk["mlp.fc2.bias"].data_ptr(), next_n1_g=nb["norm1.weight"].data_ptr() if nb else None,
-                next_n1_b=nb["norm1.bias"].data_ptr() if nb else None)
+                next_n1_b=nb["norm1.bias"].data_ptr() if nb else None,
+                n1_g=blk["norm1.weight"].data_ptr() if n1 else None, n1_b=blk["norm1.bias"].data_ptr() if n1 else None, norm1_in_attn=int(n1))
         b16 = torch.empty(n16 // 2, device=dev, dtype=BF16)
         b32 = torch.empty(n32 // 4, device=dev, dtype=F32)
         p16, p32 = b16.data_ptr(), b32.data_ptr()
         st.fuse_attn = fuse_attn
-        st.x, st.ln1 = inp_ptr[0], inp_ptr[1]
+        st.x, st.ln1 = inp_ptr[0], (inp_ptr[1] or None)
         for k in off:
             setattr(st, k, (p32 if k in _F32_PIECES else p16) + off[k])
         ops.L.call("dig_encoder_block_fwd", ctypes.byref(st), stream)
-        cur = _BlockSaved(b16, b32, off, R, D, Fh, n_img, heads, inp, inp_ptr)
+        if n1 and save:
+            inp_ptr = (inp_ptr[0], p16 + off["ln1"], p32 + off["mu1"], p32 + off["rs1"])
+        cur = _BlockSaved(b16, b32, off, R, D, Fh, n_img, heads, inp, inp_ptr, own_n1=n1)
         if save:
             saved.append(cur)
+        if n1:
+            inp, inp_ptr = ((b16, b32, cur) if save else (b16, b32)), (p16 + off["out"], 0, 0, 0)
+        elif save:
             inp, inp_ptr = (b16, b32, cur), (p16 + off["out"], p16 + off["nln"], p32 + off["nmu"], p32 + off["nrs"])
         else:
             inp, inp_ptr = (b16, b32), (p16 + off["out"], p16 + off["nln"], 0, 0)
diff --git a/dig_amd/build.py b/dig_amd/build.py
--- a/dig_amd/build.py
+++ b/dig_amd/build.py
@@ -77,7 +77,8 @@
 
 
 HOT_KERNELS = ("mlp_chain_kernel<1, true, false>", "mlp_chain_kernel<2, true, false>", "mlp_chain_kernel<0, true, false>",
-               "wgrad_wide_kernel<3, 7>", "attn_block_kernel<true, 2>", "attn_block_kernel<false, 2>", "attn_bwd_kernel<false, 3, false>", "attn_bwd_kernel<false, 3, true>",
+               "wgrad_wide_kernel<3, 7>", "attn_block_kernel<true, 2, false>", "attn_block_kernel<false, 2, false>",
+               "attn_block_kernel<true, 2, true>", "attn_block_kernel<false, 2, true>", "attn_bwd_kernel<false, 3, false>", "attn_bwd_kernel<false, 3, true>",
                "gemm_wide_kernel<false, true, 0, 4, 3, 2, 2, false, 64, 2, false>", "gemm_pwide_kernel<4, false, false>",
                "keyview_sample_kernel", "keyview_stage_a_kernel", "keyview_stage_b_kernel",
                "abiaug_sample_kernel", "abiaug_warp_kernel", "abiaug_det_kernel", "abiaug_tail_kernel",
diff --git a/dig_amd/csrc/abi_rules.h b/dig_amd/csrc/abi_rules.h
--- a/dig_amd/csrc/abi_rules.h
+++ b/dig_amd/csrc/abi_rules.h
@@ -450,6 +450,17 @@
   if (attn_qkv_bytes_over(n_img, ATTN_BLOCK_DIM)) return DIG_ERR_ARG;
   return DIG_OK;
 }
+static inline int attn_block_fwd_ln(const void* x, const void* qkv_w, const float* qkv_b, const void* proj_w, const float* proj_b, const float* n1_g,
+                                    const float* n1_b, float eps, void* ln1_out, float* mean, float* rstd, void* qkv, void* ctx, float* lse,
+                                    void* x_mid, int n_img, int heads, int embed_dim, float scale) {
+  if (!n1_g || !n1_b) return DIG_ERR_ARG;
+  if ((ln1_out == nullptr) != (mean == nullptr) || (ln1_out == nullptr) != (rstd == nullptr) || (ln1_out == nullptr) != (qkv == nullptr))
+    return DIG_ERR_ARG;
+  if (int rc = attn_block_fwd(x, x, qkv_w, qkv_b, proj_w, proj_b, qkv, ctx, lse, x_mid, n_img, heads, embed_dim, scale)) return rc;
+  if (ln1_out && !aligned16(ln1_out)) return DIG_ERR_ALIGN;
+  (void)eps;
+  return DIG_OK;
+}
 
 static inline int im2col3x3(const void* x, void* col, int n_img, int H, int W, int C, int ldc) {
   if (!x || !col || n_img <= 0 || H <= 0 || W <= 0 || C <= 0 || (C & 7) || ldc < 9LL * C || (ldc & 7)) return DIG_ERR_ARG;
diff --git a/dig_amd/csrc/attn_block.hip b/dig_amd/csrc/attn_block.hip
--- a/dig_amd/csrc/attn_block.hip
+++ b/dig_amd/csrc/attn_block.hip
@@ -58,6 +58,12 @@
   bf16_t* out;
   float scale;
   unsigned x_bytes;
+  const float* n1_g;
+  const float* n1_b;
+  float eps;
+  bf16_t* ln1_out;
+  float* mean;
+  float* rstd;
 };
 
 template <int N>
@@ -96,7 +102,42 @@
   }
 }
 
+template <bool NT = false>
+__device__ __forceinline__ void store_frag_lines(bf16_t* blk , int ld, const dig_u32x4* V ,
+                                                 unsigned char* stg, int lane) {
+  const int rr = lane & 31, hi = lane >> 5;
+  const int wr = (rr & 15) * 128, ws = rr & 7;
+  const int r8 = lane >> 3, c = lane & 7;
+#pragma unroll
+  for (int pass = 0; pass < 2; ++pass) {
+    if ((rr >> 4) == pass) {
+#pragma unroll
+      for (int s = 0; s < 4; ++s) *reinterpret_cast<dig_u32x4*>(stg + wr + (((2 * s + hi) ^ ws) << 4)) = V[s];
+    }
+    asm volatile("s_waitcnt lgkmcnt(0)" ::: "memory");
+    __builtin_amdgcn_wave_barrier();
+    const dig_u32x4 v0 = *reinterpret_cast<const dig_u32x4*>(stg + r8 * 128 + ((c ^ (r8 & 7)) << 4));
+    const dig_u32x4 v1 = *reinterpret_cast<const dig_u32x4*>(stg + (8 + r8) * 128 + ((c ^ (r8 & 7)) << 4));
+    asm volatile("s_waitcnt lgkmcnt(0)" ::: "memory");
+    __builtin_amdgcn_wave_barrier();
+    if (!(DIG_AB_ABL & 4)) {
+      dig_u32x4* d0 = reinterpret_cast<dig_u32x4*>(blk + (size_t)(16 * pass + r8) * ld + c * 8);
+      dig_u32x4* d1 = reinterpret_cast<dig_u32x4*>(blk + (size_t)(16 * pass + 8 + r8) * ld + c * 8);
+      if (NT) { __builtin_nontemporal_store(v0, d0); __builtin_nontemporal_store(v1, d1); }
+      else { *d0 = v0; *d1 = v1; }
+    }
+  }
+}
+
+__device__ __forceinline__ float ab_half_sum(float v) {
+  const unsigned a = __float_as_uint(v);
+  const auto r = __builtin_amdgcn_permlane32_swap(a, a, false, false);
+  const unsigned r0 = r[0], r1 = r[1];
+  return __uint_as_float(r0) + __uint_as_float(r1);
+}
+
 template <bool SAVE> struct AbCounts {
+  static constexpr int E_LN = (DIG_AB_ABL & 4) ? 0 : (SAVE ? 24 : 0);
   static constexpr int E_BLK = (DIG_AB_ABL & 4) ? 0 : (SAVE ? 4 : 0);
   static constexpr int E_ATT = (DIG_AB_ABL & 4) ? 0 : 4 + (SAVE ? 1 : 0);
   static constexpr int E_OUT = (DIG_AB_ABL & 4) ? 0 : 4;
@@ -108,7 +149,7 @@
   return v;
 }
 
-template <bool SAVE, int NSPLIT>
+template <bool SAVE, int NSPLIT, bool LN = false>
 __global__ __launch_bounds__(512) void attn_block_kernel(AbParams p) {
   using C = AbCounts<SAVE>;
   extern __shared__ __attribute__((aligned(16))) unsigned char smem[];
@@ -171,6 +212,68 @@
       else v = p.bp ? p.bp[i - 3 * KD] : 0.f;
       vec[i] = v;
     }
+  }
+  if constexpr (LN) {
+    float* gb = reinterpret_cast<float*>(smem + V_OFF);
+#pragma unroll
+    for (int u = 0; u < 2; ++u) {
+      const int i = u * 512 + tid0;
+      if (i < 2 * KD) gb[i] = i < KD ? p.n1_g[i] : p.n1_b[i - KD];
+    }
+    ab_wait_lgkm0();
+    __builtin_amdgcn_s_barrier();
+    asm volatile("" ::: "memory");
+    const int tid = ab_opaque(tid0);
+    const int rr = tid & 31, hi = (tid >> 5) & 1;
+    auto lo16 = [](unsigned w) { return __uint_as_float(w << 16); };
+    auto up16 = [](unsigned w) { return __uint_as_float(w & 0xffff0000u); };
+    auto tree8 = [](const float (&t)[8]) { return ((t[0] + t[1]) + (t[2] + t[3])) + ((t[4] + t[5]) + (t[6] + t[7])); };
+    float a[8] = {0.f, 0.f, 0.f, 0.f, 0.f, 0.f, 0.f, 0.f};
+#pragma unroll
+    for (int s = 0; s < KD / 16; ++s)
+#pragma unroll
+      for (int e = 0; e < 4; ++e) { a[2 * e] += lo16(xf[s][e]); a[2 * e + 1] += up16(xf[s][e]); }
+    const float mu = ab_half_sum(tree8(a)) / (float)KD;
+    float q[8] = {0.f, 0.f, 0.f, 0.f, 0.f, 0.f, 0.f, 0.f};
+#pragma unroll
+    for (int s = 0; s < KD / 16; ++s)
+#pragma unroll
+      for (int e = 0; e < 4; ++e) {
+        unsigned w = xf[s][e];
+        asm volatile("" : "+v"(w));
+        const float d0 = lo16(w) - mu, d1 = up16(w) - mu;
+        q[2 * e] += d0 * d0;
+        q[2 * e + 1] += d1 * d1;
+      }
+    const float rs = rsqrtf(ab_half_sum(tree8(q)) / (float)KD + p.eps);
+#pragma unroll
+    for (int s = 0; s < KD / 16; ++s) {
+      const f32x4 g0 = *reinterpret_cast<const f32x4*>(gb + 16 * s + 8 * hi), g1 = *reinterpret_cast<const f32x4*>(gb + 16 * s + 8 * hi + 4);
+      const f32x4 b0 = *reinterpret_cast<const f32x4*>(gb + KD + 16 * s + 8 * hi), b1 = *reinterpret_cast<const f32x4*>(gb + KD + 16 * s + 8 * hi + 4);
+      unsigned w0 = xf[s][0], w1 = xf[s][1], w2 = xf[s][2], w3 = xf[s][3];
+      asm volatile("" : "+v"(w0), "+v"(w1), "+v"(w2), "+v"(w3));
+      w0 = pack_bf2((lo16(w0) - mu) * rs * g0[0] + b0[0], (up16(w0) - mu) * rs * g0[1] + b0[1]);
+      w1 = pack_bf2((lo16(w1) - mu) * rs * g0[2] + b0[2], (up16(w1) - mu) * rs * g0[3] + b0[3]);
+      w2 = pack_bf2((lo16(w2) - mu) * rs * g1[0] + b1[0], (up16(w2) - mu) * rs * g1[1] + b1[1]);
+      w3 = pack_bf2((lo16(w3) - mu) * rs * g1[2] + b1[2], (up16(w3) - mu) * rs * g1[3] + b1[3]);
+      asm volatile("" : "+v"(w0), "+v"(w1), "+v"(w2), "+v"(w3));
+      dig_u32x4 y;
+      y[0] = w0; y[1] = w1; y[2] = w2; y[3] = w3;
+      xf[s] = y;
+    }
+    if constexpr (SAVE) {
+      const size_t row0 = (size_t)img * 256 + wave * 32;
+#pragma unroll
+      for (int j = 0; j < KD / 64; ++j) {
+        store_frag_lines<true>(p.ln1_out + row0 * KD + j * 64, KD, &xf[4 * j], smem + STG_OFF + wave * 2048, ab_opaque(tid0) & 63);
+        __builtin_amdgcn_sched_barrier(0);
+      }
+      if (hi == 0 && !(DIG_AB_ABL & 4)) {
+        p.mean[row0 + rr] = mu;
+        p.rstd[row0 + rr] = rs;
+      }
+    }
+    __builtin_amdgcn_sched_barrier(0);
   }
 
   auto tick = [&](auto slot_tag, auto tau_tag, auto nw_tag, auto pre_tag, f32x16 (&acc)[2], auto&& pre_fn) {
@@ -241,7 +344,7 @@
 
   auto head = [&](auto first_tag, int h) {
     constexpr bool FIRST = decltype(first_tag)::value;
-    constexpr int EPREV = FIRST ? 0 : C::E_BLK + C::E_ATT;
+    constexpr int EPREV = FIRST ? (LN ? C::E_LN : 0) : C::E_BLK + C::E_ATT;
     using I0 = std::integral_constant<int, 0>;
     using I1 = std::integral_constant<int, 1>;
     using I2 = std::integral_constant<int, 2>;
@@ -492,6 +595,7 @@
   p.X = (const bf16_t*)ln1; p.resid = (const bf16_t*)x; p.Wqkv = (const bf16_t*)qkv_w; p.bqkv = qkv_b; p.Wp = (const bf16_t*)proj_w; p.bp = proj_b;
   p.qkv = (bf16_t*)qkv; p.ctx = (bf16_t*)ctx; p.lse = lse; p.out = (bf16_t*)x_mid; p.scale = scale;
   p.x_bytes = (unsigned)((size_t)n_img * 256 * KD * 2);
+  p.n1_g = p.n1_b = nullptr; p.eps = 0.f; p.ln1_out = nullptr; p.mean = p.rstd = nullptr;
   static bool attr[DIG_MAX_DEVICES] = {};
   const int dev = dig_device();
   if (!attr[dev]) {
@@ -504,3 +608,27 @@
   else dig_launch(attn_block_kernel<false, DIG_AB_NSPLIT>, dim3(n_img), dim3(512), LDS_BYTES, stream, p);
   return dig_check_launch();
 }
+
+extern "C" int dig_attn_block_fwd_ln(const void* x, const void* qkv_w, const float* qkv_b, const void* proj_w, const float* proj_b,
+                                     const float* n1_g, const float* n1_b, float eps, void* ln1_out, float* mean, float* rstd, void* qkv,
+                                     void* ctx, float* lse, void* x_mid, int n_img, int heads, int embed_dim, float scale, hipStream_t stream) {
+  if (int rc = dig_rules::attn_block_fwd_ln(x, qkv_w, qkv_b, proj_w, proj_b, n1_g, n1_b, eps, ln1_out, mean, rstd, qkv, ctx, lse, x_mid, n_img, heads,
+                                            embed_dim, scale))
+    return rc;
+  AbParams p;
+  p.X = (const bf16_t*)x; p.resid = (const bf16_t*)x; p.Wqkv = (const bf16_t*)qkv_w; p.bqkv = qkv_b; p.Wp = (const bf16_t*)proj_w; p.bp = proj_b;
+  p.qkv = (bf16_t*)qkv; p.ctx = (bf16_t*)ctx; p.lse = lse; p.out = (bf16_t*)x_mid; p.scale = scale;
+  p.x_bytes = (unsigned)((size_t)n_img * 256 * KD * 2);
+  p.n1_g = n1_g; p.n1_b = n1_b; p.eps = eps; p.ln1_out = (bf16_t*)ln1_out; p.mean = mean; p.rstd = rstd;
+  static bool attr[DIG_MAX_DEVICES] = {};
+  const int dev = dig_device();
+  if (!attr[dev]) {
+    if (hipFuncSetAttribute(reinterpret_cast<const void*>(&attn_block_kernel<false, DIG_AB_NSPLIT, true>), hipFuncAttributeMaxDynamicSharedMemorySize, LDS_BYTES) != hipSuccess ||
+        hipFuncSetAttribute(reinterpret_cast<const void*>(&attn_block_kernel<true, DIG_AB_NSPLIT, true>), hipFuncAttributeMaxDynamicSharedMemorySize, LDS_BYTES) != hipSuccess)
+      return DIG_ERR_LAUNCH;
+    attr[dev] = true;
+  }
+  if (qkv) dig_launch(attn_block_kernel<true, DIG_AB_NSPLIT, true>, dim3(n_img), dim3(512), LDS_BYTES, stream, p);
+  else dig_launch(attn_block_kernel<false, DIG_AB_NSPLIT, true>, dim3(n_img), dim3(512), LDS_BYTES, stream, p);
+  return dig_check_launch();
+}
diff --git a/dig_amd/csrc/encoder_block.inc b/dig_amd/csrc/encoder_block.inc
--- a/dig_amd/csrc/encoder_block.inc
+++ b/dig_amd/csrc/encoder_block.inc
@@ -3,11 +3,19 @@
 
 extern "C" int dig_encoder_block_fwd(const dig_block_fwd_t* b, hipStream_t stream) {
   if (!b || b->rows <= 0 || b->D <= 0 || b->F <= 0 || b->n_img <= 0 || b->heads <= 0 || b->rows != b->n_img * 256) return -1;
-  if (!b->x || !b->ln1 || !b->qkv || !b->ctx || !b->lse || !b->x_mid || !b->out) return -1;
+  const bool n1_attn = b->norm1_in_attn && b->fuse_attn && dig_attn_block_supported(b->heads, b->D);
+  if (b->norm1_in_attn && (!b->n1_g || !b->n1_b)) return -1;
+  if (n1_attn && b->save && (!b->ln1 || !b->mu1 || !b->rs1)) return -1;
+  if (!b->x || (!n1_attn && !b->ln1) || !b->qkv || !b->ctx || !b->lse || !b->x_mid || !b->out) return -1;
   if (b->save && (!b->ln2 || !b->mu2 || !b->rs2 || !b->pre || !b->act)) return -1;
-  if (b->next_n1_g && (!b->nln || (b->save && (!b->nmu || !b->nrs)))) return -1;
+  if (!n1_attn && b->next_n1_g && (!b->nln || (b->save && (!b->nmu || !b->nrs)))) return -1;
   const int D = b->D, R = b->rows;
-  if (b->fuse_attn && dig_attn_block_supported(b->heads, D)) {
+  const float* nn_g = n1_attn ? nullptr : b->next_n1_g;
+  if (n1_attn) {
+    DIG_BLOCK_TRY(dig_attn_block_fwd_ln(b->x, b->qkv_w, b->qkv_b, b->proj_w, b->proj_b, b->n1_g, b->n1_b, b->eps, b->save ? (void*)b->ln1 : nullptr,
+                                        b->save ? b->mu1 : nullptr, b->save ? b->rs1 : nullptr, b->save ? b->qkv : nullptr, b->ctx,
+                                        b->save ? b->lse : nullptr, b->x_mid, b->n_img, b->heads, D, b->scale, stream));
+  } else if (b->fuse_attn && dig_attn_block_supported(b->heads, D)) {
     DIG_BLOCK_TRY(dig_attn_block_fwd(b->ln1, b->x, b->qkv_w, b->qkv_b, b->proj_w, b->proj_b, b->save ? b->qkv : nullptr, b->ctx,
                                      b->save ? b->lse : nullptr, b->x_mid, b->n_img, b->heads, D, b->scale, stream));
   } else {
@@ -19,8 +27,8 @@
   }
   return dig_mlp_chain_fwd_ln(b->x_mid, b->x_mid, b->n2_g, b->n2_b, b->eps, b->save ? b->ln2 : nullptr, b->save ? b->mu2 : nullptr,
                               b->save ? b->rs2 : nullptr, b->fc1_w, b->fc1_b, b->fc2_w, b->fc2_b, b->out, b->save ? b->pre : nullptr,
-                              b->save ? b->act : nullptr, b->next_n1_g, b->next_n1_b, b->next_n1_g ? b->nln : nullptr,
-                              (b->next_n1_g && b->save) ? b->nmu : nullptr, (b->next_n1_g && b->save) ? b->nrs : nullptr, R, D, b->F, stream);
+                              b->save ? b->act : nullptr, nn_g, n1_attn ? nullptr : b->next_n1_b, nn_g ? b->nln : nullptr,
+                              (nn_g && b->save) ? b->nmu : nullptr, (nn_g && b->save) ? b->nrs : nullptr, R, D, b->F, stream);
 }
 
 extern "C" int dig_encoder_block_bwd(const dig_block_bwd_t* b, hipStream_t stream) {
diff --git a/dig_amd/encoder_blocks.py b/dig_amd/encoder_blocks.py
--- a/dig_amd/encoder_blocks.py
+++ b/dig_amd/encoder_blocks.py
@@ -12,6 +12,7 @@
     chain: bool = False
     chain_ln: bool = False
     attn_block: bool = False
+    attn_norm1: bool = False
     chain_bwd: bool = False
     chain_every: int = 1
     chain_phase: int = 0
@@ -39,21 +40,32 @@
     R, D = x.shape
     scale = (D // heads) ** -0.5
     saved, nxt, last = [], None, len(blocks) - 1
+
+    def fused_attn(i):
+        da, dp, _ = (drops[i] or _NO_DROP) if drops is not None else _NO_DROP
+        return plan.attn_block and da is None and dp is None
+
     for i, blk in enumerate(blocks):
         keep = save and i >= frozen
-        ln1, mu1, rs1 = nxt if nxt is not None else ops.layernorm_fwd(x, blk["norm1.weight"], blk["norm1.bias"], eps)
+        da, dp, dm = (drops[i] or _NO_DROP) if drops is not None else _NO_DROP
+        if plan.attn_norm1 and fused_attn(i) and nxt is None:
+            n1 = ops.Norm1Rows(x, blk["norm1.weight"], blk["norm1.bias"], eps)
+            x_mid, ctx, qkv, lse = ops.attn_block_fwd(n1, x, blk["attn.qkv.weight"], blk["qkv_bias"], blk["attn.proj.weight"],
+                                                      blk["attn.proj.bias"], n_img, heads, D, scale, save=keep)
+            ln1, mu1, rs1 = n1.saved if keep else (None, None, None)
+        else:
+            ln1, mu1, rs1 = nxt if nxt is not None else ops.layernorm_fwd(x, blk["norm1.weight"], blk["norm1.bias"], eps)
+            if fused_attn(i):
+                x_mid, ctx, qkv, lse = ops.attn_block_fwd(ln1, x, blk["attn.qkv.weight"], blk["qkv_bias"], blk["attn.proj.weight"],
+                                                          blk["attn.proj.bias"], n_img, heads, D, scale, save=keep)
+            else:
+                qkv = ops.linear_fwd(ln1, blk["attn.qkv.weight"], bias=blk["qkv_bias"], alpha=scale, alpha_cols=D)
+                ctx, lse = ops.attn_fwd(qkv, n_img, heads, D, drop=da)
+                x_mid = ops.linear_fwd(ctx, blk["attn.proj.weight"], bias=blk["attn.proj.bias"], resid=x, drop=dp)
         nxt = None
-        da, dp, dm = (drops[i] or _NO_DROP) if drops is not None else _NO_DROP
-        if plan.attn_block and da is None and dp is None:
-            x_mid, ctx, qkv, lse = ops.attn_block_fwd(ln1, x, blk["attn.qkv.weight"], blk["qkv_bias"], blk["attn.proj.weight"],
-                                                      blk["attn.proj.bias"], n_img, heads, D, scale, save=keep)
-        else:
-            qkv = ops.linear_fwd(ln1, blk["attn.qkv.weight"], bias=blk["qkv_bias"], alpha=scale, alpha_cols=D)
-            ctx, lse = ops.attn_fwd(qkv, n_img, heads, D, drop=da)
-            x_mid = ops.linear_fwd(ctx, blk["attn.proj.weight"], bias=blk["attn.proj.bias"], resid=x, drop=dp)
         if plan.chain_ln:
             ng, nb = (blocks[i + 1]["norm1.weight"], blocks[i + 1]["norm1.bias"]) if i < last else tail
-            if i < frozen:
+            if i < frozen or (i < last and plan.attn_norm1 and fused_attn(i + 1)):
                 ng = nb = None
             r = ops.mlp_chain_fwd_ln(x_mid, blk["norm2.weight"], blk["norm2.bias"], eps, blk["mlp.fc1.weight"], blk["mlp.fc1.bias"],
                                      blk["mlp.fc2.weight"], blk["mlp.fc2.bias"], ng, nb, save=keep, drop=dm)
diff --git a/dig_amd/engine_core.py b/dig_amd/engine_core.py
--- a/dig_amd/engine_core.py
+++ b/dig_amd/engine_core.py
@@ -100,10 +100,11 @@
                        ops.L.ptr(mask_u8[half * B:(half + 1) * B]), ops.L.ptr(ew.mask_token), ops.L.ptr(M._pos),
                        ops.L.ptr(x[half * B * N:(half + 1) * B * N]), B, M.gh, M.gw, D, ops.L.stream())
         chain = ops.mlp_chain_supported(D, M.F, R) and bool(ops.MLP_CHAIN_MASK & (2 if save else 1))
-        plan = EB.Plan(chain=chain, chain_ln=chain and ops.MLP_CHAIN_LN and M.F <= 2048,
-                       attn_block=ops.attn_block_supported(H, D, B if views == 1 else None))
+        attn_block = ops.attn_block_supported(H, D, B if views == 1 else None)
+        plan = EB.Plan(chain=chain, chain_ln=chain and ops.MLP_CHAIN_LN and M.F <= 2048, attn_block=attn_block,
+                       attn_norm1=attn_block and ops.ATTN_NORM1)
         if plan.chain_ln and ops.BLOCK_CALLS and D == H * 64 and path is None:
-            return BC.forward(ew.blocks, x, views * B, H, M.F, M.ln_eps, save, fuse_attn=plan.attn_block)
+            return BC.forward(ew.blocks, x, views * B, H, M.F, M.ln_eps, save, fuse_attn=plan.attn_block, norm1_in_attn=plan.attn_norm1)
         drops = [ds and (None, ds[0], ds[1]) for ds in path] if path is not None else None
         x, saved, _ = EB.forward(plan, ew.blocks, x, views * B, H, M.ln_eps, save, drops=drops)
         return x, saved
diff --git a/dig_amd/ops.py b/dig_amd/ops.py
--- a/dig_amd/ops.py
+++ b/dig_amd/ops.py
@@ -468,7 +468,8 @@
 class BlockFwd(ctypes.Structure):
     _fields_ = ([(k, _I) for k in ("n_img", "heads", "D", "F", "rows", "save", "tile_qkv", "tile_proj", "fuse_attn", "reserved0")] + [("eps", _F), ("scale", _F)] +
                 [(k, _VP) for k in ("qkv_w", "qkv_b", "proj_w", "proj_b", "n2_g", "n2_b", "fc1_w", "fc1_b", "fc2_w", "fc2_b", "next_n1_g", "next_n1_b",
-                                    "x", "ln1", "qkv", "ctx", "lse", "x_mid", "ln2", "mu2", "rs2", "pre", "act", "out", "nln", "nmu", "nrs")])
+                                    "x", "ln1", "qkv", "ctx", "lse", "x_mid", "ln2", "mu2", "rs2", "pre", "act", "out", "nln", "nmu", "nrs",
+                                    "n1_g", "n1_b", "mu1", "rs1")] + [("norm1_in_attn", _I)])
 
 
 class BlockBwd(ctypes.Structure):
@@ -490,15 +491,17 @@
 _block_layouts = {}
 
 
-def block_fwd_layout(rows, D, Fh, n_img, heads, save):
-    key = ("f", rows, D, Fh, n_img, heads, bool(save))
+def block_fwd_layout(rows, D, Fh, n_img, heads, save, norm1=False):
+    key = ("f", rows, D, Fh, n_img, heads, bool(save), bool(norm1))
     lay = _block_layouts.get(key)
     if lay is None:
         off, n16, n32 = {}, 0, 0
-        for name, cols in (("qkv", 3 * D), ("ctx", D), ("x_mid", D), ("out", D), ("nln", D)) + ((("ln2", D), ("pre", Fh), ("act", Fh)) if save else ()):
+        n1_16 = ((("ln1", D),) if save else ()) if norm1 else (("nln", D),)
+        n1_32 = (("mu1", rows), ("rs1", rows)) if norm1 else (("nmu", rows), ("nrs", rows))
+        for name, cols in (("qkv", 3 * D), ("ctx", D), ("x_mid", D), ("out", D)) + n1_16 + ((("ln2", D), ("pre", Fh), ("act", Fh)) if save else ()):
             off[name] = n16
             n16 += _round_up(rows * cols * 2, 256)
-        for name, n in (("lse", n_img * heads * 256),) + ((("mu2", rows), ("rs2", rows), ("nmu", rows), ("nrs", rows)) if save else ()):
+        for name, n in (("lse", n_img * heads * 256),) + ((("mu2", rows), ("rs2", rows)) + n1_32 if save else ()):
             off[name] = n32
             n32 += _round_up(n * 4, 256)
         lay = _block_layouts[key] = (off, n16, n32)
@@ -626,12 +629,42 @@
             and bool(L.query("dig_attn_block_supported", int(heads), int(D))))
 
 
+ATTN_NORM1 = os.environ.get("DIG_ATTN_NORM1", "1") != "0"
+
+
+class Norm1Rows:
+    __slots__ = ("x", "gamma", "beta", "eps", "saved")
+
+    def __init__(self, x, gamma, beta, eps):
+        self.x, self.gamma, self.beta, self.eps, self.saved = x, gamma, beta, eps, None
+
+    @property
+    def shape(self):
+        return self.x.shape
+
+    @property
+    def device(self):
+        return self.x.device
+
+
 def attn_block_fwd(ln1, x, qkv_w, qkv_b, proj_w, proj_b, n_img, heads, D, scale, save=False):
     rows = ln1.shape[0]
     x_mid = torch.empty((rows, D), device=ln1.device, dtype=BF16)
     ctx = torch.empty((rows, D), device=ln1.device, dtype=BF16)
     qkv = torch.empty((rows, 3 * D), device=ln1.device, dtype=BF16) if save else None
     lse = torch.empty((n_img * heads, 256), device=ln1.device, dtype=F32) if save else None
+    if isinstance(ln1, Norm1Rows):
+        if ln1.x is not x:
+            raise ValueError("attn_block_fwd: a Norm1Rows normalises the residual rows themselves")
+        out = mean = rstd = None
+        if save:
+            out = torch.empty((rows, D), device=x.device, dtype=BF16)
+            mean, rstd = torch.empty(rows, device=x.device, dtype=F32), torch.empty(rows, device=x.device, dtype=F32)
+            ln1.saved = (out, mean, rstd)
+        L.call("dig_attn_block_fwd_ln", L.ptr(x), L.ptr(qkv_w), L.ptr(qkv_b), L.ptr(proj_w), L.ptr(proj_b), L.ptr(ln1.gamma), L.ptr(ln1.beta),
+               cf(ln1.eps), L.ptr(out), L.ptr(mean), L.ptr(rstd), L.ptr(qkv), L.ptr(ctx), L.ptr(lse), L.ptr(x_mid), n_img, heads, D, cf(scale),
+               L.stream())
+        return x_mid, ctx, qkv, lse
     L.call("dig_attn_block_fwd", L.ptr(ln1), L.ptr(x), L.ptr(qkv_w), L.ptr(qkv_b), L.ptr(proj_w), L.ptr(proj_b), L.ptr(qkv), L.ptr(ctx),
            L.ptr(lse), L.ptr(x_mid), n_img, heads, D, cf(scale), L.stream())
     return x_mid, ctx, qkv, lse
diff --git a/include/dig_block_types.h b/include/dig_block_types.h
--- a/include/dig_block_types.h
+++ b/include/dig_block_types.h
@@ -19,6 +19,9 @@
   const void* x; const void* ln1;
   void* qkv; void* ctx; float* lse; void* x_mid; void* ln2; float* mu2; float* rs2; void* pre; void* act;
   void* out; void* nln; float* nmu; float* nrs;
+  const float* n1_g; const float* n1_b;
+  float* mu1; float* rs1;
+  int norm1_in_attn;
 } dig_block_fwd_t;
 
 typedef struct dig_block_bwd {
diff --git a/include/dig_hip.h b/include/dig_hip.h
--- a/include/dig_hip.h
+++ b/include/dig_hip.h
@@ -82,6 +82,9 @@
 int dig_attn_block_fwd(const void* ln1, const void* x, const void* qkv_w, const float* qkv_b, const void* proj_w, const float* proj_b,
                        void* qkv, void* ctx, float* lse, void* x_mid, int n_img, int heads, int embed_dim, float scale,
                        hipStream_t stream);
+int dig_attn_block_fwd_ln(const void* x, const void* qkv_w, const float* qkv_b, const void* proj_w, const float* proj_b,
+                          const float* n1_g, const float* n1_b, float eps, void* ln1_out, float* mean, float* rstd, void* qkv,
+                          void* ctx, float* lse, void* x_mid, int n_img, int heads, int embed_dim, float scale, hipStream_t stream);
 
 int dig_layernorm_fwd(const void* x, const float* gamma, const float* beta, void* y, float* mean, float* rstd, int rows, int D,
                       float eps, int fuse_gelu, hipStream_t stream);
```

New measurement: 6783 (median of 6 runs). No clear change (+0.5%).
